# YihongSun/Dynamo-Depth

Hardware: AMD Instinct MI355X
Metric: training images/sec (192x640 triplets) (higher is better)
Workload: dtype f32

## Files before the change

### dynamo-depth_amd/csrc/dd_conv_mfma.hip

```cpp
#include <hip/hip_runtime.h>
#include <cstdlib>
#include <type_traits>

#include "../../include/dynamo_hip.h"
#include "dd_attr.h"
#include "dd_split.h"
#include "dd_store_tile.h"

namespace dd {
namespace cm {

constexpr int TH = 8, TW = 32, NT = 256;
constexpr int HH = TH + 2, HW = TW + 2, HN = HH * HW;
constexpr int CK = 16;
constexpr int PSTR = 48;
constexpr int A_PIECE = HN * PSTR;
constexpr int A_BYTES = 3 * A_PIECE;
__device__ __forceinline__ int halo_addr(int px, int half) {
  return px * 48 + half * 16;
}
__host__ __device__ constexpr int pieces_of(int products) { return products == 6 ? 3 : (products == 3 ? 2 : 1); }
constexpr int FRAG = 1024;
constexpr int PRE = (HN * 4 + NT - 1) / NT;

// ... 288 lines not shown
#pragma unroll
  for (int m = 0; m < 2; ++m) {
    const int loc = (2 * wave + m) * 32 + (lane & 31), p = p0 + loc;
    const int rem = p % (H * W), yy = rem / W, xx = rem - yy * W;
    unsigned mk = 0u;
#pragma unroll
    for (int t = 0; t < 9; ++t) {
      const int Y = yy + t / 3 - 1, X = xx + t % 3 - 1;
      if (p < M && Y >= 0 && Y < H && X >= 0 && X < W) mk |= 1u << t;
    }
    tapmask[m] = mk;
    a_base[m] = (W + 1) + loc;
  }
  const unsigned char* b_lane = s_b + lane * 16;

  uint4 af[2][2][3], bfr[2][NB][3];
  auto read_frags = [&](int set, int tap, int s) {
    const int toff = (tap / 3 - 1) * W + (tap % 3 - 1);
#pragma unroll
    for (int m = 0; m < 2; ++m) {
      const int addr = halo_addr(((tapmask[m] >> tap) & 1u) ? a_base[m] + toff : FLAT_ZERO, lane >> 5);
#pragma unroll
      for (int pc = 0; pc < pieces_of(NP); ++pc) af[set][m][pc] = *reinterpret_cast<const uint4*>(smem + addr + pc * A_PIECE);
    }
    const unsigned char* bb = b_lane + (s & 1) * b_buf_bytes<NB>();
#pragma unroll
    for (int n = 0; n < NB; ++n)
#pragma unroll
      for (int pc = 0; pc < pieces_of(NP); ++pc) bfr[set][n][pc] = *reinterpret_cast<const uint4*>(bb + (n * 3 + pc) * FRAG);
  };

  const int s_last = c_end * 9 - 1;
  float bv[NB];
#pragma unroll
  for (int n = 0; n < NB; ++n) bv[n] = tile_bias(splits == 1 ? bias : nullptr, (ntile * NB + n) * 32 + (lane & 31), n_out, pack);
  fetch_b(c_begin * 9);
  fetch(c_begin);
  store_b(c_begin * 9);
  fetch_b(min(c_begin * 9 + 1, s_last));
  for (int chunk = c_begin; chunk < c_end; ++chunk) {
    lds_barrier();
    stage(chunk);
    store_b(chunk * 9 + 1);
    lds_barrier();
    read_frags(0, 0, chunk * 9);
#pragma unroll
    for (int tap = 0; tap < 9; ++tap) {
      const int s = chunk * 9 + tap, cur = tap & 1;
      if (tap < 8) read_frags(cur ^ 1, tap + 1, s + 1);
      fetch_b(min(s + 2, s_last));
      if (tap == 1) fetch(min(chunk + 1, c_end - 1));
      constexpr int PA[6] = {2, 0, 1, 1, 0, 0}, PB[6] = {0, 2, 1, 0, 1, 0};
#pragma unroll
      for (int t = 6 - NP; t < 6; ++t)
#pragma unroll
        for (int m = 0; m < 2; ++m)
#pragma unroll
          for (int n = 0; n < NB; ++n)
            acc[m][n] = __builtin_amdgcn_mfma_f32_32x32x16_bf16(__builtin_bit_cast(bf8, af[cur][m][PA[t]]), __builtin_bit_cast(bf8, bfr[cur][n][PB[t]]), acc[m][n], 0, 0, 0);
      __builtin_amdgcn_sched_barrier(0);
      if (tap < 8) {
        store_b(s + 2);
        lds_barrier();
      }
    }
  }

  float* dst = out + (splits > 1 ? (size_t)split * M * n_out : 0);
  auto tail = [&](auto full) {
#pragma unroll
    for (int n = 0; n < NB; ++n) {
      const int co = (ntile * NB + n) * 32 + (lane & 31);
#pragma unroll
      for (int m = 0; m < 2; ++m) {
        const int p = p0 + (2 * wave + m) * 32 + 4 * (lane >> 5);
        store_acc32<decltype(full)::value>(acc[m][n], bv[n], dst + (size_t)p * n_out + co, (size_t)n_out, co < n_out ? M - p : 0, StoreF32{});
      }
    }
  };
  if (p0 + FLAT_MT <= M && (ntile + 1) * (32 * NB) <= n_out) tail(std::true_type{});
  else tail(std::false_type{});
}

__global__ __launch_bounds__(256) void conv_flat_fold_kernel(const float* __restrict__ part, const float* __restrict__ bias, int total4, int n_out, int splits,
                                                             float* __restrict__ y) {
  const int i = blockIdx.x * 256 + threadIdx.x;
  if (i >= total4) return;
  const float4* P = reinterpret_cast<const float4*>(part);
  float4 a = P[i];
  for (int s = 1; s < splits; ++s) {
    const float4 v = P[(size_t)s * total4 + i];
    a.x += v.x; a.y += v.y; a.z += v.z; a.w += v.w;
  }
  if (bias) {
    const int c = (i * 4) % n_out;
    a.x += bias[c]; a.y += bias[c + 1]; a.z += bias[c + 2]; a.w += bias[c + 3];
  }
  reinterpret_cast<float4*>(y)[i] = a;
}

static int flat_splits(int M, int k_in, int n_out) {
  const int wgs = ((M + FLAT_MT - 1) / FLAT_MT) * ((n_out + 63) / 64), nchunks = (k_in + CK - 1) / CK;
  const char* env = getenv("DD_FLAT_SPLITS");
  int s = env ? atoi(env) : (480 + wgs / 2) / wgs;
  if (s > nchunks / 2) s = nchunks / 2;
  return s < 1 ? 1 : s;
}

static size_t pack_bytes(int n_out, int k_in) { return (size_t)frags_of(n_out, k_in) * 3 * FRAG; }

template <int NB, int NP>
static int launch(const float* x, const void* pack, const float* bias, int B, int Hi, int Wi, int k_in, int n_out, int pad, float* y, hipStream_t stream) {
  const int Ho = Hi + 2 * pad - 2, Wo = Wi + 2 * pad - 2;
  const int tiles_x = (Wo + TW - 1) / TW, tiles_y = (Ho + TH - 1) / TH;
  auto kern = conv_mfma_kernel<NB, NP>;
  static dd::LdsAttrOnce lds_attr;
  if (const int rc = lds_attr.ensure(reinterpret_cast<const void*>(kern), (int)(lds_bytes<NB>()))) return rc;
  dim3 grid(tiles_x * tiles_y, (n_out + 32 * NB - 1) / (32 * NB), B);
  hipLaunchKernelGGL(kern, grid, dim3(NT), lds_bytes<NB>(), stream, x, static_cast<const uint4*>(pack), bias, Hi, Wi, Ho, Wo, k_in, n_out, pad, tiles_x,
                     tiles_y, y);
  return (int)hipGetLastError();
}

template <int NP>
static int launch_blocks(const float* x, const void* pack, const float* bias, int B, int Hi, int Wi, int k_in, int n_out, int pad, float* y, hipStream_t s) {
  switch (blocks_for(n_out)) {
    case 1: return launch<1, NP>(x, pack, bias, B, Hi, Wi, k_in, n_out, pad, y, s);
    case 2: return launch<2, NP>(x, pack, bias, B, Hi, Wi, k_in, n_out, pad, y, s);
    default: return launch<3, NP>(x, pack, bias, B, Hi, Wi, k_in, n_out, pad, y, s);
  }
}

template <int NP>
static int launch_flat(const float* x, const void* pack, const float* bias, int H, int W, int M, int k_in, int n_out, int splits, float* out, hipStream_t s) {
  auto kern = conv_mfma_flat_kernel<2, NP>;
  static dd::LdsAttrOnce lds_attr;
  if (const int rc = lds_attr.ensure(reinterpret_cast<const void*>(kern), (int)(lds_bytes<2>()))) return rc;
  hipLaunchKernelGGL(kern, dim3((M + FLAT_MT - 1) / FLAT_MT, (n_out + 63) / 64, splits), dim3(NT), lds_bytes<2>(), s, x, static_cast<const uint4*>(pack), bias, H, W, M, k_in,
                     n_out, splits, out);
  return (int)hipGetLastError();
}

namespace wg {
constexpr int TR = 2, TC = 16;
constexpr int XR = TR + 2, XC = TC + 2;
constexpr int XROW = 24;
constexpr int GSTR = TR * TC * 2 + 16;
constexpr int XSTR = XR * XROW * 2 + 16;
constexpr int G_PIECE = 64 * GSTR, X_PIECE = 64 * XSTR;
constexpr int LDS = 3 * (G_PIECE + X_PIECE);
constexpr int XITEMS = XR * (XC / 2) * 16;
constexpr int XJ = (XITEMS + NT - 1) / NT;
constexpr int BLOCK = 64 * 9 * 64;
}

template <int NP>
__global__ __launch_bounds__(NT, 2) void conv_wgrad_kernel(const float* __restrict__ x, const float* __restrict__ g, int B, int Hi, int Wi, int Ho, int Wo,
                                                           int cin, int cout, int pad, int tiles_x, int tiles_y, float* __restrict__ partial) {
  using namespace wg;
  extern __shared__ __align__(16) unsigned char smem[];
  unsigned char* const s_g = smem;
  unsigned char* const s_x = smem + 3 * G_PIECE;
  const int tid = threadIdx.x, lane = tid & 63, wave = __builtin_amdgcn_readfirstlane(tid >> 6);
  const int ks = blockIdx.x, nks = gridDim.x, ci0 = blockIdx.y * 64, co0 = blockIdx.z * 64;
  const int total = B * tiles_y * tiles_x;
  const int t_begin = (int)((long long)total * ks / nks), t_end = (int)((long long)total * (ks + 1) / nks);

  const int gq = tid >> 4, grow = (tid >> 3) & 1, gpair = tid & 7;
  const int g_lds = (4 * gq) * GSTR + (grow * TC + 2 * gpair) * 2;
  int xq[XJ], xrow[XJ], xpair[XJ], x_lds[XJ];
#pragma unroll
  for (int j = 0; j < XJ; ++j) {
    const int item = tid + j * NT;
    xq[j] = item / (XR * (XC / 2));
    const int rem = item - xq[j] * (XR * (XC / 2));
    xrow[j] = rem / (XC / 2);
    xpair[j] = rem - xrow[j] * (XC / 2);
    x_lds[j] = item < XITEMS ? (4 * xq[j]) * XSTR + (xrow[j] * XROW + 2 * xpair[j]) * 2 : -1;
  }
  const bool g_ch = co0 + 4 * gq < cout;

  float4 pg[2], px[XJ][2];
  auto fetch = [&](int t) {
    const int b = t / (tiles_y * tiles_x), r = t - b * (tiles_y * tiles_x);
    const int Y0 = (r / tiles_x) * TR, X0 = (r - (r / tiles_x) * tiles_x) * TC;
    {
      const int Y = Y0 + grow, X = X0 + 2 * gpair;
      const float* src = g + (((size_t)b * Ho + Y) * Wo + X) * cout + co0 + 4 * gq;
      const bool ok = g_ch && Y < Ho;
      pg[0] = (ok && X < Wo) ? *reinterpret_cast<const float4*>(src) : make_float4(0.f, 0.f, 0.f, 0.f);
      pg[1] = (ok && X + 1 < Wo) ? *reinterpret_cast<const float4*>(src + cout) : make_float4(0.f, 0.f, 0.f, 0.f);
    }
#pragma unroll
    for (int j = 0; j < XJ; ++j) {
      const int Y = Y0 - pad + xrow[j], X = X0 - pad + 2 * xpair[j];
      const bool ok = x_lds[j] >= 0 && ci0 + 4 * xq[j] < cin && Y >= 0 && Y < Hi;
      const float* src = x + (((ptrdiff_t)b * Hi + Y) * Wi + X) * cin + ci0 + 4 * xq[j];
      px[j][0] = (ok && X >= 0 && X < Wi) ? *reinterpret_cast<const float4*>(src) : make_float4(0.f, 0.f, 0.f, 0.f);
      px[j][1] = (ok && X + 1 >= 0 && X + 1 < Wi) ? *reinterpret_cast<const float4*>(src + cin) : make_float4(0.f, 0.f, 0.f, 0.f);
    }
  };
  auto put = [&](unsigned char* plane, int piece_bytes, int stride, int off, const float4& a, const float4& b) {
    const float av[4] = {a.x, a.y, a.z, a.w}, bv[4] = {b.x, b.y, b.z, b.w};
#pragma unroll
    for (int c = 0; c < 4; ++c) {
      unsigned p1, p2, p3;
      split2(av[c], bv[c], p1, p2, p3);
      *reinterpret_cast<unsigned*>(plane + off + c * stride) = p1;
      if (pieces_of(NP) > 1) *reinterpret_cast<unsigned*>(plane + piece_bytes + off + c * stride) = p2;
      if (pieces_of(NP) > 2) *reinterpret_cast<unsigned*>(plane + 2 * piece_bytes + off + c * stride) = p3;
    }
  };
  auto stage = [&]() {
    put(s_g, G_PIECE, GSTR, g_lds, pg[0], pg[1]);
#pragma unroll
    for (int j = 0; j < XJ; ++j)
      if (x_lds[j] >= 0) put(s_x, X_PIECE, XSTR, x_lds[j], px[j][0], px[j][1]);
  };

  const int ngroups = (cin - ci0 > 32) ? 6 : 3;
  const int g_full = wave, g_half = 4 + (wave >> 1), half = wave & 1;
  const bool full_on = g_full < ngroups, half_on = g_half < ngroups;
  auto group_off = [&](int g) { return (g / 3) * 32 * XSTR + (g % 3) * (XROW * 2); };
  const int off_full = group_off(g_full), off_half = group_off(g_half);
  f16v acc[9];
#pragma unroll
  for (int a = 0; a < 9; ++a)
#pragma unroll
    for (int r = 0; r < 16; ++r) acc[a][r] = 0.f;

  const unsigned char* a_lane = s_g + (lane & 31) * GSTR + (lane >> 5) * 16;
  const unsigned char* b_lane = s_x + (lane & 31) * XSTR + (lane >> 5) * 16;
  constexpr int PA[6] = {2, 0, 1, 1, 0, 0}, PB[6] = {0, 2, 1, 0, 1, 0};
  auto shifted = [](const uint4& w0, unsigned w1, int tx) -> uint4 {
    if (tx == 0) return w0;
    if (tx == 2) return make_uint4(w0.y, w0.z, w0.w, w1);
    return make_uint4(__builtin_amdgcn_alignbit(w0.y, w0.x, 16), __builtin_amdgcn_alignbit(w0.z, w0.y, 16), __builtin_amdgcn_alignbit(w0.w, w0.z, 16),
                      __builtin_amdgcn_alignbit(w1, w0.w, 16));
  };

  if (t_begin < t_end) fetch(t_begin);
  for (int t = t_begin; t < t_end; ++t) {
    __syncthreads();
    stage();
    __syncthreads();
    if (t + 1 < t_end) fetch(t + 1);
#pragma unroll
    for (int row = 0; row < TR; ++row) {
      uint4 af[2][3];
#pragma unroll
      for (int m = 0; m < 2; ++m)
#pragma unroll
        for (int pc = 0; pc < pieces_of(NP); ++pc) af[m][pc] = *reinterpret_cast<const uint4*>(a_lane + m * 32 * GSTR + row * (TC * 2) + pc * G_PIECE);
      uint4 w0[3];
      unsigned w1[3];
      if (full_on) {
#pragma unroll
        for (int pc = 0; pc < pieces_of(NP); ++pc) {
          const unsigned char* src = b_lane + off_full + row * (XROW * 2) + pc * X_PIECE;
          w0[pc] = *reinterpret_cast<const uint4*>(src);
          w1[pc] = *reinterpret_cast<const unsigned*>(src + 16);
        }
#pragma unroll
        for (int tx = 0; tx < 3; ++tx) {
          uint4 bf[3];
#pragma unroll
          for (int pc = 0; pc < pieces_of(NP); ++pc) bf[pc] = shifted(w0[pc], w1[pc], tx);
#pragma unroll
          for (int tt = 6 - NP; tt < 6; ++tt)
#pragma unroll
            for (int m = 0; m < 2; ++m)
              acc[tx * 2 + m] = __builtin_amdgcn_mfma_f32_32x32x16_bf16(__builtin_bit_cast(bf8, af[m][PA[tt]]), __builtin_bit_cast(bf8, bf[PB[tt]]),
                                                                        acc[tx * 2 + m], 0, 0, 0);
          __builtin_amdgcn_sched_barrier(0);
        }
      }
      if (half_on) {
#pragma unroll
        for (int pc = 0; pc < pieces_of(NP); ++pc) {
          const unsigned char* src = b_lane + off_half + row * (XROW * 2) + pc * X_PIECE;
          w0[pc] = *reinterpret_cast<const uint4*>(src);
          w1[pc] = *reinterpret_cast<const unsigned*>(src + 16);
        }
        {
          const int txd = half == 0 ? 0 : 2;
          uint4 bf[3];
#pragma unroll
          for (int pc = 0; pc < pieces_of(NP); ++pc) bf[pc] = txd == 0 ? shifted(w0[pc], w1[pc], 0) : shifted(w0[pc], w1[pc], 2);
#pragma unroll
          for (int tt = 6 - NP; tt < 6; ++tt)
#pragma unroll
            for (int m = 0; m < 2; ++m)
              acc[6 + m] = __builtin_amdgcn_mfma_f32_32x32x16_bf16(__builtin_bit_cast(bf8, af[m][PA[tt]]), __builtin_bit_cast(bf8, bf[PB[tt]]), acc[6 + m], 0, 0, 0);
          __builtin_amdgcn_sched_barrier(0);
          uint4 am[3];
#pragma unroll
          for (int pc = 0; pc < pieces_of(NP); ++pc) {
            bf[pc] = shifted(w0[pc], w1[pc], 1);
            am[pc] = half == 0 ? af[0][pc] : af[1][pc];
          }
#pragma unroll
          for (int tt = 6 - NP; tt < 6; ++tt)
            acc[8] = __builtin_amdgcn_mfma_f32_32x32x16_bf16(__builtin_bit_cast(bf8, am[PA[tt]]), __builtin_bit_cast(bf8, bf[PB[tt]]), acc[8], 0, 0, 0);
        }
      }
    }
  }

  float* P = partial + (((size_t)blockIdx.z * gridDim.y + blockIdx.y) * nks + ks) * BLOCK;
  auto put_acc = [&](const f16v& A, int g, int tx, int m) {
    const int nb = g / 3, tap = (g % 3) * 3 + tx;
#pragma unroll
    for (int r = 0; r < 16; ++r) {
      const int co = m * 32 + (r & 3) + 8 * (r >> 2) + 4 * (lane >> 5);
      P[(co * 9 + tap) * 64 + nb * 32 + (lane & 31)] = A[r];
    }
  };
  if (full_on) {
#pragma unroll
    for (int tx = 0; tx < 3; ++tx)
#pragma unroll
      for (int m = 0; m < 2; ++m) put_acc(acc[tx * 2 + m], g_full, tx, m);
  }
  if (half_on) {
    put_acc(acc[6], g_half, half == 0 ? 0 : 2, 0);
    put_acc(acc[7], g_half, half == 0 ? 0 : 2, 1);
    put_acc(acc[8], g_half, 1, half);
  }
}

__global__ __launch_bounds__(256) void conv_wgrad_fold_kernel(const float* __restrict__ partial, int nks, int cin, int cout, int ci_groups, float* __restrict__ gw) {
  __shared__ float red[4][64];
  const int lane = threadIdx.x & 63, wave = threadIdx.x >> 6;
  const int idx = blockIdx.x * 64 + lane;
  const bool in = idx < cout * 9 * cin;
  float s[8] = {0.f, 0.f, 0.f, 0.f, 0.f, 0.f, 0.f, 0.f};
  if (in) {
    const int ci = idx % cin, tap = (idx / cin) % 9, co = idx / (9 * cin);
    const int z = co >> 6, y = ci >> 6;
    const float* P = partial + ((size_t)z * ci_groups + y) * nks * wg::BLOCK + ((co & 63) * 9 + tap) * 64 + (ci & 63);
    int k = wave;
    for (; k + 28 < nks; k += 32) {
#pragma unroll
      for (int j = 0; j < 8; ++j) s[j] += P[(size_t)(k + 4 * j) * wg::BLOCK];
    }
    for (; k < nks; k += 4) s[0] += P[(size_t)k * wg::BLOCK];
  }
  red[wave][lane] = ((s[0] + s[1]) + (s[2] + s[3])) + ((s[4] + s[5]) + (s[6] + s[7]));
  __syncthreads();
  if (wave == 0 && in) gw[idx] = (red[0][lane] + red[1][lane]) + (red[2][lane] + red[3][lane]);
}

static int wgrad_splits(int B, int Ho, int Wo, int cin, int cout) {
  const int groups = ((cin + 63) / 64) * ((cout + 63) / 64);
  const int tiles = B * ((Ho + wg::TR - 1) / wg::TR) * ((Wo + wg::TC - 1) / wg::TC);
  int n = 512 / groups;
  if (n > tiles / 11) n = tiles / 11;
  return n < 1 ? 1 : n;
}

}
}

extern "C" int dd_conv3x3_mfma_supported(int cin, int cout) {
  return (cin >= 16 && cout >= 16 && cin % 4 == 0 && cout % 4 == 0 && cin <= 1024 && cout <= 1024) ? 1 : 0;
}

extern "C" size_t dd_conv3x3_mfma_pack_bytes(int n_out, int k_in) { return dd::cm::pack_bytes(n_out, k_in); }

extern "C" int dd_conv3x3_mfma_pack(const float* weight, long long s_co, long long s_ci, long long s_kh, long long s_kw, int cout, int cin, void* pack_fwd,
                                    void* pack_bwd_data, void* stream) {
  using namespace dd::cm;
  if (!weight || (!pack_fwd && !pack_bwd_data) || cout < 1 || cin < 1) return (int)hipErrorInvalidValue;
  const int frags_fwd = pack_fwd ? (int)(pack_bytes(cout, cin) / (3 * FRAG)) : 0;
  const int frags_bwd = pack_bwd_data ? (int)(pack_bytes(cin, cout) / (3 * FRAG)) : 0;
  const int threads = (frags_fwd + frags_bwd) * 64;
  hipLaunchKernelGGL(conv_mfma_pack_kernel, dim3((threads + 255) / 256), dim3(256), 0, static_cast<hipStream_t>(stream), weight, s_co, s_ci, s_kh, s_kw, cout,
                     cin, static_cast<uint4*>(pack_fwd), static_cast<uint4*>(pack_bwd_data), frags_fwd, frags_bwd);
  return (int)hipGetLastError();
}

extern "C" int dd_conv3x3_mfma_pack_many_job_words(void) { return dd::cm::PACK_JOB_WORDS; }

extern "C" int dd_conv3x3_mfma_pack_many_blocks(int cout, int cin, int want_fwd, int want_bwd_data) {
  using namespace dd::cm;
  if (cout < 1 || cin < 1) return 0;
  return ((want_fwd ? frags_of(cout, cin) : 0) + (want_bwd_data ? frags_of(cin, cout) : 0) + 3) / 4;
}

extern "C" int dd_conv3x3_mfma_pack_many(const long long* jobs, const int* block_job, int n_blocks, void* stream) {
  using namespace dd::cm;
  if (!jobs || !block_job || n_blocks < 1) return (int)hipErrorInvalidValue;
  hipLaunchKernelGGL(conv_mfma_pack_many_kernel, dim3(n_blocks), dim3(256), 0, static_cast<hipStream_t>(stream), jobs, block_job);
  return (int)hipGetLastError();
}

extern "C" int dd_conv3x3_mfma_n(const float* x, const void* pack, const float* bias, int B, int Hi, int Wi, int k_in, int n_out, int pad, int products,
                                 float* y, void* stream) {
  using namespace dd::cm;
  if (!x || !pack || !y || B < 1 || pad < 0 || pad > 2 || Hi + 2 * pad < 3 || Wi + 2 * pad < 3 || k_in % 4 || k_in < 4 || n_out < 1) return (int)hipErrorInvalidValue;
  if ((size_t)Hi * Wi * k_in >= (1ull << 31) || (reinterpret_cast<unsigned long long>(x) & 15ull)) return (int)hipErrorInvalidValue;
  hipStream_t s = static_cast<hipStream_t>(stream);
  switch (products) {
    case 6: return launch_blocks<6>(x, pack, bias, B, Hi, Wi, k_in, n_out, pad, y, s);
    case 3: return launch_blocks<3>(x, pack, bias, B, Hi, Wi, k_in, n_out, pad, y, s);
    case 1: return launch_blocks<1>(x, pack, bias, B, Hi, Wi, k_in, n_out, pad, y, s);
    default: return (int)hipErrorInvalidValue;
  }
}

extern "C" int dd_conv3x3_mfma(const float* x, const void* pack, const float* bias, int B, int Hi, int Wi, int k_in, int n_out, int pad, float* y,
                               void* stream) {
  return dd_conv3x3_mfma_n(x, pack, bias, B, Hi, Wi, k_in, n_out, pad, 6, y, stream);
}

extern "C" int dd_conv3x3_mfma_flat_supported(int B, int H, int W, int k_in, int n_out) {
  using namespace dd::cm;
  return (B >= 1 && H >= 1 && W >= 1 && W <= FLAT_MAX_W && k_in >= 32 && k_in % 4 == 0 && k_in <= 1024 && n_out % 4 == 0 && n_out <= 1024 &&
          blocks_for(n_out) == 2 && n_out > 32 &&
          (size_t)B * H * W * (size_t)(k_in > n_out ? k_in : n_out) < (1ull << 31)) ? 1 : 0;
}

extern "C" size_t dd_conv3x3_mfma_flat_workspace_bytes(int B, int H, int W, int k_in, int n_out) {
  using namespace dd::cm;
  const int M = B * H * W, s = flat_splits(M, k_in, n_out);
  return s > 1 ? (size_t)s * M * n_out * sizeof(float) : 16;
}

extern "C" int dd_conv3x3_mfma_flat_n(const float* x, const void* pack, const float* bias, int B, int H, int W, int k_in, int n_out, int products, float* y,
                                      void* workspace, size_t workspace_bytes, void* stream) {
  using namespace dd::cm;
  if (!x || !pack || !y || !dd_conv3x3_mfma_flat_supported(B, H, W, k_in, n_out) || (reinterpret_cast<unsigned long long>(x) & 15ull) ||
      (reinterpret_cast<unsigned long long>(y) & 15ull) || (products != 6 && products != 3 && products != 1))
    return (int)hipErrorInvalidValue;
  const int M = B * H * W, splits = flat_splits(M, k_in, n_out);
  if (splits > 1 && (!workspace || workspace_bytes < dd_conv3x3_mfma_flat_workspace_bytes(B, H, W, k_in, n_out) || (reinterpret_cast<unsigned long long>(workspace) & 15ull)))
    return (int)hipErrorInvalidValue;
  hipStream_t s = static_cast<hipStream_t>(stream);
  float* out = splits > 1 ? static_cast<float*>(workspace) : y;
  const int rc = products == 6 ? launch_flat<6>(x, pack, bias, H, W, M, k_in, n_out, splits, out, s)
               : products == 3 ? launch_flat<3>(x, pack, bias, H, W, M, k_in, n_out, splits, out, s)
                               : launch_flat<1>(x, pack, bias, H, W, M, k_in, n_out, splits, out, s);
  if (rc != 0 || splits == 1) return rc;
  const int total4 = M * n_out / 4;
  hipLaunchKernelGGL(conv_flat_fold_kernel, dim3((total4 + 255) / 256), dim3(256), 0, s, static_cast<const float*>(workspace), bias, total4, n_out, splits, y);
  return (int)hipGetLastError();
}

extern "C" int dd_conv3x3_mfma_flat(const float* x, const void* pack, const float* bias, int B, int H, int W, int k_in, int n_out, float* y, void* workspace,
                                    size_t workspace_bytes, void* stream) {
  return dd_conv3x3_mfma_flat_n(x, pack, bias, B, H, W, k_in, n_out, 6, y, workspace, workspace_bytes, stream);
}

extern "C" size_t dd_conv3x3_mfma_wgrad_workspace_bytes(int B, int Ho, int Wo, int cin, int cout) {
  const size_t groups = (size_t)((cin + 63) / 64) * ((cout + 63) / 64);
  return groups * dd::cm::wgrad_splits(B, Ho, Wo, cin, cout) * dd::cm::wg::BLOCK * sizeof(float);
}

extern "C" int dd_conv3x3_mfma_bwd_weight_n(const float* x, const float* g_out, int B, int Hi, int Wi, int cin, int cout, int pad, int products, float* g_weight,
                                            void* workspace, size_t workspace_bytes, void* stream) {
  using namespace dd::cm;
  if (!x || !g_out || !g_weight || !workspace || B < 1 || pad < 0 || pad > 1 || cin % 4 || cout % 4 || cin < 4 || cout < 4) return (int)hipErrorInvalidValue;
  if (products != 6 && products != 3 && products != 1) return (int)hipErrorInvalidValue;
  const int Ho = Hi + 2 * pad - 2, Wo = Wi + 2 * pad - 2;
  if (Ho < 1 || Wo < 1 || workspace_bytes < dd_conv3x3_mfma_wgrad_workspace_bytes(B, Ho, Wo, cin, cout)) return (int)hipErrorInvalidValue;
  if ((size_t)B * Hi * Wi * cin >= (1ull << 31) || (size_t)B * Ho * Wo * cout >= (1ull << 31)) return (int)hipErrorInvalidValue;
  if ((reinterpret_cast<unsigned long long>(x) | reinterpret_cast<unsigned long long>(g_out)) & 15ull) return (int)hipErrorInvalidValue;
  hipStream_t s = static_cast<hipStream_t>(stream);
  const int tiles_x = (Wo + wg::TC - 1) / wg::TC, tiles_y = (Ho + wg::TR - 1) / wg::TR;
  const int nks = wgrad_splits(B, Ho, Wo, cin, cout), ci_groups = (cin + 63) / 64, co_groups = (cout + 63) / 64;
  const dim3 grid(nks, ci_groups, co_groups);
  float* part = static_cast<float*>(workspace);
  if (products == 6)
    hipLaunchKernelGGL(conv_wgrad_kernel<6>, grid, dim3(NT), wg::LDS, s, x, g_out, B, Hi, Wi, Ho, Wo, cin, cout, pad, tiles_x, tiles_y, part);
  else if (products == 3)
    hipLaunchKernelGGL(conv_wgrad_kernel<3>, grid, dim3(NT), wg::LDS, s, x, g_out, B, Hi, Wi, Ho, Wo, cin, cout, pad, tiles_x, tiles_y, part);
  else
    hipLaunchKernelGGL(conv_wgrad_kernel<1>, grid, dim3(NT), wg::LDS, s, x, g_out, B, Hi, Wi, Ho, Wo, cin, cout, pad, tiles_x, tiles_y, part);
  hipError_t e = hipGetLastError();
  if (e != hipSuccess) return (int)e;
  hipLaunchKernelGGL(conv_wgrad_fold_kernel, dim3((cout * 9 * cin + 63) / 64), dim3(256), 0, s, static_cast<const float*>(workspace), nks, cin, cout, ci_groups,
                     g_weight);
  return (int)hipGetLastError();
}

extern "C" int dd_conv3x3_mfma_bwd_weight(const float* x, const float* g_out, int B, int Hi, int Wi, int cin, int cout, int pad, float* g_weight, void* workspace,
                                          size_t workspace_bytes, void* stream) {
  return dd_conv3x3_mfma_bwd_weight_n(x, g_out, B, Hi, Wi, cin, cout, pad, 6, g_weight, workspace, workspace_bytes, stream);
}
```

### dynamo-depth_amd/csrc/dd_decoder.hip

```cpp
#include <hip/hip_runtime.h>

#include "dd_half.h"
#include "dd_math.h"

namespace dd {

constexpr int DEC_NT = 256;

__device__ __forceinline__ float elu1(float v) {
  float h = 0x1.ed9a98p-8f;
  h = fmaf(h, v, 0x1.53f994p-5f);
  h = fmaf(h, v, 0x1.554e28p-3f);
  h = fmaf(h, v, 0x1.ffffe8p-2f);
  const float near0 = v * fmaf(h, v, 1.f), far = __expf(v) - 1.f;
  return v > 0.f ? v : (v > -0.25f ? near0 : far);
}
__device__ __forceinline__ float elu1_grad(float v) { return v <= 0.f ? expf(v) : 1.f; }
template <bool ELU>
__device__ __forceinline__ float4 act4(float4 v) {
  if (ELU) return make_float4(elu1(v.x), elu1(v.y), elu1(v.z), elu1(v.w));
  return v;
}

__device__ __forceinline__ void bilinear_src(int o, int n, int& i0, int& i1, float& l1) {
  const float src = fmaxf((o + 0.5f) * 0.5f - 0.5f, 0.f);
  i0 = (int)src;
  i1 = i0 + (i0 < n - 1 ? 1 : 0);
  l1 = src - (float)i0;
}

template <typename T, int MODE, bool ELU>
__global__ __launch_bounds__(DEC_NT) void up_cat_pad_kernel(const T* __restrict__ x, const T* __restrict__ skip, int h, int w, int C1q, int C2q,
                                                            T* __restrict__ out) {
  const int H = MODE == 2 ? h : 2 * h, W = MODE == 2 ? w : 2 * w, Wp = W + 2, Cq = C1q + C2q;
  const int yo = blockIdx.y, b = blockIdx.z;
  const int j = blockIdx.x * DEC_NT + threadIdx.x;
  if (j >= Wp * Cq) return;
  const int xo = j / Cq, cq = j - xo * Cq;
  const int Y = dd_reflect(yo - 1, H), X = dd_reflect(xo - 1, W);
  float4 v;
  if (cq >= C1q) {
    v = IO<T>::load4(skip, (((long long)b * H + Y) * W + X) * C2q + (cq - C1q));
  } else if (MODE == 2) {
    v = act4<ELU>(IO<T>::load4(x, (((long long)b * h + Y) * w + X) * C1q + cq));
  } else if (MODE == 0) {
    v = act4<ELU>(IO<T>::load4(x, (((long long)b * h + (Y >> 1)) * w + (X >> 1)) * C1q + cq));
  } else {
    int y0, y1, x0, x1;
    float ly, lx;
    bilinear_src(Y, h, y0, y1, ly);
    bilinear_src(X, w, x0, x1, lx);
    const long long r0 = ((long long)b * h + y0) * w, r1 = ((long long)b * h + y1) * w;
    const float4 a = act4<ELU>(IO<T>::load4(x, (r0 + x0) * C1q + cq)), bb = act4<ELU>(IO<T>::load4(x, (r0 + x1) * C1q + cq));
    const float4 c = act4<ELU>(IO<T>::load4(x, (r1 + x0) * C1q + cq)), d = act4<ELU>(IO<T>::load4(x, (r1 + x1) * C1q + cq));
    const float hy = 1.f - ly, hx = 1.f - lx;
    v.x = hy * (hx * a.x + lx * bb.x) + ly * (hx * c.x + lx * d.x);
    v.y = hy * (hx * a.y + lx * bb.y) + ly * (hx * c.y + lx * d.y);
    v.z = hy * (hx * a.z + lx * bb.z) + ly * (hx * c.z + lx * d.z);
    v.w = hy * (hx * a.w + lx * bb.w) + ly * (hx * c.w + lx * d.w);
  }
  IO<T>::store4(out, ((long long)b * (H + 2) + yo) * Wp * Cq + j, v);
}

template <typename T>
__device__ __forceinline__ float4 pad_fold(const T* __restrict__ g, int b, int Y, int X, int H, int W, int Cq, int cq) {
  const int Hp = H + 2, Wp = W + 2;
  const int ys[2] = {Y + 1, Y == 1 ? 0 : (Y == H - 2 ? Hp - 1 : -1)};
  const int xs[2] = {X + 1, X == 1 ? 0 : (X == W - 2 ? Wp - 1 : -1)};
  float4 acc = make_float4(0.f, 0.f, 0.f, 0.f);
#pragma unroll
  for (int a = 0; a < 2; ++a)
#pragma unroll
    for (int d = 0; d < 2; ++d)
      if (ys[a] >= 0 && xs[d] >= 0) {
        const float4 t = IO<T>::load4(g, (((long long)b * Hp + ys[a]) * Wp + xs[d]) * Cq + cq);
        acc.x += t.x; acc.y += t.y; acc.z += t.z; acc.w += t.w;
      }
  return acc;
}

template <int MODE>
__device__ __forceinline__ int up_taps(int i, int n, int (&o)[4], float (&wt)[4]) {
  if (MODE == 0) {
    o[0] = 2 * i; o[1] = 2 * i + 1; wt[0] = wt[1] = 1.f;
    return 2;
  }
  int cnt = 0;
  if (i >= 1) { o[cnt] = 2 * i - 1; wt[cnt++] = 0.25f; }
  o[cnt] = 2 * i; wt[cnt++] = i == 0 ? 1.f : 0.75f;
  o[cnt] = 2 * i + 1; wt[cnt++] = i == n - 1 ? 1.f : 0.75f;
  if (i + 1 <= n - 1) { o[cnt] = 2 * i + 2; wt[cnt++] = 0.25f; }
  return cnt;
}

template <typename T, int MODE, bool ELU>
__global__ __launch_bounds__(DEC_NT) void up_cat_pad_bwd_x_kernel(const T* __restrict__ g, const T* __restrict__ x, int h, int w, int C1q, int C2q,
                                                                  T* __restrict__ gx) {
  const int H = MODE == 2 ? h : 2 * h, W = MODE == 2 ? w : 2 * w, Cq = C1q + C2q;
  const int yi = blockIdx.y, b = blockIdx.z;
  const int j = blockIdx.x * DEC_NT + threadIdx.x;
  if (j >= w * C1q) return;
  const int xi = j / C1q, cq = j - xi * C1q;
  float4 acc = make_float4(0.f, 0.f, 0.f, 0.f);
  if (MODE == 2) {
    acc = pad_fold<T>(g, b, yi, xi, H, W, Cq, cq);
  } else {
    int oy[4], ox[4];
    float wy[4], wx[4];
    const int ny = up_taps<MODE>(yi, h, oy, wy), nx = up_taps<MODE>(xi, w, ox, wx);
    for (int a = 0; a < ny; ++a)
      for (int d = 0; d < nx; ++d) {
        const float4 t = pad_fold<T>(g, b, oy[a], ox[d], H, W, Cq, cq);
        const float wgt = wy[a] * wx[d];
        acc.x += wgt * t.x; acc.y += wgt * t.y; acc.z += wgt * t.z; acc.w += wgt * t.w;
      }
  }
  const long long at = ((long long)b * h + yi) * w * C1q + j;
  if (ELU) {
    const float4 v = IO<T>::load4(x, at);
    acc.x *= elu1_grad(v.x); acc.y *= elu1_grad(v.y); acc.z *= elu1_grad(v.z); acc.w *= elu1_grad(v.w);
  }
  IO<T>::store4(gx, at, acc);
}

template <typename T>
__global__ __launch_bounds__(DEC_NT) void up_cat_pad_bwd_skip_kernel(const T* __restrict__ g, int H, int W, int C1q, int C2q, T* __restrict__ gs) {
  const int Y = blockIdx.y, b = blockIdx.z;
  const int j = blockIdx.x * DEC_NT + threadIdx.x;
  if (j >= W * C2q) return;
  const int X = j / C2q, cq = j - X * C2q;
  IO<T>::store4(gs, ((long long)b * H + Y) * W * C2q + j, pad_fold<T>(g, b, Y, X, H, W, C1q + C2q, C1q + cq));
}

template <typename T>
static void up_cat_pad_launch(const void* x_, const void* skip_, int B, int h, int w, int C1, int C2, int mode, int elu, void* out_, hipStream_t s) {
  const T* x = static_cast<const T*>(x_);
  const T* skip = static_cast<const T*>(skip_);
  T* out = static_cast<T*>(out_);
  const int H = mode == 2 ? h : 2 * h, W = mode == 2 ? w : 2 * w, C1q = C1 / 4, C2q = C2 / 4;
  const dim3 grid(((W + 2) * (C1q + C2q) + DEC_NT - 1) / DEC_NT, H + 2, B), block(DEC_NT);
#define DD_UCP(M, E) hipLaunchKernelGGL((up_cat_pad_kernel<T, M, E>), grid, block, 0, s, x, skip, h, w, C1q, C2q, out)
  if (mode == 0) { if (elu) DD_UCP(0, true); else DD_UCP(0, false); }
  else if (mode == 1) { if (elu) DD_UCP(1, true); else DD_UCP(1, false); }
  else { if (elu) DD_UCP(2, true); else DD_UCP(2, false); }
#undef DD_UCP
}

template <typename T>
static void up_cat_pad_bwd_launch(const void* g_, const void* x_, int B, int h, int w, int C1, int C2, int mode, int elu, void* gx_, void* gs_,
                                  hipStream_t s) {
  const T* g = static_cast<const T*>(g_);
  const T* x = static_cast<const T*>(x_);
  T* gx = static_cast<T*>(gx_);
  T* gs = static_cast<T*>(gs_);
  const int H = mode == 2 ? h : 2 * h, W = mode == 2 ? w : 2 * w, C1q = C1 / 4, C2q = C2 / 4;
  if (gx) {
    const dim3 grid((w * C1q + DEC_NT - 1) / DEC_NT, h, B), block(DEC_NT);
#define DD_UCPB(M, E) hipLaunchKernelGGL((up_cat_pad_bwd_x_kernel<T, M, E>), grid, block, 0, s, g, x, h, w, C1q, C2q, gx)
    if (mode == 0) { if (elu) DD_UCPB(0, true); else DD_UCPB(0, false); }
    else if (mode == 1) { if (elu) DD_UCPB(1, true); else DD_UCPB(1, false); }
    else { if (elu) DD_UCPB(2, true); else DD_UCPB(2, false); }
#undef DD_UCPB
  }
  if (gs && C2q > 0)
    hipLaunchKernelGGL(up_cat_pad_bwd_skip_kernel<T>, dim3((W * C2q + DEC_NT - 1) / DEC_NT, H, B), dim3(DEC_NT), 0, s, g, H, W, C1q, C2q, gs);
}

}

using namespace dd;

static bool up_cat_pad_ok(const void* x, int B, int h, int w, int C1, int C2, int mode, int dtype) {
  const int H = mode == 2 ? h : 2 * h, W = mode == 2 ? w : 2 * w;
  return x && B >= 1 && B <= 65535 && h >= 2 && w >= 2 && H >= 4 && W >= 4 && H + 2 <= 65535 && C1 >= 4 && C1 % 4 == 0 && C2 >= 0 && C2 % 4 == 0 &&
         mode >= 0 && mode <= 2 && dtype >= 0 && dtype <= 2;
}

extern "C" int dd_up_cat_pad_t(const void* x, const void* skip, int B, int h, int w, int C1, int C2, int mode, int elu, void* out, int dtype,
                               void* stream) {
  if (!up_cat_pad_ok(x, B, h, w, C1, C2, mode, dtype) || !out || (C2 > 0 && !skip)) return (int)hipErrorInvalidValue;
  DD_DISPATCH_DTYPE(dtype, up_cat_pad_launch, x, skip, B, h, w, C1, C2, mode, elu, out, static_cast<hipStream_t>(stream));
  return (int)hipGetLastError();
}

extern "C" int dd_up_cat_pad_bwd_t(const void* g_out, const void* x, int B, int h, int w, int C1, int C2, int mode, int elu, void* g_x, void* g_skip,
                                   int dtype, void* stream) {
  if (!up_cat_pad_ok(x, B, h, w, C1, C2, mode, dtype) || !g_out || (!g_x && !g_skip)) return (int)hipErrorInvalidValue;
  DD_DISPATCH_DTYPE(dtype, up_cat_pad_bwd_launch, g_out, x, B, h, w, C1, C2, mode, elu, g_x, g_skip, static_cast<hipStream_t>(stream));
  return (int)hipGetLastError();
}
```

### dynamo-depth_amd/csrc/dd_redu.hip

```cpp
#include <hip/hip_runtime.h>

#include "../../include/dynamo_hip.h"

namespace dd {

constexpr int RD_NT = 256;
constexpr int RD_MAX_BLOCKS = 1024;
constexpr int RD_FOLD = 32;

__device__ __forceinline__ float rd_dot4(const float4 a, const float4 b) { return fmaf(a.x, b.x, fmaf(a.y, b.y, fmaf(a.z, b.z, a.w * b.w))); }

template <int C4>
__device__ __forceinline__ void rd_stage_weights(const float* __restrict__ w, int cout, float4* s_w) {
  for (int i = threadIdx.x; i < cout * 2 * C4; i += RD_NT) s_w[i] = reinterpret_cast<const float4*>(w)[i];
  __syncthreads();
}

template <int COUT, int LPP, int QUADS>
__global__ __launch_bounds__(RD_NT) void redu_fwd_kernel(const float* __restrict__ a, const float* __restrict__ b, const float* __restrict__ w,
                                                         const float* __restrict__ bias, long long P, float* __restrict__ y) {
  constexpr int C4 = LPP * QUADS, PX = RD_NT / LPP;
  __shared__ float4 s_w[COUT * 2 * C4];
  rd_stage_weights<C4>(w, COUT, s_w);
  const int pl = threadIdx.x / LPP, q = threadIdx.x % LPP;
  const float4* a4 = reinterpret_cast<const float4*>(a);
  const float4* b4 = reinterpret_cast<const float4*>(b);
  float bv[COUT];
#pragma unroll
  for (int co = 0; co < COUT; ++co) bv[co] = bias ? bias[co] : 0.f;
  const long long groups = (P + PX - 1) / PX;
  for (long long grp = blockIdx.x; grp < groups; grp += gridDim.x) {
    const long long p = grp * PX + pl;
    const long long pc = p < P ? p : P - 1;
    float acc[COUT];
#pragma unroll
    for (int co = 0; co < COUT; ++co) acc[co] = 0.f;
#pragma unroll
    for (int j = 0; j < QUADS; ++j) {
      const int c4 = q + LPP * j;
      const float4 av = a4[pc * C4 + c4], bb = b4[pc * C4 + c4];
#pragma unroll
      for (int co = 0; co < COUT; ++co) acc[co] += rd_dot4(av, s_w[co * 2 * C4 + c4]) + rd_dot4(bb, s_w[co * 2 * C4 + C4 + c4]);
    }
#pragma unroll
    for (int co = 0; co < COUT; ++co) {
#pragma unroll
      for (int m = 1; m < LPP; m <<= 1) acc[co] += __shfl_xor(acc[co], m, 64);
    }
    if (q == 0 && p < P) {
#pragma unroll
      for (int co = 0; co < COUT; ++co) y[p * COUT + co] = acc[co] + bv[co];
    }
  }
}

template <int COUT, int LPP, int QUADS>
__global__ __launch_bounds__(RD_NT) void redu_bwd_data_kernel(const float* __restrict__ g, const float* __restrict__ w, long long P, float* __restrict__ ga,
                                                              float* __restrict__ gb) {
  constexpr int C4 = LPP * QUADS, PX = RD_NT / LPP;
  __shared__ float4 s_w[COUT * 2 * C4];
  rd_stage_weights<C4>(w, COUT, s_w);
  const int pl = threadIdx.x / LPP, q = threadIdx.x % LPP;
  const long long groups = (P + PX - 1) / PX;
  for (long long grp = blockIdx.x; grp < groups; grp += gridDim.x) {
    const long long p = grp * PX + pl;
    if (p >= P) continue;
    float gv[COUT];
#pragma unroll
    for (int co = 0; co < COUT; ++co) gv[co] = g[p * COUT + co];
#pragma unroll
    for (int j = 0; j < QUADS; ++j) {
      const int c4 = q + LPP * j;
      float4 ra = make_float4(0.f, 0.f, 0.f, 0.f), rb = ra;
#pragma unroll
      for (int co = 0; co < COUT; ++co) {
        const float4 wa = s_w[co * 2 * C4 + c4], wb = s_w[co * 2 * C4 + C4 + c4];
        ra.x = fmaf(gv[co], wa.x, ra.x); ra.y = fmaf(gv[co], wa.y, ra.y); ra.z = fmaf(gv[co], wa.z, ra.z); ra.w = fmaf(gv[co], wa.w, ra.w);
        rb.x = fmaf(gv[co], wb.x, rb.x); rb.y = fmaf(gv[co], wb.y, rb.y); rb.z = fmaf(gv[co], wb.z, rb.z); rb.w = fmaf(gv[co], wb.w, rb.w);
      }
      if (ga) reinterpret_cast<float4*>(ga)[p * C4 + c4] = ra;
      if (gb) reinterpret_cast<float4*>(gb)[p * C4 + c4] = rb;
    }
  }
}

template <int COUT, int LPP, int QUADS>
__global__ __launch_bounds__(RD_NT) void redu_wgrad_kernel(const float* __restrict__ a, const float* __restrict__ b, const float* __restrict__ g, long long P,
                                                           float* __restrict__ part) {
  constexpr int C4 = LPP * QUADS, PX = RD_NT / LPP, C = 4 * C4, N = COUT * 2 * C + COUT;
  constexpr int SLOTS = COUT * QUADS * 2 * 4 + COUT, STR = SLOTS | 1;
  extern __shared__ float s_red[];
  const int pl = threadIdx.x / LPP, q = threadIdx.x % LPP;
  const float4* a4 = reinterpret_cast<const float4*>(a);
  const float4* b4 = reinterpret_cast<const float4*>(b);
  float4 accA[COUT][QUADS], accB[COUT][QUADS];
  float gs[COUT];
#pragma unroll
  for (int co = 0; co < COUT; ++co) {
    gs[co] = 0.f;
#pragma unroll
    for (int j = 0; j < QUADS; ++j) accA[co][j] = accB[co][j] = make_float4(0.f, 0.f, 0.f, 0.f);
  }
  const long long groups = (P + PX - 1) / PX;
  for (long long grp = blockIdx.x; grp < groups; grp += gridDim.x) {
    const long long p = grp * PX + pl;
    if (p >= P) continue;
    float gv[COUT];
#pragma unroll
    for (int co = 0; co < COUT; ++co) { gv[co] = g[p * COUT + co]; gs[co] += gv[co]; }
#pragma unroll
    for (int j = 0; j < QUADS; ++j) {
      const int c4 = q + LPP * j;
      const float4 av = a4[p * C4 + c4], bb = b4[p * C4 + c4];
#pragma unroll
      for (int co = 0; co < COUT; ++co) {
        accA[co][j].x = fmaf(gv[co], av.x, accA[co][j].x); accA[co][j].y = fmaf(gv[co], av.y, accA[co][j].y);
        accA[co][j].z = fmaf(gv[co], av.z, accA[co][j].z); accA[co][j].w = fmaf(gv[co], av.w, accA[co][j].w);
        accB[co][j].x = fmaf(gv[co], bb.x, accB[co][j].x); accB[co][j].y = fmaf(gv[co], bb.y, accB[co][j].y);
        accB[co][j].z = fmaf(gv[co], bb.z, accB[co][j].z); accB[co][j].w = fmaf(gv[co], bb.w, accB[co][j].w);
      }
    }
  }
  float* mine = s_red + threadIdx.x * STR;
#pragma unroll
  for (int co = 0; co < COUT; ++co) {
#pragma unroll
    for (int j = 0; j < QUADS; ++j) {
      const int t = ((co * QUADS + j) * 2) * 4;
      mine[t] = accA[co][j].x; mine[t + 1] = accA[co][j].y; mine[t + 2] = accA[co][j].z; mine[t + 3] = accA[co][j].w;
      mine[t + 4] = accB[co][j].x; mine[t + 5] = accB[co][j].y; mine[t + 6] = accB[co][j].z; mine[t + 7] = accB[co][j].w;
    }
    mine[COUT * QUADS * 8 + co] = q == 0 ? gs[co] : 0.f;
  }
  __syncthreads();
  for (int e = threadIdx.x; e < N; e += RD_NT) {
    float s = 0.f;
    if (e < COUT * 2 * C) {
      const int co = e / (2 * C), r = e - co * 2 * C, half = r / C, c = r - half * C;
      const int cq = c >> 2, qq = cq % LPP, j = cq / LPP, slot = ((co * QUADS + j) * 2 + half) * 4 + (c & 3);
#pragma unroll 4
      for (int pp = 0; pp < PX; ++pp) s += s_red[(pp * LPP + qq) * STR + slot];
    } else {
      const int co = e - COUT * 2 * C;
#pragma unroll 4
      for (int pp = 0; pp < PX; ++pp) s += s_red[(pp * LPP) * STR + COUT * QUADS * 8 + co];
    }
    part[(long long)blockIdx.x * N + e] = s;
  }
}

__global__ __launch_bounds__(RD_NT) void redu_fold1_kernel(const float* __restrict__ part, int nparts, int N, float* __restrict__ slices) {
  const int e = blockIdx.x * RD_NT + threadIdx.x, sl = blockIdx.y;
  if (e >= N) return;
  float a0 = 0.f, a1 = 0.f;
  int i = sl;
  for (; i + RD_FOLD < nparts; i += 2 * RD_FOLD) { a0 += part[(long long)i * N + e]; a1 += part[(long long)(i + RD_FOLD) * N + e]; }
  if (i < nparts) a0 += part[(long long)i * N + e];
  slices[(long long)sl * N + e] = a0 + a1;
}
__global__ __launch_bounds__(RD_NT) void redu_fold2_kernel(const float* __restrict__ slices, int N, int nw, float* __restrict__ gw, float* __restrict__ gbias) {
  const int e = blockIdx.x * RD_NT + threadIdx.x;
  if (e >= N) return;
  float a[4] = {0.f, 0.f, 0.f, 0.f};
#pragma unroll
  for (int i = 0; i < RD_FOLD; ++i) a[i & 3] += slices[(long long)i * N + e];
  const float v = (a[0] + a[1]) + (a[2] + a[3]);
  if (e < nw) gw[e] = v;
  else if (gbias) gbias[e - nw] = v;
}

struct ReduShape { int lpp, quads; };
static inline ReduShape redu_shape(int C) {
  ReduShape s = {0, 0};
  if (C == 64) s = {16, 1};
  else if (C == 128) s = {32, 1};
  else if (C == 256) s = {64, 1};
  else if (C == 512) s = {64, 2};
  return s;
}
static inline int redu_blocks(long long P, int lpp) {
  const long long groups = (P + RD_NT / lpp - 1) / (RD_NT / lpp);
  long long nb = (groups + 7) / 8;
  if (nb < 1) nb = 1;
  return (int)(nb > RD_MAX_BLOCKS ? RD_MAX_BLOCKS : nb);
}

}

extern "C" int dd_redu_supported(int C, int cout) { return dd::redu_shape(C).lpp != 0 && (cout == 1 || cout == 3); }

extern "C" size_t dd_redu_workspace_bytes(long long P, int C, int cout) {
  if (!dd_redu_supported(C, cout) || P < 1) return 0;
  const size_t N = (size_t)cout * 2 * C + cout;
  return ((size_t)dd::redu_blocks(P, dd::redu_shape(C).lpp) + dd::RD_FOLD) * N * sizeof(float);
}

#define DD_REDU_DISPATCH(KERNEL, GRID, LDS, ...)                                                                                             \
  do {                                                                                                                                       \
    const dd::ReduShape sh_ = dd::redu_shape(C);                                                                                             \
    if (cout == 1) {                                                                                                                         \
      if (sh_.lpp == 16) hipLaunchKernelGGL((dd::KERNEL<1, 16, 1>), GRID, dim3(dd::RD_NT), LDS(1, 1), st, __VA_ARGS__);                         \
      else if (sh_.lpp == 32) hipLaunchKernelGGL((dd::KERNEL<1, 32, 1>), GRID, dim3(dd::RD_NT), LDS(1, 1), st, __VA_ARGS__);                    \
      else if (sh_.quads == 1) hipLaunchKernelGGL((dd::KERNEL<1, 64, 1>), GRID, dim3(dd::RD_NT), LDS(1, 1), st, __VA_ARGS__);                   \
      else hipLaunchKernelGGL((dd::KERNEL<1, 64, 2>), GRID, dim3(dd::RD_NT), LDS(1, 2), st, __VA_ARGS__);                                        \
    } else {                                                                                                                                 \
      if (sh_.lpp == 16) hipLaunchKernelGGL((dd::KERNEL<3, 16, 1>), GRID, dim3(dd::RD_NT), LDS(3, 1), st, __VA_ARGS__);                         \
      else if (sh_.lpp == 32) hipLaunchKernelGGL((dd::KERNEL<3, 32, 1>), GRID, dim3(dd::RD_NT), LDS(3, 1), st, __VA_ARGS__);                    \
      else if (sh_.quads == 1) hipLaunchKernelGGL((dd::KERNEL<3, 64, 1>), GRID, dim3(dd::RD_NT), LDS(3, 1), st, __VA_ARGS__);                   \
      else hipLaunchKernelGGL((dd::KERNEL<3, 64, 2>), GRID, dim3(dd::RD_NT), LDS(3, 2), st, __VA_ARGS__);                                        \
    }                                                                                                                                        \
  } while (0)
#define DD_REDU_NO_LDS(co, qd) 0
#define DD_REDU_WG_LDS(co, qd) ((size_t)dd::RD_NT * ((((co) * (qd) * 8 + (co))) | 1) * sizeof(float))

extern "C" int dd_redu_fwd(const float* a, const float* b, const float* weight, const float* bias, long long P, int C, int cout, float* y, void* stream) {
  if (!a || !b || !weight || !y || P < 1 || !dd_redu_supported(C, cout)) return (int)hipErrorInvalidValue;
  hipStream_t st = (hipStream_t)stream;
  const dim3 grid(dd::redu_blocks(P, dd::redu_shape(C).lpp));
  DD_REDU_DISPATCH(redu_fwd_kernel, grid, DD_REDU_NO_LDS, a, b, weight, bias, P, y);
  return (int)hipGetLastError();
}

extern "C" int dd_redu_bwd_data(const float* g_out, const float* weight, long long P, int C, int cout, float* g_a, float* g_b, void* stream) {
  if (!g_out || !weight || (!g_a && !g_b) || P < 1 || !dd_redu_supported(C, cout)) return (int)hipErrorInvalidValue;
  hipStream_t st = (hipStream_t)stream;
  const dim3 grid(dd::redu_blocks(P, dd::redu_shape(C).lpp));
  DD_REDU_DISPATCH(redu_bwd_data_kernel, grid, DD_REDU_NO_LDS, g_out, weight, P, g_a, g_b);
  return (int)hipGetLastError();
}

extern "C" int dd_redu_bwd_weight(const float* a, const float* b, const float* g_out, long long P, int C, int cout, float* g_weight, float* g_bias,
                                  void* workspace, size_t workspace_bytes, void* stream) {
  if (!a || !b || !g_out || !g_weight || !workspace || P < 1 || !dd_redu_supported(C, cout)) return (int)hipErrorInvalidValue;
  if (workspace_bytes < dd_redu_workspace_bytes(P, C, cout)) return (int)hipErrorInvalidValue;
  hipStream_t st = (hipStream_t)stream;
  const int blocks = dd::redu_blocks(P, dd::redu_shape(C).lpp);
  const int nw = cout * 2 * C, N = nw + cout;
  float* part = static_cast<float*>(workspace);
  float* slices = part + (size_t)blocks * N;
  const dim3 grid(blocks);
  DD_REDU_DISPATCH(redu_wgrad_kernel, grid, DD_REDU_WG_LDS, a, b, g_out, P, part);
  hipLaunchKernelGGL(dd::redu_fold1_kernel, dim3((N + dd::RD_NT - 1) / dd::RD_NT, dd::RD_FOLD), dim3(dd::RD_NT), 0, st, part, blocks, N, slices);
  hipLaunchKernelGGL(dd::redu_fold2_kernel, dim3((N + dd::RD_NT - 1) / dd::RD_NT), dim3(dd::RD_NT), 0, st, slices, N, nw, g_weight, g_bias);
  return (int)hipGetLastError();
}
```

### dynamo-depth_amd/hipops/abi.py

```python
import ctypes as C

DD_MAX_SCALES = 4
DD_NUM_SRC = 2
DD_ABI_VERSION = 2
DD_MODE_RIGID, DD_MODE_FLOW, DD_MODE_FLOW_MASK = 0, 1, 2
DD_PARTIAL_STRIDE = 40
DD_SUMS_STRIDE = 8

_fp = C.c_void_p


class DDPhotoScale(C.Structure):
    _fields_ = [
        ("shift", C.c_int), ("h", C.c_int), ("w", C.c_int),
        ("w_photo", C.c_float), ("w_cons", C.c_float),
        ("disp", _fp),
        ("flow", _fp * DD_NUM_SRC),
        ("mask", _fp * DD_NUM_SRC),
        ("noise", _fp),
        ("g_disp", _fp),
        ("g_flow", _fp * DD_NUM_SRC),
        ("g_mask", _fp * DD_NUM_SRC),
        ("out_color", _fp * DD_NUM_SRC),
        ("out_sample", _fp * DD_NUM_SRC),
# ... 4 lines not shown
    ]


class DDPhotoArgs(C.Structure):
    _fields_ = [
        ("abi_version", C.c_int),
        ("B", C.c_int), ("H", C.c_int), ("W", C.c_int),
        ("num_scales", C.c_int), ("mode", C.c_int), ("automask", C.c_int), ("want_grad", C.c_int),
        ("min_depth", C.c_float), ("max_depth", C.c_float), ("ssim_weight", C.c_float),
        ("eps", C.c_float), ("disp_thr", C.c_float),
        ("target", _fp),
        ("source", _fp * DD_NUM_SRC),
        ("source_packed", _fp * DD_NUM_SRC),
        ("K", _fp), ("inv_K", _fp),
        ("T", _fp * DD_NUM_SRC),
        ("ts", _fp * DD_NUM_SRC),
        ("g_T", _fp * DD_NUM_SRC),
        ("sums", _fp),
        ("workspace", _fp),
        ("scale", DDPhotoScale * DD_MAX_SCALES),
    ]


DD_NUM_TERMS = 7
DD_MAX_RES = 128
TERM_NAMES = ("p_photo", "d_smooth", "d_ground", "c_smooth", "c_consistency", "m_sparsity", "m_smooth")


class DDAssembleArgs(C.Structure):
    _fields_ = [
        ("n", C.c_int), ("num_scales", C.c_int),
        ("coef", C.c_float * DD_NUM_TERMS),
        ("norm", C.c_float * DD_MAX_RES),
        ("term_of", C.c_int8 * DD_MAX_RES),
        ("scale_of", C.c_int8 * DD_MAX_RES),
    ]


DD_VIS_MAX_TILES = 16
DD_VIS_KINDS = {"img": 0, "ref_img": 1, "disp": 2, "mask": 3, "ego_flow": 4, "ind_flow": 5, "comp_flow": 6, "samp_flow": 7}

DD_REG_SMOOTH = 5
DD_REG_RES_STRIDE = 16


class DDRegSmooth(C.Structure):
    _fields_ = [("inp", _fp), ("g_inp", _fp), ("C", C.c_int), ("normalise", C.c_int), ("weight", C.c_float)]


class DDRegScale(C.Structure):
    _fields_ = [
        ("h", C.c_int), ("w", C.c_int),
        ("img", _fp),
        ("smooth", DDRegSmooth * DD_REG_SMOOTH),
        ("delta", _fp * DD_NUM_SRC), ("delta_sum", _fp * DD_NUM_SRC), ("prob", _fp * DD_NUM_SRC), ("g_prob", _fp * DD_NUM_SRC),
        ("w_sparsity", C.c_float * DD_NUM_SRC),
        ("disp", _fp), ("g_disp", _fp), ("inv_K", _fp), ("rand_idx", _fp), ("plane", _fp),
        ("w_ground", C.c_float),
    ]


class DDRegArgs(C.Structure):
    _fields_ = [
        ("abi_version", C.c_int), ("B", C.c_int), ("num_scales", C.c_int),
        ("np_per_it", C.c_int), ("max_it", C.c_int),
        ("tol", C.c_float), ("g_prior", C.c_float), ("min_depth", C.c_float), ("max_depth", C.c_float),
        ("res", _fp), ("workspace", _fp),
        ("scale", DDRegScale * DD_MAX_SCALES),
    ]


class DDJpegHeader(C.Structure):
    _fields_ = [("data_offset", C.c_int32), ("data_end", C.c_int32), ("width", C.c_int32), ("height", C.c_int32), ("restart_interval", C.c_int32),
                ("ncomp", C.c_int32), ("h", C.c_int32 * 3), ("v", C.c_int32 * 3), ("tq", C.c_int32 * 3), ("td", C.c_int32 * 3), ("ta", C.c_int32 * 3),
                ("reserved", C.c_int32 * 3), ("qt", (C.c_uint16 * 64) * 4), ("bits", (C.c_uint8 * 16) * 4), ("vals", (C.c_uint8 * 256) * 4)]


def ptr(t):
    return None if t is None else C.c_void_p(t.data_ptr())


def declare(lib):
    i, f, v, z = C.c_int, C.c_float, C.c_void_p, C.c_size_t
    sig = {
        "dd_photo_loss": (i, [C.POINTER(DDPhotoArgs), v]),
        "dd_photo_workspace_bytes": (z, [C.POINTER(DDPhotoArgs)]),
        "dd_photo_timing": (i, [i]),
        "dd_photo_timing_read": (i, [C.POINTER(C.c_float), C.POINTER(i), i]),
        "dd_smooth_loss": (i, [v, v, i, i, i, i, i, f, v, v, v, v]),
        "dd_smooth_workspace_bytes": (z, [i, i, i, i]),
        "dd_ground_loss": (i, [v, v, v, i, i, i, i, i, f, f, f, f, f, v, v, v, v, v]),
        "dd_ground_workspace_bytes": (z, [i, i, i, i]),
        "dd_resize_workspace_bytes": (z, [i, i, i, i, i]),
        "dd_resize_bicubic": (i, [v, i, i, i, v, v, i, i, v, v, i, v, v, i, v, z, v]),
        "dd_ground_candidates": (i, [v, v, v, i, i, i, i, i, f, f, f, v, v]),
        "dd_ground_select": (i, [v, v, v, i, i, i, i, f, f, f, f, f, v, v, v, v, v, v]),
        "dd_ground_plane": (i, [v, v, i, i, i, i, i, f, f, v, v, v, v]),
        "dd_assemble_losses": (i, [v, C.POINTER(DDAssembleArgs), v, v, v]),
        "dd_reg_losses_finish": (i, [C.POINTER(DDRegArgs), C.POINTER(DDAssembleArgs), v, v, v]),
        "dd_fused_loss": (i, [C.POINTER(DDPhotoArgs), C.POINTER(DDRegArgs), C.POINTER(DDAssembleArgs), v, v, v]),
        "dd_fused_loss_part": (i, [C.POINTER(DDPhotoArgs), C.POINTER(DDRegArgs), C.POINTER(DDAssembleArgs), v, v, v, i]),
        "dd_fused_loss_supported": (i, [C.POINTER(DDPhotoArgs), C.POINTER(DDRegArgs)]),
        "dd_reg_workspace_bytes": (z, [C.POINTER(DDRegArgs)]),
        "dd_jpeg_workspace_bytes": (z, [i, i, i, i, C.POINTER(C.c_int), C.POINTER(C.c_int)]),
        "dd_jpeg_decode": (i, [v, C.c_longlong, v, i, i, i, i, C.POINTER(C.c_int), C.POINTER(C.c_int), v, v, z, v]),
        "dd_backproject": (i, [v, v, i, i, i, v, v]),
        "dd_backproject_bwd": (i, [v, v, i, i, i, v, v]),
        "dd_project3d": (i, [v, v, v, i, i, i, f, v, v, v]),
        "dd_project3d_bwd": (i, [v, v, v, v, v, i, i, i, f, v, v, v, v]),
        "dd_project3d_workspace_bytes": (z, [i, i, i]),
        "dd_ssim": (i, [v, v, i, i, i, i, v, v]),
        "dd_ssim_bwd": (i, [v, v, v, i, i, i, i, v, v, v]),
        "dd_disp_to_depth": (i, [v, z, f, f, v, v, v]),
        "dd_pose_matrix": (i, [v, v, i, i, v, v]),
        "dd_pose_matrix_bwd": (i, [v, v, v, i, i, v, v, v]),
        "dd_channel_sum_nhwc": (i, [v, C.c_longlong, i, v, v, v]),
        "dd_channel_sum_workspace_bytes": (z, [i]),
        "dd_reflect_pad1_nhwc": (i, [v, i, i, i, i, v, v]),
        "dd_reflect_pad1_nhwc_bwd": (i, [v, i, i, i, i, v, v]),
        "dd_dwconv3x3_nhwc": (i, [v, v, i, i, i, i, i, v, v]),
        "dd_dwconv3x3_nhwc_bwd_data": (i, [v, v, i, i, i, i, i, v, v]),
        "dd_dwconv3x3_nhwc_bwd_weight": (i, [v, v, i, i, i, i, i, v, v, z, v]),
        "dd_dwconv3x3_workspace_bytes": (z, [i, i, i]),
        "dd_conv3x3_cout1_bwd_data": (i, [v, v, i, i, i, i, i, v, v]),
        "dd_prepare_frames": (i, [v, v, v, i, i, i, i, v, v, v, v]),
        "dd_prepare_frames_workspace_bytes": (z, [i, i]),
        "dd_pyramid_down2": (i, [v, i, i, i, v, v]),
        "dd_pack_rgb": (i, [v, i, i, i, v, v]),
        "dd_depth_metrics": (i, [v, i, i, i, v, v, i, v, C.POINTER(C.c_double), f, f, v, v, v, z, v]),
        "dd_depth_metrics_workspace_bytes": (z, [i, i]),
        "dd_depth_metrics_masked": (i, [v, i, i, i, v, v, i, v, C.POINTER(C.c_double), f, f, v, i, i, v, v, v, v, z, v]),
        "dd_depth_metrics_masked_workspace_bytes": (z, [i, i]),
        "dd_depth_metrics_accumulate": (i, [v, v, i, v, v, v]),
        "dd_odom_snippet_count": (i, [i, i]),
        "dd_odom_snippets": (i, [v, v, i, i, v, v, v]),
        "dd_motion_pr": (i, [v, i, i, i, v, v, i, i, v, i, i, v, v]),
        "dd_fill_contours": (i, [v, i, v, i, i, i, i, v, v]),
        "dd_lidar_depth_points_workspace_bytes": (z, [i, i, i, i]),
        "dd_lidar_depth_points": (i, [v, C.c_longlong, C.POINTER(C.c_int32), i, v, i, i, i, v, v, v, v, z, v]),
        "dd_vis_frame": (i, [v, v, v, v, v, v, v, v, f, f, i, i, C.POINTER(C.c_int), i, i, i, v, f, f, f, f, i, i, v, v, v, v]),
        "dd_vis_flow_tiles": (i, [v, v, C.POINTER(C.c_int), i, i, i, i, i, i, f, i, v, v]),
        "dd_export_depth": (i, [v, v, v, i, i, i, i, i, f, f, f, v, f, f, v, v, v, v]),
        "dd_export_plane_u8": (i, [v, i, i, i, i, i, v, v]),
        "dd_bn_act_fwd": (i, [v, v, C.c_longlong, i, v, v, f, f, v, v, v, v, i, v, v, z, v]),
        "dd_bn_act_bwd": (i, [v, v, v, C.c_longlong, i, v, v, v, v, i, v, v, v, v, v, z, v]),
        "dd_bn_workspace_bytes": (z, [i]),
        "dd_bn_act_fwd_t": (i, [v, v, C.c_longlong, i, v, v, f, f, v, v, v, v, i, v, i, v, z, v]),
        "dd_bn_act_bwd_t": (i, [v, v, v, C.c_longlong, i, v, v, v, v, i, v, v, v, v, i, v, z, v]),
        "dd_channel_sum_nhwc_t": (i, [v, C.c_longlong, i, v, i, v, v]),
        "dd_reflect_pad1_nhwc_t": (i, [v, i, i, i, i, v, i, v]),
        "dd_reflect_pad1_nhwc_bwd_t": (i, [v, i, i, i, i, v, i, v]),
        "dd_up_cat_pad_t": (i, [v, v, i, i, i, i, i, i, i, v, i, v]),
        "dd_up_cat_pad_bwd_t": (i, [v, v, i, i, i, i, i, i, i, v, v, i, v]),
        "dd_layer_norm_fwd": (i, [v, C.c_longlong, i, v, v, f, v, v, v, v]),
        "dd_layer_norm_bwd": (i, [v, v, v, v, v, C.c_longlong, i, v, v, v, z, v]),
        "dd_layer_norm_workspace_bytes": (z, [i]),
        "dd_layer_scale_bwd": (i, [v, v, v, i, i, i, v, v, v, z, v]),
        "dd_layer_scale_workspace_bytes": (z, [i, i]),
        "dd_layer_norm_fwd_t": (i, [v, C.c_longlong, i, v, v, f, v, v, v, i, v]),
        "dd_layer_norm_bwd_t": (i, [v, v, v, v, v, C.c_longlong, i, v, v, v, z, i, v]),
        "dd_layer_scale_bwd_t": (i, [v, v, v, i, i, i, v, v, v, z, i, v]),
        "dd_layer_scale_fwd_t": (i, [v, v, v, i, i, i, v, i, v]),
        "dd_dwconv3x3_nhwc_t": (i, [v, v, i, i, i, i, i, v, i, v]),
        "dd_dwconv3x3_nhwc_bwd_data_t": (i, [v, v, i, i, i, i, i, v, i, v]),
        "dd_dwconv3x3_nhwc_bwd_weight_t": (i, [v, v, i, i, i, i, i, v, v, z, i, v]),
        "dd_redu_supported": (i, [i, i]),
        "dd_redu_workspace_bytes": (z, [C.c_longlong, i, i]),
        "dd_redu_fwd": (i, [v, v, v, v, C.c_longlong, i, i, v, v]),
        "dd_redu_bwd_data": (i, [v, v, C.c_longlong, i, i, v, v, v]),
        "dd_redu_bwd_weight": (i, [v, v, v, C.c_longlong, i, i, v, v, v, z, v]),
        "dd_conv_head_supported": (i, [i]),
        "dd_conv_head_workspace_bytes": (z, [i, i, i, i]),
        "dd_conv_head_fwd": (i, [v, v, C.c_longlong, C.c_longlong, C.c_longlong, v, i, i, i, i, v, v]),
        "dd_conv_head_bwd_weight": (i, [v, v, i, i, i, i, v, v, v, z, v]),
        "dd_conv_small_supported": (i, [i, i, i]),
        "dd_conv_small_workspace_bytes": (z, [i, i, i]),
        "dd_conv_small_fwd": (i, [v, v, C.c_longlong, C.c_longlong, C.c_longlong, C.c_longlong, v, i, i, i, i, i, i, v, v, z, v]),
        "dd_conv_small_bwd_data": (i, [v, v, C.c_longlong, C.c_longlong, C.c_longlong, C.c_longlong, i, i, i, i, i, i, v, v, z, v]),
        "dd_conv_small_bwd_weight": (i, [v, v, i, i, i, i, i, i, v, v, v, z, v]),
        "dd_conv3x3_mfma_supported": (i, [i, i]),
        "dd_conv3x3_mfma_pack_bytes": (z, [i, i]),
        "dd_conv3x3_mfma_pack": (i, [v, C.c_longlong, C.c_longlong, C.c_longlong, C.c_longlong, i, i, v, v, v]),
        "dd_conv3x3_mfma_pack_many_job_words": (i, []),
        "dd_conv3x3_mfma_pack_many_blocks": (i, [i, i, i, i]),
        "dd_conv3x3_mfma_pack_many": (i, [v, v, i, v]),
        "dd_conv3x3_mfma": (i, [v, v, v, i, i, i, i, i, i, v, v]),
        "dd_conv3x3_mfma_n": (i, [v, v, v, i, i, i, i, i, i, i, v, v]),
        "dd_conv3x3_mfma_flat_supported": (i, [i, i, i, i, i]),
        "dd_conv3x3_mfma_flat_workspace_bytes": (z, [i, i, i, i, i]),
        "dd_conv3x3_mfma_flat": (i, [v, v, v, i, i, i, i, i, v, v, z, v]),
        "dd_conv3x3_mfma_flat_n": (i, [v, v, v, i, i, i, i, i, i, v, v, z, v]),
        "dd_conv3x3_mfma_wgrad_workspace_bytes": (z, [i, i, i, i, i]),
        "dd_conv3x3_mfma_bwd_weight": (i, [v, v, i, i, i, i, i, i, v, v, z, v]),
        "dd_conv3x3_mfma_bwd_weight_n": (i, [v, v, i, i, i, i, i, i, i, v, v, z, v]),
        "dd_conv3x3_half_supported": (i, [i, i]),
        "dd_conv3x3_half_pack_bytes": (z, [i, i]),
        "dd_conv3x3_half_pack": (i, [v, C.c_longlong, C.c_longlong, C.c_longlong, C.c_longlong, i, i, i, v, v, v]),
        "dd_conv3x3_half": (i, [v, v, v, i, i, i, i, i, i, i, v, v]),
        "dd_conv3x3_half_wgrad_workspace_bytes": (z, [i, i, i, i, i]),
        "dd_conv3x3_half_bwd_weight": (i, [v, v, i, i, i, i, i, i, i, v, v, z, v]),
        "dd_pw_gemm_pack_bytes": (z, [i, i]),
        "dd_mlp_pack": (i, [v, C.c_longlong, C.c_longlong, v, C.c_longlong, C.c_longlong, i, i, v, v, v, v, v, v]),
        "dd_mlp_fwd_supported": (i, [i]),
        "dd_mlp_fwd": (i, [v, v, v, v, v, i, i, v, v]),
        "dd_pw_gemm": (i, [v, v, v, i, i, i, i, v, v]),
        "dd_gelu_pair": (i, [v, v, v, z, v]),
        "dd_linear_wgrad_supported": (i, [i, i, i]),
        "dd_linear_wgrad_workspace_bytes": (z, [i, i, i]),
        "dd_linear_wgrad": (i, [v, v, i, i, i, v, v, v, z, v]),
        "dd_linear_wgrad_n": (i, [v, v, i, i, i, i, v, v, v, z, v]),
        "dd_adam_chunk": (i, []),
        "dd_adam_multi": (i, [v, i, v, i, v, C.c_double, C.c_double, C.c_double, C.c_double, C.c_double, v, v, v]),
        "dd_error_string": (C.c_char_p, [i]),
        "dd_abi_version": (i, []),
    }
    found = []
    for name, (res, args) in sig.items():
        try:
            fn = getattr(lib, name)
        except AttributeError:
            continue
        fn.restype = res
        fn.argtypes = args
        found.append(name)
    return found


EXPORTED = (
    "dd_photo_loss", "dd_photo_workspace_bytes", "dd_photo_timing", "dd_photo_timing_read", "dd_photo_loss_part", "dd_smooth_loss", "dd_smooth_workspace_bytes",
    "dd_ground_loss", "dd_ground_workspace_bytes", "dd_ground_plane", "dd_ground_candidates", "dd_ground_select",
    "dd_assemble_losses", "dd_reg_losses_finish", "dd_fused_loss", "dd_fused_loss_part", "dd_fused_loss_supported", "dd_reg_workspace_bytes", "dd_backproject", "dd_backproject_bwd", "dd_project3d", "dd_project3d_bwd", "dd_project3d_workspace_bytes",
    "dd_ssim", "dd_ssim_bwd", "dd_disp_to_depth", "dd_pose_matrix", "dd_pose_matrix_bwd",
    "dd_channel_sum_nhwc", "dd_channel_sum_workspace_bytes", "dd_reflect_pad1_nhwc", "dd_reflect_pad1_nhwc_bwd",
    "dd_dwconv3x3_nhwc", "dd_dwconv3x3_nhwc_bwd_data", "dd_dwconv3x3_nhwc_bwd_weight", "dd_dwconv3x3_workspace_bytes", "dd_conv3x3_cout1_bwd_data",
    "dd_prepare_frames", "dd_prepare_frames_workspace_bytes", "dd_pyramid_down2", "dd_pack_rgb", "dd_depth_metrics", "dd_depth_metrics_workspace_bytes", "dd_depth_metrics_masked", "dd_depth_metrics_masked_workspace_bytes", "dd_depth_metrics_accumulate", "dd_odom_snippet_count", "dd_odom_snippets", "dd_motion_pr", "dd_fill_contours", "dd_lidar_depth_points", "dd_lidar_depth_points_workspace_bytes", "dd_vis_frame", "dd_vis_flow_tiles", "dd_export_depth", "dd_export_plane_u8", "dd_bn_act_fwd", "dd_bn_act_bwd", "dd_bn_workspace_bytes",
    "dd_bn_act_fwd_t", "dd_bn_act_bwd_t", "dd_channel_sum_nhwc_t", "dd_reflect_pad1_nhwc_t", "dd_reflect_pad1_nhwc_bwd_t", "dd_up_cat_pad_t", "dd_up_cat_pad_bwd_t",
    "dd_layer_norm_fwd", "dd_layer_norm_bwd", "dd_layer_norm_workspace_bytes", "dd_layer_scale_bwd", "dd_layer_scale_workspace_bytes",
    "dd_jpeg_workspace_bytes", "dd_jpeg_decode", "dd_resize_workspace_bytes", "dd_resize_bicubic", "dd_layer_norm_fwd_t", "dd_layer_norm_bwd_t", "dd_layer_scale_bwd_t", "dd_layer_scale_fwd_t", "dd_dwconv3x3_nhwc_t", "dd_dwconv3x3_nhwc_bwd_data_t",
    "dd_dwconv3x3_nhwc_bwd_weight_t", "dd_adam_chunk", "dd_adam_multi", "dd_conv_small_supported", "dd_conv_small_workspace_bytes",
    "dd_conv_small_fwd", "dd_conv_small_bwd_data", "dd_conv_small_bwd_weight", "dd_conv_head_supported", "dd_conv_head_workspace_bytes", "dd_conv_head_fwd",
    "dd_conv_head_bwd_weight", "dd_redu_supported", "dd_redu_workspace_bytes", "dd_redu_fwd", "dd_redu_bwd_data", "dd_redu_bwd_weight",
    "dd_conv3x3_mfma_supported", "dd_conv3x3_mfma_pack_bytes", "dd_conv3x3_mfma_pack", "dd_conv3x3_mfma_pack_many_job_words",
    "dd_conv3x3_mfma_pack_many_blocks", "dd_conv3x3_mfma_pack_many", "dd_conv3x3_mfma", "dd_conv3x3_mfma_n",
    "dd_conv3x3_mfma_flat_supported", "dd_conv3x3_mfma_flat_workspace_bytes", "dd_conv3x3_mfma_flat", "dd_conv3x3_mfma_flat_n",
    "dd_conv3x3_mfma_wgrad_workspace_bytes", "dd_conv3x3_mfma_bwd_weight", "dd_conv3x3_mfma_bwd_weight_n",
    "dd_conv3x3_half_supported", "dd_conv3x3_half_pack_bytes", "dd_conv3x3_half_pack", "dd_conv3x3_half",
    "dd_conv3x3_half_wgrad_workspace_bytes", "dd_conv3x3_half_bwd_weight",
    "dd_pw_gemm_pack_bytes", "dd_mlp_pack", "dd_pw_gemm", "dd_gelu_pair", "dd_mlp_fwd_supported", "dd_mlp_fwd",
    "dd_linear_wgrad_supported", "dd_linear_wgrad_workspace_bytes", "dd_linear_wgrad", "dd_linear_wgrad_n",
    "dd_error_string", "dd_abi_version",
)


def fill_photo_args(*, B, H, W, mode, automask, want_grad, min_depth, max_depth, ssim_weight, eps, disp_thr,
                    target, source, K, inv_K, T, ts, g_T, sums, workspace, scales, source_packed=None):
    a = DDPhotoArgs()
    a.abi_version = DD_ABI_VERSION
    a.B, a.H, a.W = B, H, W
    a.num_scales = len(scales)
    a.mode, a.automask, a.want_grad = mode, int(bool(automask)), int(bool(want_grad))
    a.min_depth, a.max_depth, a.ssim_weight, a.eps, a.disp_thr = min_depth, max_depth, ssim_weight, eps, disp_thr
    a.target = ptr(target)
    a.K, a.inv_K = ptr(K), ptr(inv_K)
    a.sums, a.workspace = ptr(sums), ptr(workspace)
    for f in range(DD_NUM_SRC):
        a.source[f] = ptr(source[f])
        a.source_packed[f] = ptr(source_packed[f]) if source_packed is not None else None
        a.T[f] = ptr(T[f])
        a.ts[f] = ptr(ts[f]) if ts is not None else None
        a.g_T[f] = ptr(g_T[f]) if g_T is not None else None
    for s, d in enumerate(scales):
        sc = a.scale[s]
        sc.shift, sc.h, sc.w = d["shift"], d["h"], d["w"]
        sc.w_photo, sc.w_cons = d.get("w_photo", 0.0), d.get("w_cons", 0.0)
        for name in ("disp", "noise", "g_disp", "out_depth", "out_idsel"):
            setattr(sc, name, ptr(d.get(name)))
        for name in ("flow", "mask", "g_flow", "g_mask", "out_color", "out_sample", "out_resid", "out_delta"):
            pair = d.get(name) or (None, None)
            arr = getattr(sc, name)
            for f in range(DD_NUM_SRC):
                arr[f] = ptr(pair[f])
    return a
```

### dynamo-depth_amd/hipops/functions.py

```python
import os

import torch

from . import lib as L
from .pack_many import PackSet, _ACTIVE_PACK_SETS, _pack_many_on, pack_many_launches, pack_weights_once_per_forward


def _dev(t, name="tensor"):
    if not t.is_cuda:
        raise L.DynamoHipError("%s must live on the GPU: the Dynamo-Depth loss path has no CPU implementation "
                               "(libdynamo_hip.so is the only backend)" % name)
    if t.dtype != torch.float32:
        raise L.DynamoHipError("%s must be float32, got %s" % (name, t.dtype))
    return t.contiguous()


DTYPE_CODE = {torch.float32: 0, torch.float16: 1, torch.bfloat16: 2}


def _p(t):
    return None if t is None else t.data_ptr()


def _ws(nbytes, device):
# ... 130 lines not shown
        return g_points, None, g_T, None, None, None


class SSIMFn(torch.autograd.Function):

    @staticmethod
    def forward(ctx, x, y):
        x, y = _dev(x, "x"), _dev(y, "y")
        B, Cc, H, W = x.shape
        out = torch.empty_like(x)
        L.check(L.load().dd_ssim(_p(x), _p(y), B, Cc, H, W, _p(out), L.current_stream()), "dd_ssim")
        ctx.save_for_backward(x, y)
        return out

    @staticmethod
    def backward(ctx, g):
        x, y = ctx.saved_tensors
        B, Cc, H, W = x.shape
        g = _dev(g, "grad")
        gx = torch.empty_like(x) if ctx.needs_input_grad[0] else None
        gy = torch.empty_like(y) if ctx.needs_input_grad[1] else None
        L.check(L.load().dd_ssim_bwd(_p(x), _p(y), _p(g), B, Cc, H, W, _p(gx), _p(gy), L.current_stream()), "dd_ssim_bwd")
        return gx, gy


class DispToDepthFn(torch.autograd.Function):

    @staticmethod
    def forward(ctx, disp, min_depth, max_depth):
        disp = _dev(disp, "disp")
        scaled, depth = torch.empty_like(disp), torch.empty_like(disp)
        L.check(L.load().dd_disp_to_depth(_p(disp), disp.numel(), min_depth, max_depth, _p(scaled), _p(depth), L.current_stream()),
                "dd_disp_to_depth")
        ctx.save_for_backward(depth)
        ctx.span = 1.0 / min_depth - 1.0 / max_depth
        return scaled, depth

    @staticmethod
    def backward(ctx, g_scaled, g_depth):
        (depth,) = ctx.saved_tensors
        g = torch.zeros_like(depth)
        if g_scaled is not None:
            g = g + g_scaled * ctx.span
        if g_depth is not None:
            g = g - g_depth * depth * depth * ctx.span
        return g, None, None


class PoseMatrixFn(torch.autograd.Function):

    @staticmethod
    def forward(ctx, axisangle, translation, invert):
        B = axisangle.shape[0]
        aa = _dev(axisangle.reshape(B, 3), "axisangle")
        tr = _dev(translation.reshape(B, 3), "translation")
        T = torch.empty(B, 4, 4, dtype=torch.float32, device=aa.device)
        L.check(L.load().dd_pose_matrix(_p(aa), _p(tr), B, int(bool(invert)), _p(T), L.current_stream()), "dd_pose_matrix")
        ctx.save_for_backward(aa, tr)
        ctx.invert = int(bool(invert))
        ctx.shapes = (axisangle.shape, translation.shape)
        return T

    @staticmethod
    def backward(ctx, g):
        aa, tr = ctx.saved_tensors
        B = aa.shape[0]
        g = _dev(g, "grad")
        ga, gt = torch.empty_like(aa), torch.empty_like(tr)
        L.check(L.load().dd_pose_matrix_bwd(_p(aa), _p(tr), _p(g), B, ctx.invert, _p(ga), _p(gt), L.current_stream()), "dd_pose_matrix_bwd")
        return ga.reshape(ctx.shapes[0]), gt.reshape(ctx.shapes[1]), None


class SmoothLossFn(torch.autograd.Function):

    @staticmethod
    def forward(ctx, inp, img, normalise):
        inp = _dev(inp, "inp")
        img = None if img is None else _dev(img, "img")
        B, Cc, h, w = inp.shape
        lib = L.load()
        g = torch.zeros_like(inp)
        sums = torch.empty(2, dtype=torch.float32, device=inp.device)
        ws = _ws(lib.dd_smooth_workspace_bytes(B, Cc, h, w), inp.device)
        L.check(lib.dd_smooth_loss(_p(inp), _p(img), B, Cc, h, w, int(bool(normalise)), 1.0, _p(g), _p(sums), _p(ws), L.current_stream()),
                "dd_smooth_loss")
        ctx.save_for_backward(g)
        return sums[0] / (B * Cc * h * (w - 1)) + sums[1] / (B * Cc * (h - 1) * w)

    @staticmethod
    def backward(ctx, go):
        (g,) = ctx.saved_tensors
        return g * go, None, None


class ConvBiasFn(torch.autograd.Function):

    @staticmethod
    def forward(ctx, x, weight, bias, stride, padding, dilation, groups):
        ctx.save_for_backward(x, weight)
        ctx.conf = (stride, padding, dilation, groups, bias.shape[0])
        return torch.nn.functional.conv2d(x, weight, bias, stride, padding, dilation, groups)

    @staticmethod
    def backward(ctx, g):
        x, weight = ctx.saved_tensors
        stride, padding, dilation, groups, cout = ctx.conf
        if x.dtype != g.dtype:
            x = x.to(g.dtype)
        if weight.dtype != g.dtype:
            weight = weight.to(g.dtype)
        cin = x.shape[1]
        head = (ctx.needs_input_grad[0] and cout == 1 and _conv3x3_s1(x, weight, stride, padding, dilation, groups, ((0, 0), (1, 1)))
                and g.is_cuda and g.dtype == torch.float32 and x.dtype == torch.float32 and cin % 4 == 0 and cin <= 512
                and x.is_contiguous(memory_format=torch.channels_last) and not x.is_contiguous())
        mask = (ctx.needs_input_grad[0] and not head, ctx.needs_input_grad[1], False)
        gx, gw, _ = torch.ops.aten.convolution_backward(g, x, weight, None, stride, padding, dilation, False, [0, 0], groups, mask)
        if head:
            B, _, Hi, Wi = x.shape
            gx = torch.empty_like(x)
            L.check(L.load().dd_conv3x3_cout1_bwd_data(_p(g.contiguous()), _p(weight.contiguous()), B, Hi, Wi, cin, padding[0], _p(gx),
                                                       L.current_stream()), "dd_conv3x3_cout1_bwd_data")
        gb = None
        if ctx.needs_input_grad[2]:
            fast = g.is_cuda and g.dtype in DTYPE_CODE and g.dim() == 4 and cout <= 256
            if fast and not g.is_contiguous():
                gl = g if g.is_contiguous(memory_format=torch.channels_last) else g.contiguous(memory_format=torch.channels_last)
                B, _, H, W = gl.shape
                gb = _channel_sum(gl, B * H * W, cout, DTYPE_CODE[gl.dtype], L.current_stream())
            else:
                gb = g.sum((0, 2, 3))
        if gw is not None and gw.dtype != ctx.saved_tensors[1].dtype:
            gw = gw.to(ctx.saved_tensors[1].dtype)
        return gx, gw, (gb.to(torch.float32) if gb is not None else None), None, None, None, None


def redu_ok(a, b, conv):
    if os.environ.get("DD_STOCK_REDU", "0") == "1" or torch.is_autocast_enabled():
        return False
    w = conv.weight
    if not (a.is_cuda and a.dtype == torch.float32 and b.dtype == torch.float32 and w.dtype == torch.float32 and a.dim() == 4 and a.shape == b.shape):
        return False
    B, Cc, H, W = a.shape
    if tuple(w.shape) != (w.shape[0], 2 * Cc, 1, 1) or conv.groups != 1 or tuple(conv.stride) != (1, 1) or tuple(conv.padding) != (0, 0):
        return False
    nhwc = (H * W * Cc, 1, W * Cc, Cc)
    if a.stride() != nhwc or b.stride() != nhwc:
        return False
    return bool(L.load().dd_redu_supported(Cc, w.shape[0]))


class ReduFn(torch.autograd.Function):

    @staticmethod
    def forward(ctx, a, b, weight, bias):
        lib = L.load()
        B, Cc, H, W = a.shape
        cout = weight.shape[0]
        y = _nhwc_empty(B, cout, H, W, a.device)
        wm = weight.reshape(cout, 2 * Cc)
        if not wm.is_contiguous():
            wm = wm.contiguous()
        L.check(lib.dd_redu_fwd(_p(a), _p(b), _p(wm), _p(bias), B * H * W, Cc, cout, _p(y), L.current_stream()), "dd_redu_fwd")
        ctx.save_for_backward(a, b, wm)
        ctx.has_bias = bias is not None
        ctx.wshape = tuple(weight.shape)
        return y

    @staticmethod
    def backward(ctx, g):
        a, b, wm = ctx.saved_tensors
        lib = L.load()
        B, Cc, H, W = a.shape
        cout = wm.shape[0]
        P = B * H * W
        g = _dense_nhwc(g.to(torch.float32))
        ga = gb = gw = gbias = None
        if ctx.needs_input_grad[0] or ctx.needs_input_grad[1]:
            ga = torch.empty_like(a) if ctx.needs_input_grad[0] else None
            gb = torch.empty_like(b) if ctx.needs_input_grad[1] else None
            L.check(lib.dd_redu_bwd_data(_p(g), _p(wm), P, Cc, cout, _p(ga), _p(gb), L.current_stream()), "dd_redu_bwd_data")
        if ctx.needs_input_grad[2] or (ctx.has_bias and ctx.needs_input_grad[3]):
            gw = torch.empty(cout, 2 * Cc, dtype=torch.float32, device=g.device)
            gbias = torch.empty(cout, dtype=torch.float32, device=g.device) if ctx.has_bias else None
            nbytes = _ws_bytes("dd_redu_workspace_bytes", P, Cc, cout)
            ws = _ws(nbytes, g.device)
            L.check(lib.dd_redu_bwd_weight(_p(a), _p(b), _p(g), P, Cc, cout, _p(gw), _p(gbias), _p(ws), nbytes, L.current_stream()), "dd_redu_bwd_weight")
            gw = gw.view(ctx.wshape)
        return ga, gb, gw, gbias


def head_conv_ok(x, weight, stride, padding, dilation, groups):
    if os.environ.get("DD_STOCK_HEAD_CONV", "0") == "1":
        return False
    if not (x.is_cuda and x.dtype == torch.float32 and weight.dtype == torch.float32 and x.dim() == 4):
        return False
    if weight.shape[0] != 1 or not _conv3x3_s1(x, weight, stride, padding, dilation, groups, ((0, 0),)):
        return False
    B, Cc, Hp, Wp = x.shape
    if Hp < 3 or Wp < 3 or torch.is_autocast_enabled() or x.stride() != (Hp * Wp * Cc, 1, Wp * Cc, Cc):
        return False
    return bool(L.load().dd_conv_head_supported(Cc))


class HeadConvFn(torch.autograd.Function):

    @staticmethod
    def forward(ctx, x, weight, bias):
        lib = L.load()
        B, Cc, Hp, Wp = x.shape
        out = torch.empty((B, 1, Hp - 2, Wp - 2), dtype=torch.float32, device=x.device)
        sw = weight.stride()
        L.check(lib.dd_conv_head_fwd(_p(x), _p(weight), sw[1], sw[2], sw[3], _p(bias), B, Hp, Wp, Cc, _p(out), L.current_stream()), "dd_conv_head_fwd")
        ctx.save_for_backward(x, weight)
        ctx.has_bias = bias is not None
        return out

    @staticmethod
    def backward(ctx, g):
        x, weight = ctx.saved_tensors
        lib = L.load()
        B, Cc, Hp, Wp = x.shape
        g = g.to(torch.float32).contiguous()
        gx = gw = gb = None
        if ctx.needs_input_grad[0]:
            gx = torch.empty_like(x)
            L.check(lib.dd_conv3x3_cout1_bwd_data(_p(g), _p(weight.contiguous()), B, Hp, Wp, Cc, 0, _p(gx), L.current_stream()), "dd_conv3x3_cout1_bwd_data")
        if ctx.needs_input_grad[1] or (ctx.has_bias and ctx.needs_input_grad[2]):
            flat = torch.empty(9 * Cc, dtype=torch.float32, device=g.device)
            gb = torch.empty(1, dtype=torch.float32, device=g.device) if ctx.has_bias else None
            nbytes = int(lib.dd_conv_head_workspace_bytes(B, Hp, Wp, Cc))
            ws = _ws(nbytes, g.device)
            L.check(lib.dd_conv_head_bwd_weight(_p(x), _p(g), B, Hp, Wp, Cc, _p(flat), _p(gb), _p(ws), nbytes, L.current_stream()), "dd_conv_head_bwd_weight")
            gw = flat.view(1, 3, 3, Cc).permute(0, 3, 1, 2)
        return gx, gw, gb


def small_conv_ok(x, weight, stride, padding, dilation, groups):
    if os.environ.get("DD_STOCK_SMALL_CONV", "0") == "1":
        return False
    if not (x.is_cuda and x.dtype == torch.float32 and weight.dtype == torch.float32 and x.dim() == 4 and weight.dim() == 4):
        return False
    cout, cin, kh, kw = weight.shape
    if kh != kw or kh not in (1, 3) or groups != 1 or tuple(stride) != (1, 1) or tuple(dilation) != (1, 1) or tuple(padding) != (kh // 2, kh // 2):
        return False
    if x.shape[1] != cin or x.shape[0] * x.shape[2] * x.shape[3] < (1 << 16):
        return False
    if torch.is_autocast_enabled():
        return False
    return bool(L.load().dd_conv_small_supported(kh, cin, cout))


def _dense_nhwc(t):
    B, Cc, H, W = t.shape
    if t.stride() == (H * W * Cc, 1, W * Cc, Cc):
        return t
    return t.contiguous(memory_format=torch.channels_last).as_strided((B, Cc, H, W), (H * W * Cc, 1, W * Cc, Cc)) if Cc > 1 else \
        t.contiguous().as_strided((B, Cc, H, W), (H * W, 1, W, 1))


_SMALL_CONV_CALLS = [0]


def small_conv_calls():
    return _SMALL_CONV_CALLS[0]


class SmallConvFn(torch.autograd.Function):

    @staticmethod
    def forward(ctx, x, weight, bias):
        lib = L.load()
        cout, cin, ks, _ = weight.shape
        B, _, H, W = x.shape
        x = _dense_nhwc(x)
        y = _nhwc_empty(B, cout, H, W, x.device)
        nbytes = _ws_bytes("dd_conv_small_workspace_bytes", ks, cin, cout)
        ws = _ws(nbytes, x.device)
        sw = weight.stride()
        L.check(lib.dd_conv_small_fwd(_p(x), _p(weight), sw[0], sw[1], sw[2], sw[3], _p(bias), B, H, W, cin, cout, ks, _p(y), _p(ws), nbytes,
                                      L.current_stream()), "dd_conv_small_fwd")
        _SMALL_CONV_CALLS[0] += 1
        ctx.save_for_backward(x, weight)
        ctx.has_bias = bias is not None
        return y

    @staticmethod
    def backward(ctx, g):
        x, weight = ctx.saved_tensors
        lib = L.load()
        cout, cin, ks, _ = weight.shape
        B, _, H, W = x.shape
        g = _dense_nhwc(g.to(torch.float32))
        nbytes = _ws_bytes("dd_conv_small_workspace_bytes", ks, cin, cout)
        gx = gw = gb = None
        if ctx.needs_input_grad[0]:
            gx = _nhwc_empty(B, cin, H, W, g.device)
            ws = _ws(nbytes, g.device)
            sw = weight.stride()
            L.check(lib.dd_conv_small_bwd_data(_p(g), _p(weight), sw[0], sw[1], sw[2], sw[3], B, H, W, cin, cout, ks, _p(gx), _p(ws), nbytes,
                                               L.current_stream()), "dd_conv_small_bwd_data")
        if ctx.needs_input_grad[1] or (ctx.has_bias and ctx.needs_input_grad[2]):
            flat = torch.empty(cout * ks * ks * cin, dtype=torch.float32, device=g.device)
            gb = torch.empty(cout, dtype=torch.float32, device=g.device) if ctx.has_bias else None
            ws = _ws(nbytes, g.device)
            L.check(lib.dd_conv_small_bwd_weight(_p(x), _p(g), B, H, W, cin, cout, ks, _p(flat), _p(gb), _p(ws), nbytes, L.current_stream()),
                    "dd_conv_small_bwd_weight")
            gw = flat.view(cout, ks, ks, cin).permute(0, 3, 1, 2)
        return gx, gw, gb


def small_conv(x, weight, bias=None):
    return SmallConvFn.apply(x, weight, bias)


def mfma_conv_ok(x, weight, stride, padding, dilation, groups):
    if os.environ.get("DD_STOCK_MFMA_CONV", "0") == "1":
        return False
    if not (x.is_cuda and x.dtype == torch.float32 and weight.dtype == torch.float32 and x.dim() == 4):
        return False
    if not _conv3x3_s1(x, weight, stride, padding, dilation, groups, ((0, 0), (1, 1))) or torch.is_autocast_enabled():
        return False
    cout, cin = weight.shape[:2]
    pad = padding[0]
    Ho, Wo = x.shape[2] + 2 * pad - 2, x.shape[3] + 2 * pad - 2
    if _below_tile_pixels(x.shape[0], Ho, Wo, "DD_MFMA_CONV_MIN_PIXELS"):
        return pad == 1 and _flat_conv_ok(x.shape[0], x.shape[2], x.shape[3], cin, cout)
    return bool(L.load().dd_conv3x3_mfma_supported(cin, cout))


def _flat_conv_ok(B, H, W, cin, cout):
    if os.environ.get("DD_FLAT_MFMA_CONV", "1") != "1" or min(cin, cout) < int(os.environ.get("DD_FLAT_MIN_CHANNELS", "256")):
        return False
    lib = L.load()
    return bool(lib.dd_conv3x3_mfma_flat_supported(B, H, W, cin, cout)) and bool(lib.dd_conv3x3_mfma_flat_supported(B, H, W, cout, cin))


def _flat_shape(B, H, W, pad, k_in=None, n_out=None):
    Ho, Wo = H + 2 * pad - 2, W + 2 * pad - 2
    if not (pad == 1 and _below_tile_pixels(B, Ho, Wo, "DD_MFMA_CONV_MIN_PIXELS")):
        return False
    if os.environ.get("DD_FLAT_MFMA_CONV", "1") != "1":
        return False
    return k_in is None or bool(L.load().dd_conv3x3_mfma_flat_supported(B, H, W, k_in, n_out))


_MFMA_CONV_CALLS = [0]
_FLAT_CONV_CALLS = [0]


def mfma_conv_calls():
    return _MFMA_CONV_CALLS[0]


_PRODUCTS = {"highest": 6, "high": 3, "medium": 1}


def mfma_products():
    env = os.environ.get("DD_MFMA_PRODUCTS")
    return int(env) if env else _PRODUCTS[torch.get_float32_matmul_precision()]


class MfmaConvFn(torch.autograd.Function):

    @staticmethod
    def forward(ctx, x, weight, bias, pad):
        lib = L.load()
        cout, cin = weight.shape[:2]
        B, _, Hi, Wi = x.shape
        x = _dense_nhwc(x)
        need_gx = ctx.needs_input_grad[0]
        stream = L.current_stream()
        products = mfma_products()
        pset = _ACTIVE_PACK_SETS[-1] if (_ACTIVE_PACK_SETS and _pack_many_on()) else None
        packs = pset.take(weight, need_gx) if pset is not None else None
        if packs is not None:
            pack_f, pack_b = packs
        else:
            pack_f = torch.empty(_ws_bytes("dd_conv3x3_mfma_pack_bytes", cout, cin) // 4, dtype=torch.float32, device=x.device)
            pack_b = torch.empty(_ws_bytes("dd_conv3x3_mfma_pack_bytes", cin, cout) // 4, dtype=torch.float32, device=x.device) if need_gx else None
            sw = weight.stride()
            L.check(lib.dd_conv3x3_mfma_pack(_p(weight), sw[0], sw[1], sw[2], sw[3], cout, cin, _p(pack_f), _p(pack_b), stream), "dd_conv3x3_mfma_pack")
            if pset is not None and isinstance(weight, torch.nn.Parameter):
                pset.join(weight, pack_f, pack_b)
        Ho, Wo = Hi + 2 * pad - 2, Wi + 2 * pad - 2
        y = _nhwc_empty(B, cout, Ho, Wo, x.device)
        if _flat_shape(B, Hi, Wi, pad, cin, cout):
            nbytes = _ws_bytes("dd_conv3x3_mfma_flat_workspace_bytes", B, Hi, Wi, cin, cout)
            ws = _ws(nbytes, x.device)
            L.check(lib.dd_conv3x3_mfma_flat_n(_p(x), _p(pack_f), _p(bias), B, Hi, Wi, cin, cout, products, _p(y), _p(ws), nbytes, stream), "dd_conv3x3_mfma_flat")
            _FLAT_CONV_CALLS[0] += 1
        else:
            L.check(lib.dd_conv3x3_mfma_n(_p(x), _p(pack_f), _p(bias), B, Hi, Wi, cin, cout, pad, products, _p(y), stream), "dd_conv3x3_mfma")
        _MFMA_CONV_CALLS[0] += 1
        ctx.save_for_backward(x, weight, pack_b)
        ctx.conf = (pad, bias is not None, products)
        return y

    @staticmethod
    def backward(ctx, g):
        x, weight, pack_b = ctx.saved_tensors
        pad, has_bias, products = ctx.conf
        lib = L.load()
        cout, cin = weight.shape[:2]
        B, _, Hi, Wi = x.shape
        Ho, Wo = g.shape[2:]
        g = _dense_nhwc(g.to(torch.float32))
        gx = gw = gb = None
        stream = L.current_stream()
        if ctx.needs_input_grad[0]:
            gx = _nhwc_empty(B, cin, Hi, Wi, g.device)
            if _flat_shape(B, Hi, Wi, pad, cout, cin):
                nbytes = _ws_bytes("dd_conv3x3_mfma_flat_workspace_bytes", B, Ho, Wo, cout, cin)
                ws = _ws(nbytes, g.device)
                L.check(lib.dd_conv3x3_mfma_flat_n(_p(g), _p(pack_b), None, B, Ho, Wo, cout, cin, products, _p(gx), _p(ws), nbytes, stream), "dd_conv3x3_mfma_flat (data gradient)")
            else:
                L.check(lib.dd_conv3x3_mfma_n(_p(g), _p(pack_b), None, B, Ho, Wo, cout, cin, 2 - pad, products, _p(gx), stream), "dd_conv3x3_mfma (data gradient)")
        if ctx.needs_input_grad[1]:
            if (cout % 4 == 0 and min(cin, cout) >= 32 and os.environ.get("DD_STOCK_MFMA_WGRAD", "0") != "1"
                    and (products < 6 or not _flat_shape(B, Hi, Wi, pad, cin, cout))):
                flat = torch.empty(cout * 9 * cin, dtype=torch.float32, device=g.device)
                nbytes = _ws_bytes("dd_conv3x3_mfma_wgrad_workspace_bytes", B, Ho, Wo, cin, cout)
                ws = _ws(nbytes, g.device)
                L.check(lib.dd_conv3x3_mfma_bwd_weight_n(_p(x), _p(g), B, Hi, Wi, cin, cout, pad, products, _p(flat), _p(ws), nbytes, stream), "dd_conv3x3_mfma_bwd_weight")
                gw = flat.view(cout, 3, 3, cin).permute(0, 3, 1, 2)
            else:
                gw = _wgrad_3x3_library(g, x, weight, pad)
        if has_bias and ctx.needs_input_grad[2]:
            gb = _channel_sum(g, B * Ho * Wo, cout, DTYPE_CODE[g.dtype], stream) if cout <= 256 else g.sum((0, 2, 3))
        return gx, gw, gb, None


def mfma_conv(x, weight, bias=None, pad=1):
    return MfmaConvFn.apply(x, weight, bias, int(pad))


_HALF_CONV_CALLS = [0]


def half_conv_calls():
    return _HALF_CONV_CALLS[0]


def half_conv_ok(x, weight, stride, padding, dilation, groups):
    if os.environ.get("DD_HALF_MFMA_CONV", "1") != "1" or not x.is_cuda or x.dim() != 4 or x.dtype not in (torch.float16, torch.bfloat16):
        return False
    if not torch.is_autocast_enabled() or torch.get_autocast_dtype("cuda") != x.dtype or weight.dtype not in (torch.float32, x.dtype):
        return False
    if not _conv3x3_s1(x, weight, stride, padding, dilation, groups, ((0, 0), (1, 1))):
        return False
    if not (x.is_contiguous(memory_format=torch.channels_last) or x.stride(1) == 1):
        return False
    cout, cin = weight.shape[:2]
    pad = padding[0]
    Ho, Wo = x.shape[2] + 2 * pad - 2, x.shape[3] + 2 * pad - 2
    if _below_tile_pixels(x.shape[0], Ho, Wo, "DD_HALF_CONV_MIN_PIXELS"):
        return False
    return bool(L.load().dd_conv3x3_half_supported(cin, cout))


class HalfConvFn(torch.autograd.Function):

    @staticmethod
    def forward(ctx, x, weight, bias, pad):
        lib = L.load()
        cout, cin = weight.shape[:2]
        B, _, Hi, Wi = x.shape
        x = _dense_nhwc(x)
        code = DTYPE_CODE[x.dtype]
        w32 = weight if weight.dtype == torch.float32 else weight.float()
        need_gx = ctx.needs_input_grad[0]
        pack_f = torch.empty(_ws_bytes("dd_conv3x3_half_pack_bytes", cout, cin) // 4, dtype=torch.float32, device=x.device)
        pack_b = torch.empty(_ws_bytes("dd_conv3x3_half_pack_bytes", cin, cout) // 4, dtype=torch.float32, device=x.device) if need_gx else None
        sw = w32.stride()
        stream = L.current_stream()
        L.check(lib.dd_conv3x3_half_pack(_p(w32), sw[0], sw[1], sw[2], sw[3], cout, cin, code, _p(pack_f), _p(pack_b), stream), "dd_conv3x3_half_pack")
        Ho, Wo = Hi + 2 * pad - 2, Wi + 2 * pad - 2
        y = _nhwc_empty(B, cout, Ho, Wo, x.device, dtype=x.dtype)
        b32 = None if bias is None else (bias if bias.dtype == torch.float32 else bias.float())
        L.check(lib.dd_conv3x3_half(_p(x), _p(pack_f), _p(b32), B, Hi, Wi, cin, cout, pad, code, _p(y), stream), "dd_conv3x3_half")
        _HALF_CONV_CALLS[0] += 1
        ctx.save_for_backward(x, weight, pack_b)
        ctx.conf = (pad, bias is not None, None if bias is None else bias.dtype)
        return y

    @staticmethod
    def backward(ctx, g):
        x, weight, pack_b = ctx.saved_tensors
        pad, has_bias, bias_dtype = ctx.conf
        lib = L.load()
        cout, cin = weight.shape[:2]
        B, _, Hi, Wi = x.shape
        Ho, Wo = g.shape[2:]
        g = _dense_nhwc(g.to(x.dtype))
        code = DTYPE_CODE[x.dtype]
        gx = gw = gb = None
        stream = L.current_stream()
        if ctx.needs_input_grad[0]:
            gx = _nhwc_empty(B, cin, Hi, Wi, g.device, dtype=x.dtype)
            L.check(lib.dd_conv3x3_half(_p(g), _p(pack_b), None, B, Ho, Wo, cout, cin, 2 - pad, code, _p(gx), stream), "dd_conv3x3_half (data gradient)")
        if ctx.needs_input_grad[1]:
            if (min(cin, cout) >= 32 and weight.dtype == torch.float32 and os.environ.get("DD_STOCK_HALF_WGRAD", "0") != "1"
                    and B * Ho * Wo >= int(os.environ.get("DD_HALF_WGRAD_MIN_PIXELS", "100000"))):
                flat = torch.empty(cout * 9 * cin, dtype=torch.float32, device=g.device)
                nbytes = _ws_bytes("dd_conv3x3_half_wgrad_workspace_bytes", B, Ho, Wo, cin, cout)
                ws = _ws(nbytes, g.device)
                L.check(lib.dd_conv3x3_half_bwd_weight(_p(x), _p(g), B, Hi, Wi, cin, cout, pad, code, _p(flat), _p(ws), nbytes, stream), "dd_conv3x3_half_bwd_weight")
                gw = flat.view(cout, 3, 3, cin).permute(0, 3, 1, 2)
            else:
                gw = _wgrad_3x3_library(g, x, torch.empty_like(weight, dtype=x.dtype), pad).to(weight.dtype)
        if has_bias and ctx.needs_input_grad[2]:
            gb = _channel_sum(g, B * Ho * Wo, cout, code, stream) if cout <= 256 else g.float().sum((0, 2, 3))
            gb = gb.to(bias_dtype)
        return gx, gw, gb, None


def half_conv(x, weight, bias=None, pad=1):
    return HalfConvFn.apply(x, weight, bias, int(pad))


class ReflectPad1NHWCFn(torch.autograd.Function):

    @staticmethod
    def forward(ctx, x):
        B, Cc, H, W = x.shape
        out = torch.empty((B, Cc, H + 2, W + 2), dtype=x.dtype, device=x.device, memory_format=torch.channels_last)
        L.check(L.load().dd_reflect_pad1_nhwc_t(_p(x), B, H, W, Cc, _p(out), DTYPE_CODE[x.dtype], L.current_stream()), "dd_reflect_pad1_nhwc_t")
        ctx.dims = (B, Cc, H, W, x.dtype)
        return out

    @staticmethod
    def backward(ctx, g):
        B, Cc, H, W, dtype = ctx.dims
        g = g.to(dtype).contiguous(memory_format=torch.channels_last)
        gx = torch.empty((B, Cc, H, W), dtype=dtype, device=g.device, memory_format=torch.channels_last)
        L.check(L.load().dd_reflect_pad1_nhwc_bwd_t(_p(g), B, H, W, Cc, _p(gx), DTYPE_CODE[dtype], L.current_stream()), "dd_reflect_pad1_nhwc_bwd_t")
        return gx


def reflect_pad1(x):
    if (x.is_cuda and x.dtype in DTYPE_CODE and x.dim() == 4 and x.shape[1] > 1 and x.shape[2] >= 4 and x.shape[3] >= 4
            and x.is_contiguous(memory_format=torch.channels_last) and not x.is_contiguous()):
        return ReflectPad1NHWCFn.apply(x)
    return torch.nn.functional.pad(x, (1, 1, 1, 1), mode="reflect")


class UpCatPadFn(torch.autograd.Function):

    @staticmethod
    def forward(ctx, x, skip, mode, elu):
        B, C1, h, w = x.shape
        C2 = 0 if skip is None else skip.shape[1]
        H, W = (h, w) if mode == 2 else (2 * h, 2 * w)
        out = torch.empty((B, C1 + C2, H + 2, W + 2), dtype=x.dtype, device=x.device, memory_format=torch.channels_last)
        L.check(L.load().dd_up_cat_pad_t(_p(x), None if skip is None else _p(skip), B, h, w, C1, C2, mode, int(elu), _p(out), DTYPE_CODE[x.dtype],
                                         L.current_stream()), "dd_up_cat_pad_t")
        ctx.save_for_backward(x)
        ctx.cfg = (C2, mode, int(elu))
        return out

    @staticmethod
    def backward(ctx, g):
        (x,) = ctx.saved_tensors
        C2, mode, elu = ctx.cfg
        B, C1, h, w = x.shape
        H, W = (h, w) if mode == 2 else (2 * h, 2 * w)
        g = g.to(x.dtype).contiguous(memory_format=torch.channels_last)
        gx = torch.empty_like(x) if ctx.needs_input_grad[0] else None
        gs = (torch.empty((B, C2, H, W), dtype=x.dtype, device=x.device, memory_format=torch.channels_last)
              if C2 and ctx.needs_input_grad[1] else None)
        if gx is not None or gs is not None:
            L.check(L.load().dd_up_cat_pad_bwd_t(_p(g), _p(x), B, h, w, C1, C2, mode, elu, None if gx is None else _p(gx), None if gs is None else _p(gs),
                                                 DTYPE_CODE[x.dtype], L.current_stream()), "dd_up_cat_pad_bwd_t")
        return gx, gs, None, None


def _nhwc(t):
    return t.is_contiguous(memory_format=torch.channels_last) and not t.is_contiguous()


def up_cat_pad_ok(x, skip, mode):
    if os.environ.get("DD_STOCK_DECODER_GLUE", "0") == "1":
        return False
    if not (x.is_cuda and x.dtype in DTYPE_CODE and x.dim() == 4 and x.shape[1] % 4 == 0 and x.shape[1] >= 4 and _nhwc(x)
            and x.shape[2] >= 2 and x.shape[3] >= 2 and (mode != 2 or (x.shape[2] >= 4 and x.shape[3] >= 4))):
        return False
    if skip is not None:
        H, W = (x.shape[2], x.shape[3]) if mode == 2 else (2 * x.shape[2], 2 * x.shape[3])
        if not (skip.dtype == x.dtype and skip.is_cuda and skip.shape[0] == x.shape[0] and skip.shape[1] % 4 == 0 and tuple(skip.shape[2:]) == (H, W)
                and _nhwc(skip)):
            return False
    return True


def up_cat_pad(x, skip=None, mode="bilinear", elu=True):
    code = {"nearest": 0, "bilinear": 1, None: 2}[mode]
    if up_cat_pad_ok(x, skip, code):
        return UpCatPadFn.apply(x, skip, code, bool(elu))
    F = torch.nn.functional
    y = F.elu(x) if elu else x
    if mode is not None:
        y = F.interpolate(y, scale_factor=2, mode=mode)
    if skip is not None:
        y = torch.cat((y, skip), 1)
    return reflect_pad1(y)


class DepthwiseConv3x3NHWCFn(torch.autograd.Function):

    @staticmethod
    def forward(ctx, x, weight, dilation):
        B, Cc, H, W = x.shape
        w = weight.contiguous()
        out = torch.empty((B, Cc, H, W), dtype=x.dtype, device=x.device, memory_format=torch.channels_last)
        L.check(L.load().dd_dwconv3x3_nhwc_t(_p(x), _p(w), B, H, W, Cc, dilation, _p(out), DTYPE_CODE[x.dtype], L.current_stream()), "dd_dwconv3x3_nhwc_t")
        ctx.save_for_backward(x, w)
        ctx.dilation = dilation
        return out

    @staticmethod
    def backward(ctx, g):
        x, w = ctx.saved_tensors
        B, Cc, H, W = x.shape
        g = g.to(x.dtype).contiguous(memory_format=torch.channels_last)
        lib, gx, gw = L.load(), None, None
        code = DTYPE_CODE[x.dtype]
        if ctx.needs_input_grad[0]:
            gx = torch.empty((B, Cc, H, W), dtype=x.dtype, device=g.device, memory_format=torch.channels_last)
            L.check(lib.dd_dwconv3x3_nhwc_bwd_data_t(_p(g), _p(w), B, H, W, Cc, ctx.dilation, _p(gx), code, L.current_stream()), "dd_dwconv3x3_nhwc_bwd_data_t")
        if ctx.needs_input_grad[1]:
            gw = torch.empty_like(w)
            nbytes = _ws_bytes("dd_dwconv3x3_workspace_bytes", B, H, Cc)
            ws = _ws(nbytes, g.device)
            L.check(lib.dd_dwconv3x3_nhwc_bwd_weight_t(_p(g), _p(x), B, H, W, Cc, ctx.dilation, _p(gw), _p(ws), nbytes, code, L.current_stream()),
                    "dd_dwconv3x3_nhwc_bwd_weight_t")
        return gx, gw, None


def depthwise_conv3x3(x, weight, dilation):
    Cc = x.shape[1]
    if (x.is_cuda and x.dtype in DTYPE_CODE and weight.dtype == torch.float32 and x.dim() == 4 and Cc % 4 == 0 and Cc <= 512
            and x.is_contiguous(memory_format=torch.channels_last) and not x.is_contiguous()):
        return DepthwiseConv3x3NHWCFn.apply(x, weight, dilation)
    return torch.nn.functional.conv2d(x, weight, None, 1, dilation, dilation, Cc)


class PointwiseLinearFn(torch.autograd.Function):

    @staticmethod
    def forward(ctx, x, weight, bias):
        B, H, W, cin = x.shape
        ctx.save_for_backward(x, weight)
        with torch.autocast("cuda", enabled=False):
            return torch.addmm(bias, x.reshape(-1, cin), weight.t()).view(B, H, W, weight.shape[0])

    @staticmethod
    def backward(ctx, g):
        x, weight = ctx.saved_tensors
        B, H, W, cin = x.shape
        cout = weight.shape[0]
        g = g.to(x.dtype).contiguous()
        gx = gw = gb = None
        if ctx.needs_input_grad[0]:
            gx = torch.mm(g.view(-1, cout), weight).view(B, H, W, cin)
        gw, gb = _linear_param_grads(g, x, weight, B, H, W, ctx.needs_input_grad[1], ctx.needs_input_grad[2], L.current_stream())
        if gb is not None:
            gb = gb.to(weight.dtype)
        return gx, gw, gb


def pointwise_linear(x, layer):
    if (x.is_cuda and x.dtype in DTYPE_CODE and layer.weight.dtype == torch.float32 and layer.bias is not None and x.dim() == 4
            and x.is_contiguous() and torch.is_grad_enabled() and layer.out_features <= 4096):
        if torch.is_autocast_enabled():
            dt = torch.get_autocast_dtype("cuda")
            return PointwiseLinearFn.apply(x.to(dt), layer.weight.to(dt), layer.bias.to(dt))
        if x.dtype == torch.float32:
            return PointwiseLinearFn.apply(x, layer.weight, layer.bias)
    return layer(x.reshape(-1, x.shape[-1])).view(*x.shape[:-1], layer.out_features)


_MLP_CALLS = [0]


def mlp_calls():
    return _MLP_CALLS[0]


def mlp_ok(y, block):
    if os.environ.get("DD_MLP", "0") != "1" or os.environ.get("DD_STOCK_MLP", "0") == "1" or torch.is_autocast_enabled():
        return False
    l1, l2 = block.pwconv1, block.pwconv2
    if y.dim() != 4 or y.shape[0] * y.shape[1] * y.shape[2] < int(os.environ.get("DD_MLP_MIN_ROWS", "16384")):
        return False
    return bool(y.is_cuda and y.dtype == torch.float32 and y.dim() == 4 and y.is_contiguous() and l1.weight.dtype == torch.float32
                and l1.bias is not None and l2.bias is not None and l1.in_features % 32 == 0 and l1.out_features % 32 == 0
                and l2.in_features == l1.out_features and l2.out_features == l1.in_features and y.shape[-1] == l1.in_features
                and isinstance(block.act, torch.nn.GELU) and getattr(block.act, "approximate", "none") == "none")


def _mlp_param_grads(needs, g, gpre, y, post, w1, w2, B, H, W, stream):
    gw1, gb1 = _linear_param_grads(gpre, y, w1, B, H, W, needs[1], needs[2], stream)
    gw2, gb2 = _linear_param_grads(g, post, w2, B, H, W, needs[3], needs[4], stream)
    return gw1, gb1, gw2, gb2


class MlpFn(torch.autograd.Function):

    @staticmethod
    def forward(ctx, y, w1, b1, w2, b2):
        lib = L.load()
        B, H, W, Cc = y.shape
        hid, M = w1.shape[0], B * H * W
        need = any(ctx.needs_input_grad)
        nb1, nb2 = _ws_bytes("dd_pw_gemm_pack_bytes", hid, Cc), _ws_bytes("dd_pw_gemm_pack_bytes", Cc, hid)
        packs = torch.empty(((nb1 + nb2) * (2 if need else 1)) // 4, dtype=torch.float32, device=y.device)
        p0 = packs.data_ptr()
        stream = L.current_stream()
        L.check(lib.dd_mlp_pack(_p(w1), w1.stride(0), w1.stride(1), _p(w2), w2.stride(0), w2.stride(1), Cc, hid, p0, p0 + nb1,
                                p0 + nb1 + nb2 if need else None, p0 + 2 * nb1 + nb2 if need else None, None, stream), "dd_mlp_pack")
        pre = torch.empty((M, hid), dtype=torch.float32, device=y.device)
        L.check(lib.dd_pw_gemm(_p(y), p0, _p(b1), M, Cc, hid, 0, _p(pre), stream), "dd_pw_gemm (pwconv1)")
        out = torch.empty((B, H, W, Cc), dtype=torch.float32, device=y.device)
        L.check(lib.dd_pw_gemm(_p(pre), p0 + nb1, _p(b2), M, hid, Cc, 1, _p(out), stream), "dd_pw_gemm (GELU, pwconv2)")
        _MLP_CALLS[0] += 1
        if need:
            ctx.save_for_backward(y, pre, w1, w2, packs)
        return out

    @staticmethod
    def backward(ctx, g):
        y, pre, w1, w2, packs = ctx.saved_tensors
        lib = L.load()
        B, H, W, Cc = y.shape
        hid, M = w1.shape[0], B * H * W
        nb1, nb2 = _ws_bytes("dd_pw_gemm_pack_bytes", hid, Cc), _ws_bytes("dd_pw_gemm_pack_bytes", Cc, hid)
        p0 = packs.data_ptr()
        stream = L.current_stream()
        g = g.to(torch.float32).contiguous()
        gpre = torch.empty((M, hid), dtype=torch.float32, device=g.device)
        L.check(lib.dd_pw_gemm(_p(g), p0 + nb1 + nb2, None, M, Cc, hid, 0, _p(gpre), stream), "dd_pw_gemm (g . w2)")
        post = torch.empty((M, hid), dtype=torch.float32, device=g.device)
        L.check(lib.dd_gelu_pair(_p(pre), _p(gpre), _p(post), M * hid, stream), "dd_gelu_pair")
        gy = None
        if ctx.needs_input_grad[0]:
            gy = torch.empty((B, H, W, Cc), dtype=torch.float32, device=g.device)
            L.check(lib.dd_pw_gemm(_p(gpre), p0 + 2 * nb1 + nb2, None, M, hid, Cc, 0, _p(gy), stream), "dd_pw_gemm (g_pre . w1)")
        return (gy,) + _mlp_param_grads(ctx.needs_input_grad, g, gpre, y, post, w1, w2, B, H, W, stream)


def mlp(y, block):
    return MlpFn.apply(y, block.pwconv1.weight, block.pwconv1.bias, block.pwconv2.weight, block.pwconv2.bias)


_MLP_FUSED_CALLS = [0]


def mlp_fused_calls():
    return _MLP_FUSED_CALLS[0]

# ... 265 lines not shown
```

### dynamo-depth_amd/networks/layers.py

```python
import os

import torch
import torch.nn as nn
import torch.nn.functional as F


def rot_from_axisangle(vec):
    angle = vec.norm(dim=2, keepdim=True)
    axis = vec / (angle + 1e-7)
    c, s = torch.cos(angle), torch.sin(angle)
    t = 1 - c
    x, y, z = axis.unbind(-1)
    c, s, t = c.squeeze(-1), s.squeeze(-1), t.squeeze(-1)
    row0 = torch.cat([x * x * t + c, x * y * t - z * s, z * x * t + y * s], 1)
    row1 = torch.cat([x * y * t + z * s, y * y * t + c, y * z * t - x * s], 1)
    row2 = torch.cat([z * x * t - y * s, y * z * t + x * s, z * z * t + c], 1)
    rot = torch.zeros(vec.shape[0], 4, 4, dtype=vec.dtype, device=vec.device)
    rot[:, 0, :3], rot[:, 1, :3], rot[:, 2, :3] = row0, row1, row2
    rot[:, 3, 3] = 1
    return rot


def get_translation_matrix(translation_vector):
    B = translation_vector.shape[0]
    T = torch.eye(4, dtype=translation_vector.dtype, device=translation_vector.device).repeat(B, 1, 1)
    T[:, :3, 3] = translation_vector.reshape(B, 3)
    return T


def transformation_from_parameters(axisangle, translation, invert=False):
    if axisangle.is_cuda:
        from hipops.functions import PoseMatrixFn
        return PoseMatrixFn.apply(axisangle.float(), translation.float(), bool(invert))
    R = rot_from_axisangle(axisangle)
    if invert:
        return torch.matmul(R.transpose(1, 2), get_translation_matrix(-translation))
    return torch.matmul(get_translation_matrix(translation), R)


def _hip_conv(x, weight, bias, stride, padding, dilation, groups):
    if not x.is_cuda:
        return None
    from hipops.functions import ConvBiasFn, HeadConvFn, half_conv, half_conv_ok, head_conv_ok, mfma_conv, mfma_conv_ok, small_conv, small_conv_ok
    conf = (stride, padding, dilation, groups)
    if x.dtype != torch.float32 and half_conv_ok(x, weight, *conf):
        return half_conv(x, weight, bias, padding[0])
    if small_conv_ok(x, weight, *conf):
        return small_conv(x, weight, bias)
    if mfma_conv_ok(x, weight, *conf):
        return mfma_conv(x, weight, bias, padding[0])
    if head_conv_ok(x, weight, *conf):
        return HeadConvFn.apply(x, weight, bias)
    if bias is not None and torch.is_grad_enabled() and os.environ.get("DD_STOCK_CONV_BIAS_GRAD", "0") != "1":
        return ConvBiasFn.apply(x, weight, bias, *conf)
    return None


class Conv2d(nn.Conv2d):

    def forward(self, x):
        if self.padding_mode == "zeros":
            y = _hip_conv(x, self.weight, self.bias, self.stride, self.padding, self.dilation, self.groups)
            if y is not None:
                return y
        return super().forward(x)


_ZERO_CHANNELS = {}


def stock_slices(which):
    v = os.environ.get("DD_STOCK_SLICES", "0")
    return v == "1" or which in v.split(",")


def _as_channels_last(t):
    if t.shape[1] == 1:
        B, _, H, W = t.shape
        return t.contiguous().as_strided(t.shape, (H * W, 1, W, 1))
    return t.contiguous(memory_format=torch.channels_last)


def conv_cat_aligned(conv, parts, force=False):
    total = sum(p.shape[1] for p in parts)
    pad = (-total) % 8
    x0 = parts[0]
    if (pad == 0 or not (x0.is_cuda or force) or conv.groups != 1 or conv.padding_mode != "zeros" or total < 32
            or os.environ.get("DD_STOCK_CAT_CONV", "0") == "1"):
        if x0.is_cuda and total <= 16 and isinstance(conv, Conv2d) and os.environ.get("DD_STOCK_SMALL_CONV", "0") != "1":
            parts = [_as_channels_last(p) for p in parts]
        return conv(torch.cat(list(parts), 1))
    big = max(parts, key=lambda p: p.shape[1])
    nhwc = big.is_contiguous(memory_format=torch.channels_last) and not big.is_contiguous()
    key = (x0.shape[0], pad, x0.shape[2], x0.shape[3], x0.dtype, str(x0.device), nhwc)
    zeros = _ZERO_CHANNELS.get(key)
    if zeros is None:
        zeros = torch.zeros((x0.shape[0], pad, x0.shape[2], x0.shape[3]), dtype=x0.dtype, device=x0.device)
        if key[-1]:
            zeros = zeros.contiguous(memory_format=torch.channels_last)
        _ZERO_CHANNELS[key] = zeros
    if key[-1]:
        parts = [_as_channels_last(p) for p in parts]
    x = torch.cat(list(parts) + [zeros], 1)
    w = F.pad(conv.weight, (0, 0, 0, 0, 0, pad))
    y = _hip_conv(x, w, conv.bias, conv.stride, conv.padding, conv.dilation, conv.groups)
    return y if y is not None else F.conv2d(x, w, conv.bias, conv.stride, conv.padding, conv.dilation, conv.groups)


class DeferredStats:

    def __init__(self, device, floats):
        self.buf = torch.zeros(floats, dtype=torch.float32, device=device)
        self.used = 0
        self.pairs = []

    def take(self, bn):
        C = bn.num_features
        if self.used + 2 * C > self.buf.numel():
            raise RuntimeError("DeferredStats scratch too small")
        mean, var = self.buf[self.used:self.used + C], self.buf[self.used + C:self.used + 2 * C]
        self.used += 2 * C
        self.pairs.append((bn, mean, var))
        return mean, var

    def apply(self):
        if not torch.cuda.is_current_stream_capturing():
            self.buf.record_stream(torch.cuda.current_stream())
        groups = {}
        for bn, mean, var in self.pairs:
            g = groups.setdefault(float(bn.momentum), ([], []))
            g[0].extend((bn.running_mean, bn.running_var))
            g[1].extend((mean, var))
        for momentum, (running, terms) in groups.items():
            running = [r.data for r in running]
            torch._foreach_mul_(running, 1.0 - momentum)
            torch._foreach_add_(running, terms)


_DEFER = None
_GROUPS = 1


class batch_groups:

    def __init__(self, groups, collectors=None):
        self.groups, self.collectors = int(groups), collectors

    def __enter__(self):
        global _GROUPS, _DEFER
        self.prev = (_GROUPS, _DEFER)
        _GROUPS = self.groups
        if self.collectors is not None:
            _DEFER = list(self.collectors)
        return self

    def __exit__(self, *exc):
        global _GROUPS, _DEFER
        _GROUPS, _DEFER = self.prev


class defer_running_stats:
    def __init__(self, collector):
        self.collector = collector

    def __enter__(self):
        global _DEFER
        self.prev, _DEFER = _DEFER, self.collector
        return self.collector

    def __exit__(self, *exc):
        global _DEFER
        _DEFER = self.prev


class BatchNorm2d(nn.BatchNorm2d):

    def __init__(self, *args, **kwargs):
        super().__init__(*args, **kwargs)
        self._pending_batches = 0

    def forward(self, x, act=None, residual=None):
        if self.training and self.track_running_stats and self.momentum is not None and _GROUPS > 1:
            assert x.shape[0] % _GROUPS == 0
            self._check_input_dim(x)
            self.__dict__["_pending_batches"] += _GROUPS
            per = x.shape[0] // _GROUPS
            bufs = [(self.running_mean, self.running_var) if _DEFER is None else _DEFER[gi].take(self) for gi in range(_GROUPS)]
            if self._hip_path(x, act, residual):
                from hipops.functions import batch_norm_act
                return batch_norm_act(x, self, act, residual, running=bufs, groups=_GROUPS)
            y = torch.cat([F.batch_norm(x[gi * per:(gi + 1) * per], bufs[gi][0], bufs[gi][1], self.weight, self.bias, True, self.momentum, self.eps)
                           for gi in range(_GROUPS)])
        elif self.training and self.track_running_stats and self.momentum is not None:
            self._check_input_dim(x)
            self.__dict__["_pending_batches"] += 1
            rm, rv = (self.running_mean, self.running_var) if _DEFER is None else _DEFER.take(self)
            if self._hip_path(x, act, residual):
                from hipops.functions import batch_norm_act
                return batch_norm_act(x, self, act, residual, running=(rm, rv))
            y = F.batch_norm(x, rm, rv, self.weight, self.bias, True, self.momentum, self.eps)
        else:
            y = super().forward(x)
        if residual is not None:
            y = y + residual
        if act == "relu":
            return F.relu(y)
        if act == "gelu":
            return F.gelu(y)
        assert act is None, act
        return y

    def _hip_path(self, x, act, residual):
        Cc = x.shape[1]
        ok = (x.is_cuda and x.dtype in (torch.float32, torch.float16, torch.bfloat16) and self.affine and self.weight.dtype == torch.float32
              and x.dim() == 4 and Cc % 4 == 0 and Cc <= 512
              and x.is_contiguous(memory_format=torch.channels_last) and not x.is_contiguous()
              and not (act == "gelu" and residual is not None) and os.environ.get("DD_STOCK_BATCHNORM", "0") != "1")
        if ok and residual is not None:
            ok = (residual.shape == x.shape and residual.dtype == x.dtype
                  and residual.is_contiguous(memory_format=torch.channels_last))
        return ok

    def flush_counter(self):
        if self._pending_batches and self.num_batches_tracked is not None:
            self.num_batches_tracked += self._pending_batches
        self._pending_batches = 0

    def _save_to_state_dict(self, destination, prefix, keep_vars):
        self.flush_counter()
        super()._save_to_state_dict(destination, prefix, keep_vars)

    def _load_from_state_dict(self, *args, **kwargs):
        self._pending_batches = 0
        super()._load_from_state_dict(*args, **kwargs)


class Conv3x3(nn.Module):

    def __init__(self, in_channels, out_channels, use_refl=True):
        super().__init__()
        self.use_refl = bool(use_refl)
        self.pad = nn.ReflectionPad2d(1) if use_refl else nn.ZeroPad2d(1)
        self.conv = Conv2d(int(in_channels), int(out_channels), 3)

    def forward(self, x):
        if self.use_refl and x.is_cuda and os.environ.get("DD_STOCK_REFLECT_PAD", "0") != "1":
            from hipops.functions import reflect_pad1
            return self.conv(reflect_pad1(x))
        return self.conv(self.pad(x))


class ConvBlock(nn.Module):

    def __init__(self, in_channels, out_channels):
        super().__init__()
        self.conv = Conv3x3(in_channels, out_channels)
# ... 9 lines not shown
```

### dynamo-depth_amd/networks/motion_decoder.py

```python
import os

import torch
import torch.nn as nn

from .layers import Conv2d, conv_cat_aligned, stock_slices
import torch.nn.functional as F


def redu_split(redu, a, b, C):
    from hipops.functions import ConvBiasFn, ReduFn, SplitChannelsFn, redu_ok
    if redu_ok(a, b, redu):
        return ReduFn.apply(a, b, redu.weight, redu.bias)
    w = redu.weight
    if not stock_slices("redu"):
        wa, wb = SplitChannelsFn.apply(w, C)
    else:
        wa, wb = w[:, :C].contiguous(), w[:, C:].contiguous()
    from hipops.functions import small_conv, small_conv_ok
    if small_conv_ok(a, wa, redu.stride, redu.padding, redu.dilation, 1) and small_conv_ok(b, wb, redu.stride, redu.padding, redu.dilation, 1):
        return small_conv(a, wa, redu.bias) + small_conv(b, wb, None)
    ya = ConvBiasFn.apply(a, wa, redu.bias, redu.stride, redu.padding, redu.dilation, 1)
    return ya + F.conv2d(b, wb, None, redu.stride, redu.padding, redu.dilation, 1)


class MotionDecoder(nn.Module):
    def __init__(self, num_inp_feat, scales=4, num_input_images=2, inp_disp=True, out_dim=4):
        super().__init__()
        self.org_in_ch = num_input_images * (3 + int(inp_disp))
        self.num_inp_feat = [int(c) for c in num_inp_feat[::-1]] + [self.org_in_ch]
        self.out_dim = out_dim
        self.scales = scales
        assert max(self.scales) < len(self.num_inp_feat)
        self._residual_translation = Conv2d(6, out_dim, kernel_size=1)
        for level, ch in enumerate(self.num_inp_feat):
            setattr(self, "refine_motion_conv{}".format(level), nn.Sequential(
                Conv2d(ch + out_dim, ch, kernel_size=3, padding=1), Conv2d(ch, ch, kernel_size=3, padding=1)))
            setattr(self, "refine_motion_redu{}".format(level), Conv2d(2 * ch, out_dim, kernel_size=1))

    def forward(self, pose_feat, ego_motion):
        amp = ego_motion.is_cuda and torch.is_autocast_enabled()
        if amp:
            with torch.autocast("cuda", enabled=False):
                field = self._residual_translation(100 * ego_motion.float())
        else:
            field = self._residual_translation(100 * ego_motion)
        per_level = []
        for level in range(len(self.num_inp_feat)):
            feat = pose_feat[-1 - level]
            up = F.interpolate(field, size=feat.shape[-2:], mode="bilinear", align_corners=False)
            convs = getattr(self, "refine_motion_conv{}".format(level))
            a = conv_cat_aligned(convs[0], (up.to(feat.dtype) if amp else up, feat))
            b = convs[1](a)
            redu = getattr(self, "refine_motion_redu{}".format(level))
            if a.is_cuda and os.environ.get("DD_STOCK_REDU_CAT", "0") != "1":
                C = a.shape[1]
                field = redu_split(redu, a, b, C)
            else:
                field = redu(torch.cat((a, b), 1))
            field = (field.float() if amp else field) + up
            per_level.append(field)
        outputs = {}
        for scale in self.scales:
            raw = 0.01 * per_level[len(self.num_inp_feat) - 1 - scale]
            if self.out_dim == 1:
                outputs[("motion_prob", scale)] = raw
                outputs[("motion_mask", scale)] = torch.sigmoid(raw)
            elif self.out_dim == 3:
                outputs[("complete_flow", scale)] = raw
            else:
                raise Exception("out_dim={} not excepted.".format(self.out_dim))
        return outputs
```

### include/dynamo_hip.h

```cpp
#ifndef DYNAMO_HIP_H_
#define DYNAMO_HIP_H_

#include <stddef.h>
#include <stdint.h>

#ifdef __cplusplus
extern "C" {
#endif

#define DD_MAX_SCALES 4
#define DD_NUM_SRC 2
#define DD_ABI_VERSION 2

#define DD_MODE_RIGID 0
#define DD_MODE_FLOW 1
#define DD_MODE_FLOW_MASK 2

#define DD_PARTIAL_STRIDE 40
#define DD_SUMS_STRIDE 8

typedef struct DDPhotoScale {
  int shift;
  int h, w;
  float w_photo;
// ... 75 lines not shown

#define DD_REG_SMOOTH 5
#define DD_REG_RES_STRIDE 16
typedef struct DDRegSmooth {
  const float* inp;
  float* g_inp;
  int C;
  int normalise;
  float weight;
} DDRegSmooth;
typedef struct DDRegScale {
  int h, w;
  const float* img;
  DDRegSmooth smooth[DD_REG_SMOOTH];
  const float* delta[DD_NUM_SRC];
  const float* delta_sum[DD_NUM_SRC];
  const float* prob[DD_NUM_SRC];
  float* g_prob[DD_NUM_SRC];
  float w_sparsity[DD_NUM_SRC];
  const float* disp;
  float* g_disp;
  const float* inv_K;
  const int32_t* rand_idx;
  float* plane;
  float w_ground;
} DDRegScale;
typedef struct DDRegArgs {
  int abi_version;
  int B, num_scales;
  int np_per_it, max_it;
  float tol, g_prior, min_depth, max_depth;
  float* res;
  float* workspace;
  DDRegScale scale[DD_MAX_SCALES];
} DDRegArgs;
size_t dd_reg_workspace_bytes(const DDRegArgs* args);
int dd_reg_losses_finish(const DDRegArgs* args, const DDAssembleArgs* assemble, float* loss, float* out, void* stream);

int dd_fused_loss(const DDPhotoArgs* photo, const DDRegArgs* reg, const DDAssembleArgs* assemble, float* loss, float* out, void* stream);
int dd_fused_loss_part(const DDPhotoArgs* photo, const DDRegArgs* reg, const DDAssembleArgs* assemble, float* loss, float* out, void* stream,
                       int part);
int dd_fused_loss_supported(const DDPhotoArgs* photo, const DDRegArgs* reg);

typedef struct DDJpegHeader {
  int32_t data_offset;
  int32_t data_end;
  int32_t width, height;
  int32_t restart_interval;
  int32_t ncomp;
  int32_t h[3], v[3], tq[3], td[3], ta[3];
  int32_t reserved[3];
  uint16_t qt[4][64];
  uint8_t bits[4][16];
  uint8_t vals[4][256];
} DDJpegHeader;
size_t dd_jpeg_workspace_bytes(int n_images, int H, int W, int ncomp, const int* h, const int* v);
int dd_jpeg_decode(const unsigned char* data, long long stride, const DDJpegHeader* headers, int n_images, int H, int W, int ncomp, const int* h,
                   const int* v, unsigned char* rgb, void* workspace, size_t workspace_bytes, void* stream);

size_t dd_resize_workspace_bytes(int n_images, int Hs, int Ws, int H, int W);
int dd_resize_bicubic(const unsigned char* src, int n_images, int Hs, int Ws, unsigned char* dst, const int32_t* dst_slot, int H, int W,
                      const int32_t* h_bounds, const int32_t* h_coef, int h_ksize, const int32_t* v_bounds, const int32_t* v_coef, int v_ksize,
                      void* workspace, size_t workspace_bytes, void* stream);


int dd_backproject(const float* depth, const float* inv_K, int B, int h, int w, float* points, void* stream);
int dd_backproject_bwd(const float* g_points, const float* inv_K, int B, int h, int w, float* g_depth, void* stream);

int dd_project3d(const float* points, const float* K, const float* T, int B, int h, int w, float eps,
                 float* pix, float* ego, void* stream);
int dd_project3d_bwd(const float* points, const float* K, const float* T, const float* g_pix, const float* g_ego,
                     int B, int h, int w, float eps, float* g_points, float* g_T, float* workspace, void* stream);
size_t dd_project3d_workspace_bytes(int B, int h, int w);

int dd_ssim(const float* x, const float* y, int B, int C, int H, int W, float* out, void* stream);
int dd_ssim_bwd(const float* x, const float* y, const float* g_out, int B, int C, int H, int W,
                float* g_x, float* g_y, void* stream);

int dd_disp_to_depth(const float* disp, size_t n, float min_depth, float max_depth, float* scaled, float* depth,
                     void* stream);

int dd_pose_matrix(const float* axisangle, const float* translation, int B, int invert, float* T, void* stream);
int dd_pose_matrix_bwd(const float* axisangle, const float* translation, const float* g_T, int B, int invert,
                       float* g_axisangle, float* g_translation, void* stream);

int dd_channel_sum_nhwc(const float* x, long long rows, int C, float* out, float* workspace, void* stream);
size_t dd_channel_sum_workspace_bytes(int C);

int dd_reflect_pad1_nhwc(const float* x, int B, int H, int W, int C, float* out, void* stream);
int dd_reflect_pad1_nhwc_bwd(const float* g_out, int B, int H, int W, int C, float* g_x, void* stream);

int dd_dwconv3x3_nhwc(const float* x, const float* weight, int B, int H, int W, int C, int dilation, float* out, void* stream);
int dd_dwconv3x3_nhwc_bwd_data(const float* g_out, const float* weight, int B, int H, int W, int C, int dilation, float* g_x, void* stream);
int dd_dwconv3x3_nhwc_bwd_weight(const float* g_out, const float* x, int B, int H, int W, int C, int dilation, float* g_weight,
                                 void* workspace, size_t workspace_bytes, void* stream);
size_t dd_dwconv3x3_workspace_bytes(int B, int H, int C);

int dd_conv3x3_cout1_bwd_data(const float* g_out, const float* weight, int B, int Hi, int Wi, int C, int padding, float* g_x, void* stream);

int dd_prepare_frames(const uint8_t* frames_u8, const float* params, const int32_t* flip, int B, int F, int H, int W, float* color,
                      float* color_aug, float* workspace, void* stream);
size_t dd_prepare_frames_workspace_bytes(int B, int F);
int dd_pyramid_down2(const float* src, int planes, int H, int W, float* dst, void* stream);
int dd_pack_rgb(const float* planar, int B, int H, int W, float* packed, void* stream);

int dd_depth_metrics(const float* disp, int B, int H, int W, const float* lidar, const float* valid, int M, const int* gt_dim,
                     const double* img_bound, float min_depth, float max_depth, float* per_sample, float* mean,
                     void* workspace, size_t workspace_bytes, void* stream);
size_t dd_depth_metrics_workspace_bytes(int B, int M);
int dd_depth_metrics_masked(const float* disp, int B, int H, int W, const float* lidar, const float* valid, int M, const int* gt_dim,
                            const double* img_bound, float min_depth, float max_depth, const uint8_t* mask, int mask_h, int mask_w,
                            float* per_sample, float* mean, float* per_label, void* workspace, size_t workspace_bytes, void* stream);
size_t dd_depth_metrics_masked_workspace_bytes(int B, int M);
int dd_depth_metrics_accumulate(const float* per_sample, const float* per_label, int B, double* totals, double* label_totals, void* stream);

int dd_odom_snippet_count(int N, int track_length);
int dd_odom_snippets(const float* pred, const double* gt_global, int N, int track_length, double* ate, double* speed, void* stream);

int dd_motion_pr(const float* pred, int B, int h, int w, const uint8_t* mot, const uint8_t* sem, int H, int W,
                 const float* thresholds, int T, int num_sem, unsigned long long* counts, void* stream);

int dd_fill_contours(const int16_t* vertices, int v_cap, const int32_t* contours, int c_cap, int B, int H, int W, uint8_t* mask,
                     void* stream);

size_t dd_lidar_depth_points_workspace_bytes(int S, int C, int H, int W);
int dd_lidar_depth_points(const float* points, long long n_total, const int32_t* offsets, int S, const double* P, int C, int H, int W,
                          int32_t* counts, double* rows, float* maps, void* workspace, size_t workspace_bytes, void* stream);

int dd_bn_act_fwd(const float* x, const float* residual, long long rows, int C, const float* gamma, const float* beta, float eps,
                  float momentum, float* running_mean, float* running_var, float* save_mean, float* save_invstd, int act,
                  float* out, void* workspace, size_t workspace_bytes, void* stream);
int dd_bn_act_bwd(const float* x, const float* g_out, const float* out, long long rows, int C, const float* gamma, const float* beta,
                  const float* save_mean, const float* save_invstd, int act, float* g_x, float* g_residual, float* g_gamma,
                  float* g_beta, void* workspace, size_t workspace_bytes, void* stream);
size_t dd_bn_workspace_bytes(int C);

#define DD_DTYPE_F32 0
#define DD_DTYPE_F16 1
#define DD_DTYPE_BF16 2
int dd_bn_act_fwd_t(const void* x, const void* residual, long long rows, int C, const float* gamma, const float* beta, float eps, float momentum,
                    float* running_mean, float* running_var, float* save_mean, float* save_invstd, int act, void* out, int dtype,
                    void* workspace, size_t workspace_bytes, void* stream);
int dd_bn_act_bwd_t(const void* x, const void* g_out, const void* out, long long rows, int C, const float* gamma, const float* beta,
                    const float* save_mean, const float* save_invstd, int act, void* g_x, void* g_residual, float* g_gamma, float* g_beta,
                    int dtype, void* workspace, size_t workspace_bytes, void* stream);
int dd_channel_sum_nhwc_t(const void* x, long long rows, int C, float* out, int dtype, float* workspace, void* stream);
int dd_reflect_pad1_nhwc_t(const void* x, int B, int H, int W, int C, void* out, int dtype, void* stream);
int dd_reflect_pad1_nhwc_bwd_t(const void* g_out, int B, int H, int W, int C, void* g_x, int dtype, void* stream);

int dd_up_cat_pad_t(const void* x, const void* skip, int B, int h, int w, int C1, int C2, int mode, int elu, void* out, int dtype, void* stream);
int dd_up_cat_pad_bwd_t(const void* g_out, const void* x, int B, int h, int w, int C1, int C2, int mode, int elu, void* g_x, void* g_skip,
                        int dtype, void* stream);

int dd_layer_norm_fwd(const float* x, long long rows, int C, const float* gamma, const float* beta, float eps, float* y, float* mean,
                      float* rstd, void* stream);
int dd_layer_norm_bwd(const float* x, const float* g_out, const float* gamma, const float* mean, const float* rstd, long long rows, int C,
                      float* g_x, float* g_gamma_beta, void* workspace, size_t workspace_bytes, void* stream);
size_t dd_layer_norm_workspace_bytes(int C);

int dd_layer_scale_bwd(const float* g_out, const float* y, const float* scale, int B, int rows, int C, float* g_y, float* g_scale,
                       void* workspace, size_t workspace_bytes, void* stream);
size_t dd_layer_scale_workspace_bytes(int B, int C);

int dd_layer_norm_fwd_t(const void* x, long long rows, int C, const float* gamma, const float* beta, float eps, void* y, float* mean, float* rstd,
                        int dtype, void* stream);
int dd_layer_norm_bwd_t(const void* x, const void* g_out, const float* gamma, const float* mean, const float* rstd, long long rows, int C,
                        void* g_x, float* g_gamma_beta, void* workspace, size_t workspace_bytes, int dtype, void* stream);
int dd_layer_scale_bwd_t(const void* g_out, const void* y, const float* scale, int B, int rows, int C, void* g_y, float* g_scale, void* workspace,
                         size_t workspace_bytes, int dtype, void* stream);
int dd_layer_scale_fwd_t(const void* res, const void* y, const float* scale, int B, int rows, int C, void* out, int dtype, void* stream);
int dd_dwconv3x3_nhwc_t(const void* x, const float* weight, int B, int H, int W, int C, int dilation, void* out, int dtype, void* stream);
int dd_dwconv3x3_nhwc_bwd_data_t(const void* g_out, const float* weight, int B, int H, int W, int C, int dilation, void* g_x, int dtype, void* stream);
int dd_dwconv3x3_nhwc_bwd_weight_t(const void* g_out, const void* x, int B, int H, int W, int C, int dilation, float* g_weight, void* workspace,
                                   size_t workspace_bytes, int dtype, void* stream);

int dd_redu_supported(int C, int cout);
size_t dd_redu_workspace_bytes(long long P, int C, int cout);
int dd_redu_fwd(const float* a, const float* b, const float* weight, const float* bias, long long P, int C, int cout, float* y, void* stream);
int dd_redu_bwd_data(const float* g_out, const float* weight, long long P, int C, int cout, float* g_a, float* g_b, void* stream);
int dd_redu_bwd_weight(const float* a, const float* b, const float* g_out, long long P, int C, int cout, float* g_weight, float* g_bias, void* workspace,
                       size_t workspace_bytes, void* stream);

int dd_conv_head_supported(int C);
size_t dd_conv_head_workspace_bytes(int B, int Hp, int Wp, int C);
int dd_conv_head_fwd(const float* x_padded, const float* weight, long long s_ci, long long s_kh, long long s_kw, const float* bias, int B, int Hp, int Wp,
                     int C, float* out, void* stream);
int dd_conv_head_bwd_weight(const float* x_padded, const float* g_out, int B, int Hp, int Wp, int C, float* g_weight, float* g_bias, void* workspace,
                            size_t workspace_bytes, void* stream);

int dd_conv_small_supported(int ks, int cin, int cout);
size_t dd_conv_small_workspace_bytes(int ks, int cin, int cout);
int dd_conv_small_fwd(const float* x, const float* weight, long long s_co, long long s_ci, long long s_kh, long long s_kw, const float* bias, int B, int H,
                      int W, int cin, int cout, int ks, float* y, void* workspace, size_t workspace_bytes, void* stream);
int dd_conv_small_bwd_data(const float* g_out, const float* weight, long long s_co, long long s_ci, long long s_kh, long long s_kw, int B, int H, int W, int cin,
                           int cout, int ks, float* g_x, void* workspace, size_t workspace_bytes, void* stream);
int dd_conv_small_bwd_weight(const float* x, const float* g_out, int B, int H, int W, int cin, int cout, int ks, float* g_weight, float* g_bias,
                             void* workspace, size_t workspace_bytes, void* stream);

int dd_conv3x3_mfma_supported(int cin, int cout);
size_t dd_conv3x3_mfma_pack_bytes(int n_out, int k_in);
int dd_conv3x3_mfma_pack(const float* weight, long long s_co, long long s_ci, long long s_kh, long long s_kw, int cout, int cin, void* pack_fwd,
                         void* pack_bwd_data, void* stream);
int dd_conv3x3_mfma_n(const float* x, const void* pack, const float* bias, int B, int Hi, int Wi, int k_in, int n_out, int pad, int products, float* y,
                      void* stream);
int dd_conv3x3_mfma_pack_many_job_words(void);
int dd_conv3x3_mfma_pack_many_blocks(int cout, int cin, int want_fwd, int want_bwd_data);
int dd_conv3x3_mfma_pack_many(const long long* jobs, const int* block_job, int n_blocks, void* stream);
int dd_conv3x3_mfma(const float* x, const void* pack, const float* bias, int B, int Hi, int Wi, int k_in, int n_out, int pad, float* y, void* stream);
int dd_conv3x3_mfma_flat_supported(int B, int H, int W, int k_in, int n_out);
size_t dd_conv3x3_mfma_flat_workspace_bytes(int B, int H, int W, int k_in, int n_out);
int dd_conv3x3_mfma_flat(const float* x, const void* pack, const float* bias, int B, int H, int W, int k_in, int n_out, float* y, void* workspace,
                         size_t workspace_bytes, void* stream);
int dd_conv3x3_mfma_flat_n(const float* x, const void* pack, const float* bias, int B, int H, int W, int k_in, int n_out, int products, float* y,
                           void* workspace, size_t workspace_bytes, void* stream);
size_t dd_conv3x3_mfma_wgrad_workspace_bytes(int B, int Ho, int Wo, int cin, int cout);
int dd_conv3x3_mfma_bwd_weight(const float* x, const float* g_out, int B, int Hi, int Wi, int cin, int cout, int pad, float* g_weight, void* workspace,
                               size_t workspace_bytes, void* stream);
int dd_conv3x3_mfma_bwd_weight_n(const float* x, const float* g_out, int B, int Hi, int Wi, int cin, int cout, int pad, int products, float* g_weight,
                                 void* workspace, size_t workspace_bytes, void* stream);

int dd_conv3x3_half_supported(int cin, int cout);
size_t dd_conv3x3_half_pack_bytes(int n_out, int k_in);
int dd_conv3x3_half_pack(const float* weight, long long s_co, long long s_ci, long long s_kh, long long s_kw, int cout, int cin, int dtype,
                         void* pack_fwd, void* pack_bwd_data, void* stream);
int dd_conv3x3_half(const void* x, const void* pack, const float* bias, int B, int Hi, int Wi, int k_in, int n_out, int pad, int dtype, void* y,
                    void* stream);
size_t dd_conv3x3_half_wgrad_workspace_bytes(int B, int Ho, int Wo, int cin, int cout);
int dd_conv3x3_half_bwd_weight(const void* x, const void* g_out, int B, int Hi, int Wi, int cin, int cout, int pad, int dtype, float* g_weight,
                               void* workspace, size_t workspace_bytes, void* stream);

size_t dd_pw_gemm_pack_bytes(int N, int K);
int dd_mlp_pack(const float* w1, long long s1_n, long long s1_k, const float* w2, long long s2_n, long long s2_k, int C, int hidden, void* pack_fwd1,
                void* pack_fwd2, void* pack_bwd2, void* pack_bwd1, void* pack_fwd2_fused, void* stream);
int dd_mlp_fwd_supported(int C);
int dd_mlp_fwd(const float* x, const void* pack_fwd1, const void* pack_fwd2_fused, const float* b1, const float* b2, int M, int C, float* y, void* stream);
int dd_pw_gemm(const float* x, const void* pack, const float* bias, int M, int K, int N, int gelu_in, float* y, void* stream);
int dd_gelu_pair(const float* pre, float* g_inout, float* post, size_t n, void* stream);

int dd_linear_wgrad_supported(int M, int cout, int cin);
size_t dd_linear_wgrad_workspace_bytes(int M, int cout, int cin);
int dd_linear_wgrad(const float* g_out, const float* x, int M, int cout, int cin, float* g_weight, float* g_bias, void* workspace, size_t workspace_bytes,
                    void* stream);
int dd_linear_wgrad_n(const float* g_out, const float* x, int M, int cout, int cin, int products, float* g_weight, float* g_bias, void* workspace,
                      size_t workspace_bytes, void* stream);

typedef struct DDAdamRecord {
  float* param;
  const float* grad;
  float* exp_avg;
  float* exp_avg_sq;
  float* step;
  long long n;
} DDAdamRecord;
int dd_adam_chunk(void);
int dd_adam_multi(const DDAdamRecord* records, int n_records, const int* block_map, int n_blocks, void* aux, double lr, double beta1, double beta2,
                  double eps, double weight_decay, const float* grad_scale, const float* found_inf, void* stream);

#define DD_VIS_MAX_TILES 16
#define DD_VIS_IMG 0
#define DD_VIS_REF_IMG 1
#define DD_VIS_DISP 2
#define DD_VIS_MASK 3
#define DD_VIS_EGO_FLOW 4
#define DD_VIS_IND_FLOW 5
#define DD_VIS_COMP_FLOW 6
#define DD_VIS_SAMP_FLOW 7
int dd_vis_frame(const float* color, const float* ref_color, const float* disp, const float* motion_mask, const float* complete_flow, const float* K,
                 const float* inv_K, const float* cam_T_cam, float min_depth, float max_depth, int H, int W, const int* tiles, int n_tiles, int R, int C,
                 const uint32_t* lut, float disp_vmin, float disp_vmax, float mask_vmin, float mask_vmax, int frame, int max_frames, uint8_t* panel,
                 float* side, float* maxima, void* stream);
int dd_vis_flow_tiles(const float* side, const float* maxima, const int* tiles, int n_tiles, int R, int C, int H, int W, int n_frames,
                      float flow_mag_factor, int consistent_flow, uint8_t* panel, void* stream);

int dd_export_depth(const float* disp, const float* disp_flipped, const float* l_mask, int B, int h, int w, int H, int W, float min_depth,
                    float max_depth, float depth_scale, const uint32_t* lut, float vmin, float vmax, float* depth, uint16_t* depth16, uint8_t* rgb,
                    void* stream);
int dd_export_plane_u8(const float* plane, int B, int h, int w, int H, int W, uint8_t* out, void* stream);

const char* dd_error_string(int code);
int dd_abi_version(void);

#ifdef __cplusplus
}
#endif
#endif
```

Before: 353.8.

## Fuse motion-decoder upsample/concat glue and bias-gradient into conv weight-gradient kernels

Adds a fused kernel that bilinearly upsamples the motion field and concatenates it with features into an aligned, padded NHWC buffer. A matching backward kernel is added, and the motion decoder uses this fused path in place of interpolate plus cat. The residual add is folded into the redu kernel. The conv weight-gradient kernel also gains a templated mode that accumulates the bias gradient from staged output-gradient tiles in LDS and reduces it in the same fold launch, avoiding a separate bias reduction pass. This costs extra LDS per block and more code paths.

```diff
diff --git a/dynamo-depth_amd/csrc/dd_conv_mfma.hip b/dynamo-depth_amd/csrc/dd_conv_mfma.hip
--- a/dynamo-depth_amd/csrc/dd_conv_mfma.hip
+++ b/dynamo-depth_amd/csrc/dd_conv_mfma.hip
@@ -464,11 +464,13 @@
 constexpr int XITEMS = XR * (XC / 2) * 16;
 constexpr int XJ = (XITEMS + NT - 1) / NT;
 constexpr int BLOCK = 64 * 9 * 64;
-}
-
-template <int NP>
+constexpr int LDS_BIAS = LDS + NT * 16;
+}
+
+template <int NP, bool BIAS = false>
 __global__ __launch_bounds__(NT, 2) void conv_wgrad_kernel(const float* __restrict__ x, const float* __restrict__ g, int B, int Hi, int Wi, int Ho, int Wo,
-                                                           int cin, int cout, int pad, int tiles_x, int tiles_y, float* __restrict__ partial) {
+                                                           int cin, int cout, int pad, int tiles_x, int tiles_y, float* __restrict__ partial,
+                                                           float* __restrict__ bias_part) {
   using namespace wg;
   extern __shared__ __align__(16) unsigned char smem[];
   unsigned char* const s_g = smem;
@@ -551,10 +553,17 @@
                       __builtin_amdgcn_alignbit(w1, w0.w, 16));
   };
 
+  float4* const s_bias = reinterpret_cast<float4*>(smem + LDS) + tid;
+  if (BIAS && blockIdx.y == 0) *s_bias = make_float4(0.f, 0.f, 0.f, 0.f);
   if (t_begin < t_end) fetch(t_begin);
   for (int t = t_begin; t < t_end; ++t) {
     __syncthreads();
     stage();
+    if (BIAS && blockIdx.y == 0) {
+      float4 bsum = *s_bias;
+      bsum.x += pg[0].x + pg[1].x; bsum.y += pg[0].y + pg[1].y; bsum.z += pg[0].z + pg[1].z; bsum.w += pg[0].w + pg[1].w;
+      *s_bias = bsum;
+    }
     __syncthreads();
     if (t + 1 < t_end) fetch(t + 1);
 #pragma unroll
@@ -619,6 +628,15 @@
     }
   }
 
+  if (BIAS && blockIdx.y == 0) {
+    float4 bsum = *s_bias;
+#pragma unroll
+    for (int m = 1; m < 16; m <<= 1) {
+      bsum.x += __shfl_xor(bsum.x, m, 64); bsum.y += __shfl_xor(bsum.y, m, 64); bsum.z += __shfl_xor(bsum.z, m, 64); bsum.w += __shfl_xor(bsum.w, m, 64);
+    }
+    if ((tid & 15) == 0) *reinterpret_cast<float4*>(bias_part + ((size_t)blockIdx.z * nks + ks) * 64 + 4 * gq) = bsum;
+  }
+
   float* P = partial + (((size_t)blockIdx.z * gridDim.y + blockIdx.y) * nks + ks) * BLOCK;
   auto put_acc = [&](const f16v& A, int g, int tx, int m) {
     const int nb = g / 3, tap = (g % 3) * 3 + tx;
@@ -641,26 +659,37 @@
   }
 }
 
-__global__ __launch_bounds__(256) void conv_wgrad_fold_kernel(const float* __restrict__ partial, int nks, int cin, int cout, int ci_groups, float* __restrict__ gw) {
+__global__ __launch_bounds__(256) void conv_wgrad_fold_kernel(const float* __restrict__ partial, int nks, int cin, int cout, int ci_groups, float* __restrict__ gw,
+                                                              const float* __restrict__ bias_part, float* __restrict__ gb) {
   __shared__ float red[4][64];
   const int lane = threadIdx.x & 63, wave = threadIdx.x >> 6;
-  const int idx = blockIdx.x * 64 + lane;
-  const bool in = idx < cout * 9 * cin;
+  const int w_blocks = (cout * 9 * cin + 63) / 64;
+  const bool bias = (int)blockIdx.x >= w_blocks;
+  const int idx = bias ? ((int)blockIdx.x - w_blocks) * 64 + lane : blockIdx.x * 64 + lane;
+  const bool in = idx < (bias ? cout : cout * 9 * cin);
   float s[8] = {0.f, 0.f, 0.f, 0.f, 0.f, 0.f, 0.f, 0.f};
   if (in) {
-    const int ci = idx % cin, tap = (idx / cin) % 9, co = idx / (9 * cin);
-    const int z = co >> 6, y = ci >> 6;
-    const float* P = partial + ((size_t)z * ci_groups + y) * nks * wg::BLOCK + ((co & 63) * 9 + tap) * 64 + (ci & 63);
+    const float* P;
+    size_t step;
+    if (bias) {
+      P = bias_part + (size_t)(idx >> 6) * nks * 64 + (idx & 63);
+      step = 64;
+    } else {
+      const int ci = idx % cin, tap = (idx / cin) % 9, co = idx / (9 * cin);
+      const int z = co >> 6, y = ci >> 6;
+      P = partial + ((size_t)z * ci_groups + y) * nks * wg::BLOCK + ((co & 63) * 9 + tap) * 64 + (ci & 63);
+      step = wg::BLOCK;
+    }
     int k = wave;
     for (; k + 28 < nks; k += 32) {
 #pragma unroll
-      for (int j = 0; j < 8; ++j) s[j] += P[(size_t)(k + 4 * j) * wg::BLOCK];
-    }
-    for (; k < nks; k += 4) s[0] += P[(size_t)k * wg::BLOCK];
+      for (int j = 0; j < 8; ++j) s[j] += P[(size_t)(k + 4 * j) * step];
+    }
+    for (; k < nks; k += 4) s[0] += P[(size_t)k * step];
   }
   red[wave][lane] = ((s[0] + s[1]) + (s[2] + s[3])) + ((s[4] + s[5]) + (s[6] + s[7]));
   __syncthreads();
-  if (wave == 0 && in) gw[idx] = (red[0][lane] + red[1][lane]) + (red[2][lane] + red[3][lane]);
+  if (wave == 0 && in) (bias ? gb : gw)[idx] = (red[0][lane] + red[1][lane]) + (red[2][lane] + red[3][lane]);
 }
 
 static int wgrad_splits(int B, int Ho, int Wo, int cin, int cout) {
@@ -769,6 +798,47 @@
   return groups * dd::cm::wgrad_splits(B, Ho, Wo, cin, cout) * dd::cm::wg::BLOCK * sizeof(float);
 }
 
+static int wgrad_bias_splits(int B, int Ho, int Wo, int cin, int cout, int splits) {
+  if (splits <= 0) return dd::cm::wgrad_splits(B, Ho, Wo, cin, cout);
+  const long long tiles = (long long)B * ((Ho + dd::cm::wg::TR - 1) / dd::cm::wg::TR) * ((Wo + dd::cm::wg::TC - 1) / dd::cm::wg::TC);
+  return (int)(splits < tiles ? splits : tiles);
+}
+
+extern "C" size_t dd_conv3x3_mfma_wgrad_bias_workspace_bytes(int B, int Ho, int Wo, int cin, int cout, int splits) {
+  const size_t ci_groups = (size_t)((cin + 63) / 64), co_groups = (size_t)((cout + 63) / 64);
+  return (ci_groups * dd::cm::wg::BLOCK + 64) * co_groups * wgrad_bias_splits(B, Ho, Wo, cin, cout, splits) * sizeof(float);
+}
+
+extern "C" int dd_conv3x3_mfma_bwd_weight_bias_n(const float* x, const float* g_out, int B, int Hi, int Wi, int cin, int cout, int pad, int products, int splits,
+                                                 float* g_weight, float* g_bias, void* workspace, size_t workspace_bytes, void* stream) {
+  using namespace dd::cm;
+  if (!x || !g_out || !g_weight || !g_bias || !workspace || B < 1 || pad < 0 || pad > 1 || cin % 4 || cout % 4 || cin < 4 || cout < 4 || splits < 0)
+    return (int)hipErrorInvalidValue;
+  if (products != 6 && products != 3 && products != 1) return (int)hipErrorInvalidValue;
+  const int Ho = Hi + 2 * pad - 2, Wo = Wi + 2 * pad - 2;
+  if (Ho < 1 || Wo < 1 || workspace_bytes < dd_conv3x3_mfma_wgrad_bias_workspace_bytes(B, Ho, Wo, cin, cout, splits)) return (int)hipErrorInvalidValue;
+  if ((size_t)B * Hi * Wi * cin >= (1ull << 31) || (size_t)B * Ho * Wo * cout >= (1ull << 31)) return (int)hipErrorInvalidValue;
+  if ((reinterpret_cast<unsigned long long>(x) | reinterpret_cast<unsigned long long>(g_out) | reinterpret_cast<unsigned long long>(workspace)) & 15ull)
+    return (int)hipErrorInvalidValue;
+  hipStream_t s = static_cast<hipStream_t>(stream);
+  const int tiles_x = (Wo + wg::TC - 1) / wg::TC, tiles_y = (Ho + wg::TR - 1) / wg::TR;
+  const int nks = wgrad_bias_splits(B, Ho, Wo, cin, cout, splits), ci_groups = (cin + 63) / 64, co_groups = (cout + 63) / 64;
+  const dim3 grid(nks, ci_groups, co_groups);
+  float* part = static_cast<float*>(workspace);
+  float* bias_part = part + (size_t)ci_groups * co_groups * nks * wg::BLOCK;
+  if (products == 6)
+    hipLaunchKernelGGL((conv_wgrad_kernel<6, true>), grid, dim3(NT), wg::LDS_BIAS, s, x, g_out, B, Hi, Wi, Ho, Wo, cin, cout, pad, tiles_x, tiles_y, part, bias_part);
+  else if (products == 3)
+    hipLaunchKernelGGL((conv_wgrad_kernel<3, true>), grid, dim3(NT), wg::LDS_BIAS, s, x, g_out, B, Hi, Wi, Ho, Wo, cin, cout, pad, tiles_x, tiles_y, part, bias_part);
+  else
+    hipLaunchKernelGGL((conv_wgrad_kernel<1, true>), grid, dim3(NT), wg::LDS_BIAS, s, x, g_out, B, Hi, Wi, Ho, Wo, cin, cout, pad, tiles_x, tiles_y, part, bias_part);
+  hipError_t e = hipGetLastError();
+  if (e != hipSuccess) return (int)e;
+  hipLaunchKernelGGL(conv_wgrad_fold_kernel, dim3((cout * 9 * cin + 63) / 64 + co_groups), dim3(256), 0, s, part, nks, cin, cout, ci_groups, g_weight, bias_part,
+                     g_bias);
+  return (int)hipGetLastError();
+}
+
 extern "C" int dd_conv3x3_mfma_bwd_weight_n(const float* x, const float* g_out, int B, int Hi, int Wi, int cin, int cout, int pad, int products, float* g_weight,
                                             void* workspace, size_t workspace_bytes, void* stream) {
   using namespace dd::cm;
@@ -784,15 +854,18 @@
   const dim3 grid(nks, ci_groups, co_groups);
   float* part = static_cast<float*>(workspace);
   if (products == 6)
-    hipLaunchKernelGGL(conv_wgrad_kernel<6>, grid, dim3(NT), wg::LDS, s, x, g_out, B, Hi, Wi, Ho, Wo, cin, cout, pad, tiles_x, tiles_y, part);
+    hipLaunchKernelGGL((conv_wgrad_kernel<6, false>), grid, dim3(NT), wg::LDS, s, x, g_out, B, Hi, Wi, Ho, Wo, cin, cout, pad, tiles_x, tiles_y, part,
+                       static_cast<float*>(nullptr));
   else if (products == 3)
-    hipLaunchKernelGGL(conv_wgrad_kernel<3>, grid, dim3(NT), wg::LDS, s, x, g_out, B, Hi, Wi, Ho, Wo, cin, cout, pad, tiles_x, tiles_y, part);
+    hipLaunchKernelGGL((conv_wgrad_kernel<3, false>), grid, dim3(NT), wg::LDS, s, x, g_out, B, Hi, Wi, Ho, Wo, cin, cout, pad, tiles_x, tiles_y, part,
+                       static_cast<float*>(nullptr));
   else
-    hipLaunchKernelGGL(conv_wgrad_kernel<1>, grid, dim3(NT), wg::LDS, s, x, g_out, B, Hi, Wi, Ho, Wo, cin, cout, pad, tiles_x, tiles_y, part);
+    hipLaunchKernelGGL((conv_wgrad_kernel<1, false>), grid, dim3(NT), wg::LDS, s, x, g_out, B, Hi, Wi, Ho, Wo, cin, cout, pad, tiles_x, tiles_y, part,
+                       static_cast<float*>(nullptr));
   hipError_t e = hipGetLastError();
   if (e != hipSuccess) return (int)e;
   hipLaunchKernelGGL(conv_wgrad_fold_kernel, dim3((cout * 9 * cin + 63) / 64), dim3(256), 0, s, static_cast<const float*>(workspace), nks, cin, cout, ci_groups,
-                     g_weight);
+                     g_weight, static_cast<const float*>(nullptr), static_cast<float*>(nullptr));
   return (int)hipGetLastError();
 }
 
diff --git a/dynamo-depth_amd/csrc/dd_decoder.hip b/dynamo-depth_amd/csrc/dd_decoder.hip
--- a/dynamo-depth_amd/csrc/dd_decoder.hip
+++ b/dynamo-depth_amd/csrc/dd_decoder.hip
@@ -1,5 +1,6 @@
 #include <hip/hip_runtime.h>
 
+#include "dd_bilinear.h"
 #include "dd_half.h"
 #include "dd_math.h"
 
@@ -166,9 +167,220 @@
     hipLaunchKernelGGL(up_cat_pad_bwd_skip_kernel<T>, dim3((W * C2q + DEC_NT - 1) / DEC_NT, H, B), dim3(DEC_NT), 0, s, g, H, W, C1q, C2q, gs);
 }
 
+constexpr int UCA_MAX_CF = 4;
+
+struct UcaGeom {
+  int B, cf, C, Ct, h, w, H, W;
+  float sy, sx;
+};
+
+template <typename T>
+__device__ __forceinline__ float uca_elem(const UcaGeom& q, const float* __restrict__ field, const T* __restrict__ feat, long long fb, long long fc,
+                                          long long fh, long long fw, float* __restrict__ up, int b, int Y, int X, int c, int y0, int y1, float ly, int x0,
+                                          int x1, float lx) {
+  if (c < q.cf) {
+    const long long r0 = ((long long)b * q.h + y0) * q.w, r1 = ((long long)b * q.h + y1) * q.w;
+    const float v = dm_blend(ly, lx, field[(r0 + x0) * q.cf + c], field[(r0 + x1) * q.cf + c], field[(r1 + x0) * q.cf + c], field[(r1 + x1) * q.cf + c]);
+    up[(((long long)b * q.H + Y) * q.W + X) * q.cf + c] = v;
+    return v;
+  }
+  if (c < q.cf + q.C) return IO<T>::load1(feat, b * fb + (c - q.cf) * fc + Y * fh + X * fw);
+  return 0.f;
+}
+
+__device__ __forceinline__ float4 uca_shift(const float4& a, const float4& b, int r) {
+  if (r == 0) return a;
+  if (r == 1) return make_float4(a.y, a.z, a.w, b.x);
+  if (r == 2) return make_float4(a.z, a.w, b.x, b.y);
+  return make_float4(a.w, b.x, b.y, b.z);
+}
+
+template <typename T>
+__global__ __launch_bounds__(DEC_NT) void up_cat_align_quad_kernel(UcaGeom q, const float* __restrict__ field, const T* __restrict__ feat, long long fb,
+                                                                   long long fh, long long fw, T* __restrict__ out, float* __restrict__ up) {
+  const int Cv = q.Ct >> 2, Cq = q.C >> 2;
+  const long long total = (long long)q.B * q.H * q.W * Cv;
+  const long long i = (long long)blockIdx.x * DEC_NT + threadIdx.x;
+  if (i >= total) return;
+  const int cv = (int)(i % Cv);
+  const long long p = i / Cv;
+  const int X = (int)(p % q.W), Y = (int)((p / q.W) % q.H), b = (int)(p / ((long long)q.W * q.H));
+  const int r = (4 - (q.cf & 3)) & 3, lo = cv - ((q.cf + 3) >> 2);
+  const long long base4 = (b * fb + Y * fh + X * fw) >> 2;
+  const float4 zero = make_float4(0.f, 0.f, 0.f, 0.f);
+  const float4 a = (lo >= 0 && lo < Cq) ? IO<T>::load4(feat, base4 + lo) : zero;
+  const float4 bb = (r != 0 && lo + 1 >= 0 && lo + 1 < Cq) ? IO<T>::load4(feat, base4 + lo + 1) : zero;
+  float4 v = uca_shift(a, bb, r);
+  if (4 * cv < q.cf) {
+    int y0, y1, x0, x1;
+    float ly, lx;
+    dm_tap(Y, q.sy, q.h, y0, y1, ly);
+    dm_tap(X, q.sx, q.w, x0, x1, lx);
+    const int c = 4 * cv;
+    if (c < q.cf) v.x = uca_elem<T>(q, field, feat, 0, 0, 0, 0, up, b, Y, X, c, y0, y1, ly, x0, x1, lx);
+    if (c + 1 < q.cf) v.y = uca_elem<T>(q, field, feat, 0, 0, 0, 0, up, b, Y, X, c + 1, y0, y1, ly, x0, x1, lx);
+    if (c + 2 < q.cf) v.z = uca_elem<T>(q, field, feat, 0, 0, 0, 0, up, b, Y, X, c + 2, y0, y1, ly, x0, x1, lx);
+    if (c + 3 < q.cf) v.w = uca_elem<T>(q, field, feat, 0, 0, 0, 0, up, b, Y, X, c + 3, y0, y1, ly, x0, x1, lx);
+  }
+  IO<T>::store4(out, i, v);
+}
+
+template <typename T, int VEC>
+__global__ __launch_bounds__(DEC_NT) void up_cat_align_kernel(UcaGeom q, const float* __restrict__ field, const T* __restrict__ feat, long long fb, long long fc,
+                                                              long long fh, long long fw, T* __restrict__ out, float* __restrict__ up) {
+  const int Cv = q.Ct / VEC;
+  const long long total = (long long)q.B * q.H * q.W * Cv;
+  const long long i = (long long)blockIdx.x * DEC_NT + threadIdx.x;
+  if (i >= total) return;
+  const int cv = (int)(i % Cv);
+  const long long p = i / Cv;
+  const int X = (int)(p % q.W), Y = (int)((p / q.W) % q.H), b = (int)(p / ((long long)q.W * q.H));
+  int y0 = 0, y1 = 0, x0 = 0, x1 = 0;
+  float ly = 0.f, lx = 0.f;
+  if (cv * VEC < q.cf) {
+    dm_tap(Y, q.sy, q.h, y0, y1, ly);
+    dm_tap(X, q.sx, q.w, x0, x1, lx);
+  }
+  if (VEC == 4) {
+    float4 v;
+    v.x = uca_elem<T>(q, field, feat, fb, fc, fh, fw, up, b, Y, X, 4 * cv, y0, y1, ly, x0, x1, lx);
+    v.y = uca_elem<T>(q, field, feat, fb, fc, fh, fw, up, b, Y, X, 4 * cv + 1, y0, y1, ly, x0, x1, lx);
+    v.z = uca_elem<T>(q, field, feat, fb, fc, fh, fw, up, b, Y, X, 4 * cv + 2, y0, y1, ly, x0, x1, lx);
+    v.w = uca_elem<T>(q, field, feat, fb, fc, fh, fw, up, b, Y, X, 4 * cv + 3, y0, y1, ly, x0, x1, lx);
+    IO<T>::store4(out, i, v);
+  } else {
+    IO<T>::store1(out, i, uca_elem<T>(q, field, feat, fb, fc, fh, fw, up, b, Y, X, cv, y0, y1, ly, x0, x1, lx));
+  }
+}
+
+constexpr int UCA_GRP = 16;
+
+__device__ __forceinline__ void uca_range(int i, float scale, int out_size, int& lo, int& hi) {
+  const float a = ((float)i - 0.5f) / scale - 0.5f, b = ((float)i + 1.5f) / scale - 0.5f;
+  lo = a < 1.f ? 0 : (a > (float)out_size ? out_size : (int)a - 1);
+  hi = b > (float)(out_size - 3) ? out_size - 1 : (int)b + 2;
+  if (i == 0) lo = 0;
+}
+__device__ __forceinline__ float uca_weight(int d, float scale, int in_size, int i) {
+  int i0, i1;
+  float l1;
+  dm_tap(d, scale, in_size, i0, i1, l1);
+  return (i0 == i ? 1.f - l1 : 0.f) + (i1 == i ? l1 : 0.f);
+}
+
+template <typename T, bool QUAD>
+__global__ __launch_bounds__(DEC_NT) void up_cat_align_bwd_kernel(UcaGeom q, const T* __restrict__ g, const float* __restrict__ g_up, int feat_blocks,
+                                                                  long long n_feat, long long n_field, T* __restrict__ g_feat, float* __restrict__ g_field) {
+  if ((int)blockIdx.x < feat_blocks) {
+    const long long i = (long long)blockIdx.x * DEC_NT + threadIdx.x;
+    if (i >= n_feat) return;
+    if (QUAD) {
+      const int Cq = q.C >> 2, Cv = q.Ct >> 2;
+      const long long p = i / Cq;
+      const int cq = (int)(i - p * Cq), r = q.cf & 3, lo = cq + (q.cf >> 2);
+      const float4 a = IO<T>::load4(g, p * Cv + lo);
+      const float4 bb = r != 0 ? IO<T>::load4(g, p * Cv + lo + 1) : a;
+      IO<T>::store4(g_feat, i, uca_shift(a, bb, r));
+    } else {
+      const long long p = i / q.C;
+      IO<T>::store1(g_feat, i, IO<T>::load1(g, p * q.Ct + q.cf + (int)(i - p * q.C)));
+    }
+    return;
+  }
+  const long long k = ((long long)((int)blockIdx.x - feat_blocks) * DEC_NT + threadIdx.x) / UCA_GRP;
+  const int l = threadIdx.x % UCA_GRP;
+  if (k >= n_field) return;
+  const int xi = (int)(k % q.w), yi = (int)((k / q.w) % q.h), b = (int)(k / ((long long)q.w * q.h));
+  int ylo, yhi, xlo, xhi;
+  uca_range(yi, q.sy, q.H, ylo, yhi);
+  uca_range(xi, q.sx, q.W, xlo, xhi);
+  const int nx = xhi - xlo + 1, n = (yhi - ylo + 1) * nx;
+  float acc[UCA_MAX_CF] = {0.f, 0.f, 0.f, 0.f};
+  for (int t = l; t < n; t += UCA_GRP) {
+    const int Y = ylo + t / nx, X = xlo + t % nx;
+    const float wgt = uca_weight(Y, q.sy, q.h, yi) * uca_weight(X, q.sx, q.w, xi);
+    if (wgt == 0.f) continue;
+    const long long at = ((long long)b * q.H + Y) * q.W + X;
+#pragma unroll
+    for (int c = 0; c < UCA_MAX_CF; ++c)
+      if (c < q.cf) {
+        float v = IO<T>::load1(g, at * q.Ct + c);
+        if (g_up) v += g_up[at * q.cf + c];
+        acc[c] += wgt * v;
+      }
+  }
+#pragma unroll
+  for (int c = 0; c < UCA_MAX_CF; ++c) {
+#pragma unroll
+    for (int m = 1; m < UCA_GRP; m <<= 1) acc[c] += __shfl_xor(acc[c], m, 64);
+    if (l == 0 && c < q.cf) g_field[k * q.cf + c] = acc[c];
+  }
+}
+
+static inline bool uca_quads(const UcaGeom& q, const void* p, long long sb, long long sc, long long sh, long long sw) {
+  return q.C % 4 == 0 && q.Ct % 4 == 0 && sc == 1 && sb % 4 == 0 && sh % 4 == 0 && sw % 4 == 0 && (reinterpret_cast<unsigned long long>(p) & 15ull) == 0;
+}
+
+template <typename T>
+static void up_cat_align_launch(const UcaGeom& q, const float* field, const void* feat, long long fb, long long fc, long long fh, long long fw, void* out,
+                                float* up, hipStream_t s) {
+  const long long px = (long long)q.B * q.H * q.W;
+  if (uca_quads(q, feat, fb, fc, fh, fw))
+    hipLaunchKernelGGL((up_cat_align_quad_kernel<T>), dim3((unsigned)((px * (q.Ct / 4) + DEC_NT - 1) / DEC_NT)), dim3(DEC_NT), 0, s, q, field,
+                       static_cast<const T*>(feat), fb, fh, fw, static_cast<T*>(out), up);
+  else if (q.Ct % 4 == 0)
+    hipLaunchKernelGGL((up_cat_align_kernel<T, 4>), dim3((unsigned)((px * (q.Ct / 4) + DEC_NT - 1) / DEC_NT)), dim3(DEC_NT), 0, s, q, field,
+                       static_cast<const T*>(feat), fb, fc, fh, fw, static_cast<T*>(out), up);
+  else
+    hipLaunchKernelGGL((up_cat_align_kernel<T, 1>), dim3((unsigned)((px * q.Ct + DEC_NT - 1) / DEC_NT)), dim3(DEC_NT), 0, s, q, field,
+                       static_cast<const T*>(feat), fb, fc, fh, fw, static_cast<T*>(out), up);
+}
+
+template <typename T>
+static void up_cat_align_bwd_launch(const UcaGeom& q, const void* g, const float* g_up, void* g_feat, float* g_field, hipStream_t s) {
+  const bool quad = g_feat && q.C % 4 == 0 && q.Ct % 4 == 0 &&
+                    ((reinterpret_cast<unsigned long long>(g) | reinterpret_cast<unsigned long long>(g_feat)) & 15ull) == 0;
+  const long long n_feat = g_feat ? (long long)q.B * q.H * q.W * (quad ? q.C / 4 : q.C) : 0, n_field = g_field ? (long long)q.B * q.h * q.w : 0;
+  const int feat_blocks = (int)((n_feat + DEC_NT - 1) / DEC_NT);
+  const dim3 grid((unsigned)(feat_blocks + (n_field * UCA_GRP + DEC_NT - 1) / DEC_NT));
+  if (quad)
+    hipLaunchKernelGGL((up_cat_align_bwd_kernel<T, true>), grid, dim3(DEC_NT), 0, s, q, static_cast<const T*>(g), g_up, feat_blocks, n_feat, n_field,
+                       static_cast<T*>(g_feat), g_field);
+  else
+    hipLaunchKernelGGL((up_cat_align_bwd_kernel<T, false>), grid, dim3(DEC_NT), 0, s, q, static_cast<const T*>(g), g_up, feat_blocks, n_feat, n_field,
+                       static_cast<T*>(g_feat), g_field);
+}
+
 }
 
 using namespace dd;
+
+static bool up_cat_align_geom(int B, int cf, int C, int pad, int h, int w, int H, int W, int dtype, UcaGeom& q) {
+  if (B < 1 || cf < 1 || cf > UCA_MAX_CF || C < 1 || pad < 0 || h < 1 || w < 1 || H < 1 || W < 1 || dtype < 0 || dtype > 2) return false;
+  const long long Ct = (long long)cf + C + pad;
+  if (Ct > (1 << 20) || Ct * B * H * W >= (1ll << 38)) return false;
+  q.B = B; q.cf = cf; q.C = C; q.Ct = (int)Ct; q.h = h; q.w = w; q.H = H; q.W = W;
+  q.sy = (float)h / (float)H;
+  q.sx = (float)w / (float)W;
+  return true;
+}
+
+extern "C" int dd_up_cat_align_t(const float* field, const void* feat, long long feat_sb, long long feat_sc, long long feat_sh, long long feat_sw, int B, int cf,
+                                 int C, int pad, int h, int w, int H, int W, void* out, float* up, int dtype, void* stream) {
+  UcaGeom q;
+  if (!field || !feat || !out || !up || !up_cat_align_geom(B, cf, C, pad, h, w, H, W, dtype, q)) return (int)hipErrorInvalidValue;
+  if (q.Ct % 4 == 0 && (reinterpret_cast<unsigned long long>(out) & (dtype == 0 ? 15ull : 7ull))) return (int)hipErrorInvalidValue;
+  DD_DISPATCH_DTYPE(dtype, up_cat_align_launch, q, field, feat, feat_sb, feat_sc, feat_sh, feat_sw, out, up, static_cast<hipStream_t>(stream));
+  return (int)hipGetLastError();
+}
+
+extern "C" int dd_up_cat_align_bwd_t(const void* g_out, const float* g_up, int B, int cf, int C, int pad, int h, int w, int H, int W, void* g_feat,
+                                     float* g_field, int dtype, void* stream) {
+  UcaGeom q;
+  if (!g_out || (!g_feat && !g_field) || !up_cat_align_geom(B, cf, C, pad, h, w, H, W, dtype, q)) return (int)hipErrorInvalidValue;
+  DD_DISPATCH_DTYPE(dtype, up_cat_align_bwd_launch, q, g_out, g_up, g_feat, g_field, static_cast<hipStream_t>(stream));
+  return (int)hipGetLastError();
+}
 
 static bool up_cat_pad_ok(const void* x, int B, int h, int w, int C1, int C2, int mode, int dtype) {
   const int H = mode == 2 ? h : 2 * h, W = mode == 2 ? w : 2 * w;
diff --git a/dynamo-depth_amd/csrc/dd_redu.hip b/dynamo-depth_amd/csrc/dd_redu.hip
--- a/dynamo-depth_amd/csrc/dd_redu.hip
+++ b/dynamo-depth_amd/csrc/dd_redu.hip
@@ -18,7 +18,8 @@
 
 template <int COUT, int LPP, int QUADS>
 __global__ __launch_bounds__(RD_NT) void redu_fwd_kernel(const float* __restrict__ a, const float* __restrict__ b, const float* __restrict__ w,
-                                                         const float* __restrict__ bias, long long P, float* __restrict__ y) {
+                                                         const float* __restrict__ bias, const float* __restrict__ addend, long long P,
+                                                         float* __restrict__ y) {
   constexpr int C4 = LPP * QUADS, PX = RD_NT / LPP;
   __shared__ float4 s_w[COUT * 2 * C4];
   rd_stage_weights<C4>(w, COUT, s_w);
@@ -49,7 +50,10 @@
     }
     if (q == 0 && p < P) {
 #pragma unroll
-      for (int co = 0; co < COUT; ++co) y[p * COUT + co] = acc[co] + bv[co];
+      for (int co = 0; co < COUT; ++co) {
+        const float v = acc[co] + bv[co];
+        y[p * COUT + co] = addend ? v + addend[p * COUT + co] : v;
+      }
     }
   }
 }
@@ -213,12 +217,23 @@
 #define DD_REDU_NO_LDS(co, qd) 0
 #define DD_REDU_WG_LDS(co, qd) ((size_t)dd::RD_NT * ((((co) * (qd) * 8 + (co))) | 1) * sizeof(float))
 
-extern "C" int dd_redu_fwd(const float* a, const float* b, const float* weight, const float* bias, long long P, int C, int cout, float* y, void* stream) {
+static int redu_fwd_launch(const float* a, const float* b, const float* weight, const float* bias, const float* addend, long long P, int C, int cout, float* y,
+                           void* stream) {
   if (!a || !b || !weight || !y || P < 1 || !dd_redu_supported(C, cout)) return (int)hipErrorInvalidValue;
   hipStream_t st = (hipStream_t)stream;
   const dim3 grid(dd::redu_blocks(P, dd::redu_shape(C).lpp));
-  DD_REDU_DISPATCH(redu_fwd_kernel, grid, DD_REDU_NO_LDS, a, b, weight, bias, P, y);
+  DD_REDU_DISPATCH(redu_fwd_kernel, grid, DD_REDU_NO_LDS, a, b, weight, bias, addend, P, y);
   return (int)hipGetLastError();
+}
+
+extern "C" int dd_redu_fwd(const float* a, const float* b, const float* weight, const float* bias, long long P, int C, int cout, float* y, void* stream) {
+  return redu_fwd_launch(a, b, weight, bias, nullptr, P, C, cout, y, stream);
+}
+
+extern "C" int dd_redu_res_fwd(const float* a, const float* b, const float* weight, const float* bias, const float* addend, long long P, int C, int cout,
+                               float* y, void* stream) {
+  if (!addend) return (int)hipErrorInvalidValue;
+  return redu_fwd_launch(a, b, weight, bias, addend, P, C, cout, y, stream);
 }
 
 extern "C" int dd_redu_bwd_data(const float* g_out, const float* weight, long long P, int C, int cout, float* g_a, float* g_b, void* stream) {
diff --git a/dynamo-depth_amd/hipops/abi.py b/dynamo-depth_amd/hipops/abi.py
--- a/dynamo-depth_amd/hipops/abi.py
+++ b/dynamo-depth_amd/hipops/abi.py
@@ -180,6 +180,8 @@
         "dd_reflect_pad1_nhwc_bwd_t": (i, [v, i, i, i, i, v, i, v]),
         "dd_up_cat_pad_t": (i, [v, v, i, i, i, i, i, i, i, v, i, v]),
         "dd_up_cat_pad_bwd_t": (i, [v, v, i, i, i, i, i, i, i, v, v, i, v]),
+        "dd_up_cat_align_t": (i, [v, v, C.c_longlong, C.c_longlong, C.c_longlong, C.c_longlong, i, i, i, i, i, i, i, i, v, v, i, v]),
+        "dd_up_cat_align_bwd_t": (i, [v, v, i, i, i, i, i, i, i, i, v, v, i, v]),
         "dd_layer_norm_fwd": (i, [v, C.c_longlong, i, v, v, f, v, v, v, v]),
         "dd_layer_norm_bwd": (i, [v, v, v, v, v, C.c_longlong, i, v, v, v, z, v]),
         "dd_layer_norm_workspace_bytes": (z, [i]),
@@ -195,6 +197,7 @@
         "dd_redu_supported": (i, [i, i]),
         "dd_redu_workspace_bytes": (z, [C.c_longlong, i, i]),
         "dd_redu_fwd": (i, [v, v, v, v, C.c_longlong, i, i, v, v]),
+        "dd_redu_res_fwd": (i, [v, v, v, v, v, C.c_longlong, i, i, v, v]),
         "dd_redu_bwd_data": (i, [v, v, C.c_longlong, i, i, v, v, v]),
         "dd_redu_bwd_weight": (i, [v, v, v, C.c_longlong, i, i, v, v, v, z, v]),
         "dd_conv_head_supported": (i, [i]),
@@ -221,6 +224,8 @@
         "dd_conv3x3_mfma_wgrad_workspace_bytes": (z, [i, i, i, i, i]),
         "dd_conv3x3_mfma_bwd_weight": (i, [v, v, i, i, i, i, i, i, v, v, z, v]),
         "dd_conv3x3_mfma_bwd_weight_n": (i, [v, v, i, i, i, i, i, i, i, v, v, z, v]),
+        "dd_conv3x3_mfma_wgrad_bias_workspace_bytes": (z, [i, i, i, i, i, i]),
+        "dd_conv3x3_mfma_bwd_weight_bias_n": (i, [v, v, i, i, i, i, i, i, i, i, v, v, v, z, v]),
         "dd_conv3x3_half_supported": (i, [i, i]),
         "dd_conv3x3_half_pack_bytes": (z, [i, i]),
         "dd_conv3x3_half_pack": (i, [v, C.c_longlong, C.c_longlong, C.c_longlong, C.c_longlong, i, i, i, v, v, v]),
@@ -262,16 +267,17 @@
     "dd_channel_sum_nhwc", "dd_channel_sum_workspace_bytes", "dd_reflect_pad1_nhwc", "dd_reflect_pad1_nhwc_bwd",
     "dd_dwconv3x3_nhwc", "dd_dwconv3x3_nhwc_bwd_data", "dd_dwconv3x3_nhwc_bwd_weight", "dd_dwconv3x3_workspace_bytes", "dd_conv3x3_cout1_bwd_data",
     "dd_prepare_frames", "dd_prepare_frames_workspace_bytes", "dd_pyramid_down2", "dd_pack_rgb", "dd_depth_metrics", "dd_depth_metrics_workspace_bytes", "dd_depth_metrics_masked", "dd_depth_metrics_masked_workspace_bytes", "dd_depth_metrics_accumulate", "dd_odom_snippet_count", "dd_odom_snippets", "dd_motion_pr", "dd_fill_contours", "dd_lidar_depth_points", "dd_lidar_depth_points_workspace_bytes", "dd_vis_frame", "dd_vis_flow_tiles", "dd_export_depth", "dd_export_plane_u8", "dd_bn_act_fwd", "dd_bn_act_bwd", "dd_bn_workspace_bytes",
-    "dd_bn_act_fwd_t", "dd_bn_act_bwd_t", "dd_channel_sum_nhwc_t", "dd_reflect_pad1_nhwc_t", "dd_reflect_pad1_nhwc_bwd_t", "dd_up_cat_pad_t", "dd_up_cat_pad_bwd_t",
+    "dd_bn_act_fwd_t", "dd_bn_act_bwd_t", "dd_channel_sum_nhwc_t", "dd_reflect_pad1_nhwc_t", "dd_reflect_pad1_nhwc_bwd_t", "dd_up_cat_pad_t", "dd_up_cat_pad_bwd_t", "dd_up_cat_align_t", "dd_up_cat_align_bwd_t",
     "dd_layer_norm_fwd", "dd_layer_norm_bwd", "dd_layer_norm_workspace_bytes", "dd_layer_scale_bwd", "dd_layer_scale_workspace_bytes",
     "dd_jpeg_workspace_bytes", "dd_jpeg_decode", "dd_resize_workspace_bytes", "dd_resize_bicubic", "dd_layer_norm_fwd_t", "dd_layer_norm_bwd_t", "dd_layer_scale_bwd_t", "dd_layer_scale_fwd_t", "dd_dwconv3x3_nhwc_t", "dd_dwconv3x3_nhwc_bwd_data_t",
     "dd_dwconv3x3_nhwc_bwd_weight_t", "dd_adam_chunk", "dd_adam_multi", "dd_conv_small_supported", "dd_conv_small_workspace_bytes",
     "dd_conv_small_fwd", "dd_conv_small_bwd_data", "dd_conv_small_bwd_weight", "dd_conv_head_supported", "dd_conv_head_workspace_bytes", "dd_conv_head_fwd",
-    "dd_conv_head_bwd_weight", "dd_redu_supported", "dd_redu_workspace_bytes", "dd_redu_fwd", "dd_redu_bwd_data", "dd_redu_bwd_weight",
+    "dd_conv_head_bwd_weight", "dd_redu_supported", "dd_redu_workspace_bytes", "dd_redu_fwd", "dd_redu_res_fwd", "dd_redu_bwd_data", "dd_redu_bwd_weight",
     "dd_conv3x3_mfma_supported", "dd_conv3x3_mfma_pack_bytes", "dd_conv3x3_mfma_pack", "dd_conv3x3_mfma_pack_many_job_words",
     "dd_conv3x3_mfma_pack_many_blocks", "dd_conv3x3_mfma_pack_many", "dd_conv3x3_mfma", "dd_conv3x3_mfma_n",
     "dd_conv3x3_mfma_flat_supported", "dd_conv3x3_mfma_flat_workspace_bytes", "dd_conv3x3_mfma_flat", "dd_conv3x3_mfma_flat_n",
-    "dd_conv3x3_mfma_wgrad_workspace_bytes", "dd_conv3x3_mfma_bwd_weight", "dd_conv3x3_mfma_bwd_weight_n",
+    "dd_conv3x3_mfma_wgrad_workspace_bytes", "dd_conv3x3_mfma_bwd_weight", "dd_conv3x3_mfma_bwd_weight_n", "dd_conv3x3_mfma_wgrad_bias_workspace_bytes",
+    "dd_conv3x3_mfma_bwd_weight_bias_n",
     "dd_conv3x3_half_supported", "dd_conv3x3_half_pack_bytes", "dd_conv3x3_half_pack", "dd_conv3x3_half",
     "dd_conv3x3_half_wgrad_workspace_bytes", "dd_conv3x3_half_bwd_weight",
     "dd_pw_gemm_pack_bytes", "dd_mlp_pack", "dd_pw_gemm", "dd_gelu_pair", "dd_mlp_fwd_supported", "dd_mlp_fwd",
diff --git a/dynamo-depth_amd/hipops/functions.py b/dynamo-depth_amd/hipops/functions.py
--- a/dynamo-depth_amd/hipops/functions.py
+++ b/dynamo-depth_amd/hipops/functions.py
@@ -306,7 +306,7 @@
 class ReduFn(torch.autograd.Function):
 
     @staticmethod
-    def forward(ctx, a, b, weight, bias):
+    def forward(ctx, a, b, weight, bias, res=None):
         lib = L.load()
         B, Cc, H, W = a.shape
         cout = weight.shape[0]
@@ -314,7 +314,12 @@
         wm = weight.reshape(cout, 2 * Cc)
         if not wm.is_contiguous():
             wm = wm.contiguous()
-        L.check(lib.dd_redu_fwd(_p(a), _p(b), _p(wm), _p(bias), B * H * W, Cc, cout, _p(y), L.current_stream()), "dd_redu_fwd")
+        if res is None:
+            L.check(lib.dd_redu_fwd(_p(a), _p(b), _p(wm), _p(bias), B * H * W, Cc, cout, _p(y), L.current_stream()), "dd_redu_fwd")
+        else:
+            if res.dtype != torch.float32 or tuple(res.shape) != (B, cout, H, W):
+                raise L.DynamoHipError("ReduFn: the residual must be fp32 of the result's shape")
+            L.check(lib.dd_redu_res_fwd(_p(a), _p(b), _p(wm), _p(bias), _p(_dense_nhwc(res)), B * H * W, Cc, cout, _p(y), L.current_stream()), "dd_redu_res_fwd")
         ctx.save_for_backward(a, b, wm)
         ctx.has_bias = bias is not None
         ctx.wshape = tuple(weight.shape)
@@ -340,7 +345,7 @@
             ws = _ws(nbytes, g.device)
             L.check(lib.dd_redu_bwd_weight(_p(a), _p(b), _p(g), P, Cc, cout, _p(gw), _p(gbias), _p(ws), nbytes, L.current_stream()), "dd_redu_bwd_weight")
             gw = gw.view(ctx.wshape)
-        return ga, gb, gw, gbias
+        return ga, gb, gw, gbias, (g if len(ctx.needs_input_grad) > 4 and ctx.needs_input_grad[4] else None)
 
 
 def head_conv_ok(x, weight, stride, padding, dilation, groups):
@@ -504,6 +509,13 @@
 
 def mfma_conv_calls():
     return _MFMA_CONV_CALLS[0]
+
+
+_MFMA_WGRAD_BIAS_CALLS = [0]
+
+
+def mfma_wgrad_bias_calls():
+    return _MFMA_WGRAD_BIAS_CALLS[0]
 
 
 _PRODUCTS = {"highest": 6, "high": 3, "medium": 1}
@@ -573,13 +585,21 @@
             if (cout % 4 == 0 and min(cin, cout) >= 32 and os.environ.get("DD_STOCK_MFMA_WGRAD", "0") != "1"
                     and (products < 6 or not _flat_shape(B, Hi, Wi, pad, cin, cout))):
                 flat = torch.empty(cout * 9 * cin, dtype=torch.float32, device=g.device)
-                nbytes = _ws_bytes("dd_conv3x3_mfma_wgrad_workspace_bytes", B, Ho, Wo, cin, cout)
-                ws = _ws(nbytes, g.device)
-                L.check(lib.dd_conv3x3_mfma_bwd_weight_n(_p(x), _p(g), B, Hi, Wi, cin, cout, pad, products, _p(flat), _p(ws), nbytes, stream), "dd_conv3x3_mfma_bwd_weight")
+                if has_bias and ctx.needs_input_grad[2] and os.environ.get("DD_STOCK_MFMA_WGRAD_BIAS", "0") != "1":
+                    gb = torch.empty(cout, dtype=torch.float32, device=g.device)
+                    nbytes = _ws_bytes("dd_conv3x3_mfma_wgrad_bias_workspace_bytes", B, Ho, Wo, cin, cout, 0)
+                    ws = _ws(nbytes, g.device)
+                    L.check(lib.dd_conv3x3_mfma_bwd_weight_bias_n(_p(x), _p(g), B, Hi, Wi, cin, cout, pad, products, 0, _p(flat), _p(gb), _p(ws), nbytes, stream),
+                            "dd_conv3x3_mfma_bwd_weight_bias")
+                    _MFMA_WGRAD_BIAS_CALLS[0] += 1
+                else:
+                    nbytes = _ws_bytes("dd_conv3x3_mfma_wgrad_workspace_bytes", B, Ho, Wo, cin, cout)
+                    ws = _ws(nbytes, g.device)
+                    L.check(lib.dd_conv3x3_mfma_bwd_weight_n(_p(x), _p(g), B, Hi, Wi, cin, cout, pad, products, _p(flat), _p(ws), nbytes, stream), "dd_conv3x3_mfma_bwd_weight")
                 gw = flat.view(cout, 3, 3, cin).permute(0, 3, 1, 2)
             else:
                 gw = _wgrad_3x3_library(g, x, weight, pad)
-        if has_bias and ctx.needs_input_grad[2]:
+        if has_bias and ctx.needs_input_grad[2] and gb is None:
             gb = _channel_sum(g, B * Ho * Wo, cout, DTYPE_CODE[g.dtype], stream) if cout <= 256 else g.sum((0, 2, 3))
         return gx, gw, gb, None
 
@@ -759,6 +779,65 @@
     return reflect_pad1(y)
 
 
+_MOTION_GLUE_CALLS = [0]
+
+
+def motion_glue_calls():
+    return _MOTION_GLUE_CALLS[0]
+
+
+def motion_glue_pad(cf, C):
+    return (-(cf + C)) % 8 if cf + C >= 32 else 0
+
+
+def motion_glue_ok(field, feat):
+    if os.environ.get("DD_STOCK_MOTION_GLUE", "0") == "1" or os.environ.get("DD_STOCK_CAT_CONV", "0") == "1" or torch.is_autocast_enabled():
+        return False
+    if not (field.is_cuda and feat.is_cuda and field.dtype == torch.float32 and feat.dtype in DTYPE_CODE and field.dim() == 4 and feat.dim() == 4):
+        return False
+    cf, C = field.shape[1], feat.shape[1]
+    if not (1 <= cf <= 4 and field.shape[0] == feat.shape[0]):
+        return False
+    total = cf + C
+    if total <= 16:
+        return os.environ.get("DD_STOCK_SMALL_CONV", "0") != "1"
+    return total >= 32 and _nhwc(feat)
+
+
+class MotionGlueFn(torch.autograd.Function):
+
+    @staticmethod
+    def forward(ctx, field, feat, pad):
+        B, cf, h, w = field.shape
+        _, C, H, W = feat.shape
+        field = _dense_nhwc(field)
+        out = _nhwc_empty(B, cf + C + pad, H, W, feat.device, dtype=feat.dtype)
+        up = _nhwc_empty(B, cf, H, W, feat.device)
+        sf = feat.stride()
+        L.check(L.load().dd_up_cat_align_t(_p(field), _p(feat), sf[0], sf[1], sf[2], sf[3], B, cf, C, pad, h, w, H, W, _p(out), _p(up),
+                                           DTYPE_CODE[feat.dtype], L.current_stream()), "dd_up_cat_align_t")
+        _MOTION_GLUE_CALLS[0] += 1
+        ctx.cfg = (B, cf, C, pad, h, w, H, W, feat.dtype)
+        return out, up
+
+    @staticmethod
+    def backward(ctx, g_out, g_up):
+        B, cf, C, pad, h, w, H, W, dtype = ctx.cfg
+        need_field, need_feat = ctx.needs_input_grad[0], ctx.needs_input_grad[1]
+        if g_out is None and g_up is None or not (need_field or need_feat):
+            return None, None, None
+        if g_out is None:
+            g_out = torch.zeros((B, H, W, cf + C + pad), dtype=dtype, device=g_up.device).permute(0, 3, 1, 2)
+        g_out = _dense_nhwc(g_out.to(dtype))
+        if g_up is not None:
+            g_up = _dense_nhwc(g_up.to(torch.float32))
+        g_feat = _nhwc_empty(B, C, H, W, g_out.device, dtype=dtype) if need_feat else None
+        g_field = _nhwc_empty(B, cf, h, w, g_out.device) if need_field else None
+        L.check(L.load().dd_up_cat_align_bwd_t(_p(g_out), _p(g_up), B, cf, C, pad, h, w, H, W, _p(g_feat), _p(g_field), DTYPE_CODE[dtype],
+                                               L.current_stream()), "dd_up_cat_align_bwd_t")
+        return g_field, g_feat, None
+
+
 class DepthwiseConv3x3NHWCFn(torch.autograd.Function):
 
     @staticmethod
diff --git a/dynamo-depth_amd/networks/layers.py b/dynamo-depth_amd/networks/layers.py
--- a/dynamo-depth_amd/networks/layers.py
+++ b/dynamo-depth_amd/networks/layers.py
@@ -102,6 +102,14 @@
     if key[-1]:
         parts = [_as_channels_last(p) for p in parts]
     x = torch.cat(list(parts) + [zeros], 1)
+    w = F.pad(conv.weight, (0, 0, 0, 0, 0, pad))
+    y = _hip_conv(x, w, conv.bias, conv.stride, conv.padding, conv.dilation, conv.groups)
+    return y if y is not None else F.conv2d(x, w, conv.bias, conv.stride, conv.padding, conv.dilation, conv.groups)
+
+
+def conv_zero_padded(conv, x, pad):
+    if pad == 0:
+        return conv(x)
     w = F.pad(conv.weight, (0, 0, 0, 0, 0, pad))
     y = _hip_conv(x, w, conv.bias, conv.stride, conv.padding, conv.dilation, conv.groups)
     return y if y is not None else F.conv2d(x, w, conv.bias, conv.stride, conv.padding, conv.dilation, conv.groups)
diff --git a/dynamo-depth_amd/networks/motion_decoder.py b/dynamo-depth_amd/networks/motion_decoder.py
--- a/dynamo-depth_amd/networks/motion_decoder.py
+++ b/dynamo-depth_amd/networks/motion_decoder.py
@@ -3,14 +3,16 @@
 import torch
 import torch.nn as nn
 
-from .layers import Conv2d, conv_cat_aligned, stock_slices
+from .layers import Conv2d, conv_cat_aligned, conv_zero_padded, stock_slices
 import torch.nn.functional as F
 
 
-def redu_split(redu, a, b, C):
+def redu_split(redu, a, b, C, res=None):
     from hipops.functions import ConvBiasFn, ReduFn, SplitChannelsFn, redu_ok
     if redu_ok(a, b, redu):
-        return ReduFn.apply(a, b, redu.weight, redu.bias)
+        return ReduFn.apply(a, b, redu.weight, redu.bias, res)
+    if res is not None:
+        return redu_split(redu, a, b, C) + res
     w = redu.weight
     if not stock_slices("redu"):
         wa, wb = SplitChannelsFn.apply(w, C)
@@ -47,11 +49,24 @@
         per_level = []
         for level in range(len(self.num_inp_feat)):
             feat = pose_feat[-1 - level]
+            convs = getattr(self, "refine_motion_conv{}".format(level))
+            redu = getattr(self, "refine_motion_redu{}".format(level))
+            if not amp and field.is_cuda:
+                from hipops.functions import MotionGlueFn, motion_glue_ok, motion_glue_pad
+                if motion_glue_ok(field, feat) and convs[0].groups == 1 and convs[0].padding_mode == "zeros":
+                    pad = motion_glue_pad(field.shape[1], feat.shape[1])
+                    x, up = MotionGlueFn.apply(field, feat, pad)
+                    a = conv_zero_padded(convs[0], x, pad)
+                    b = convs[1](a)
+                    if os.environ.get("DD_STOCK_REDU_CAT", "0") != "1":
+                        field = redu_split(redu, a, b, a.shape[1], up)
+                    else:
+                        field = redu(torch.cat((a, b), 1)) + up
+                    per_level.append(field)
+                    continue
             up = F.interpolate(field, size=feat.shape[-2:], mode="bilinear", align_corners=False)
-            convs = getattr(self, "refine_motion_conv{}".format(level))
             a = conv_cat_aligned(convs[0], (up.to(feat.dtype) if amp else up, feat))
             b = convs[1](a)
-            redu = getattr(self, "refine_motion_redu{}".format(level))
             if a.is_cuda and os.environ.get("DD_STOCK_REDU_CAT", "0") != "1":
                 C = a.shape[1]
                 field = redu_split(redu, a, b, C)
diff --git a/include/dynamo_hip.h b/include/dynamo_hip.h
--- a/include/dynamo_hip.h
+++ b/include/dynamo_hip.h
@@ -251,6 +251,11 @@
 int dd_up_cat_pad_bwd_t(const void* g_out, const void* x, int B, int h, int w, int C1, int C2, int mode, int elu, void* g_x, void* g_skip,
                         int dtype, void* stream);
 
+int dd_up_cat_align_t(const float* field, const void* feat, long long feat_sb, long long feat_sc, long long feat_sh, long long feat_sw, int B, int cf,
+                      int C, int pad, int h, int w, int H, int W, void* out, float* up, int dtype, void* stream);
+int dd_up_cat_align_bwd_t(const void* g_out, const float* g_up, int B, int cf, int C, int pad, int h, int w, int H, int W, void* g_feat, float* g_field,
+                          int dtype, void* stream);
+
 int dd_layer_norm_fwd(const float* x, long long rows, int C, const float* gamma, const float* beta, float eps, float* y, float* mean,
                       float* rstd, void* stream);
 int dd_layer_norm_bwd(const float* x, const float* g_out, const float* gamma, const float* mean, const float* rstd, long long rows, int C,
@@ -276,6 +281,8 @@
 int dd_redu_supported(int C, int cout);
 size_t dd_redu_workspace_bytes(long long P, int C, int cout);
 int dd_redu_fwd(const float* a, const float* b, const float* weight, const float* bias, long long P, int C, int cout, float* y, void* stream);
+int dd_redu_res_fwd(const float* a, const float* b, const float* weight, const float* bias, const float* addend, long long P, int C, int cout, float* y,
+                    void* stream);
 int dd_redu_bwd_data(const float* g_out, const float* weight, long long P, int C, int cout, float* g_a, float* g_b, void* stream);
 int dd_redu_bwd_weight(const float* a, const float* b, const float* g_out, long long P, int C, int cout, float* g_weight, float* g_bias, void* workspace,
                        size_t workspace_bytes, void* stream);
@@ -317,6 +324,9 @@
                                size_t workspace_bytes, void* stream);
 int dd_conv3x3_mfma_bwd_weight_n(const float* x, const float* g_out, int B, int Hi, int Wi, int cin, int cout, int pad, int products, float* g_weight,
                                  void* workspace, size_t workspace_bytes, void* stream);
+size_t dd_conv3x3_mfma_wgrad_bias_workspace_bytes(int B, int Ho, int Wo, int cin, int cout, int splits);
+int dd_conv3x3_mfma_bwd_weight_bias_n(const float* x, const float* g_out, int B, int Hi, int Wi, int cin, int cout, int pad, int products, int splits,
+                                      float* g_weight, float* g_bias, void* workspace, size_t workspace_bytes, void* stream);
 
 int dd_conv3x3_half_supported(int cin, int cout);
 size_t dd_conv3x3_half_pack_bytes(int n_out, int k_in);
```

Result: no change. 355.2 (median of 6 runs) (+0.4%).
